# jinseikenai/glomeruli_segmentation

Measured on AMD Instinct MI355X. Metric: patches/sec (1024x512 RGB) ESPNet p=2 q=8 5 classes, HBM-resident, two batches in flight, higher is better.
Workload: dtype f32; 1 GPU; ESPNet p=2 q=8 encoder+decoder, batch=32 synthetic 1024x512 uint8 BGR tiles per GPU, normalise+forward+argmax+counts, inputs resident in HBM, steps rotate through 4 distinct batches, 2 batch(es) in flight (engine lanes, one HIP stream each) for `value`; global_batch=32, weights=espnet_fold1 (tests/golden), parallelism=tile-range per rank x1

## Files before the change

### glomeruli_segmentation_amd/_lib.py

```python
import ctypes
import os

_PKG = os.path.dirname(os.path.abspath(__file__))
LIB_PATH = os.path.join(_PKG, "libglomseg.so")
if os.environ.get("GLOMSEG_LIB") and os.environ.get("GLOMSEG_EXPERIMENT") == "1":
    LIB_PATH = os.environ["GLOMSEG_LIB"]

GS_OK = 0
GS_IN_U8_BGR_NHWC = 0
GS_IN_F32_NCHW = 1
ABI_VERSION = 9
GS_BUILD_DIAG = 1
GS_FORM_NONE = -1
GS_MAX_ENSEMBLE_C = 8
MAX_CROPS_PER_CALL = 64

STATUS_NAMES = {0: "GS_OK", 1: "GS_ERR_INVALID", 2: "GS_ERR_HIP", 3: "GS_ERR_NOMEM", 4: "GS_ERR_UNSUPPORTED",
                5: "GS_ERR_NODEVICE", 6: "GS_ERR_DEVICE_FAULT"}


class GlomsegError(RuntimeError):
    def __init__(self, status, message):
        super().__init__("%s: %s" % (STATUS_NAMES.get(status, status), message))
        self.status = status


class LayerDesc(ctypes.Structure):
    _fields_ = [("name", ctypes.c_char * 96), ("offset", ctypes.c_int64), ("ndim", ctypes.c_int32),
                ("shape", ctypes.c_int32 * 4)]


class CropDesc(ctypes.Structure):
    _fields_ = [("in_off", ctypes.c_int64), ("out_off", ctypes.c_int64), ("h", ctypes.c_int32), ("w", ctypes.c_int32),
                ("x1", ctypes.c_int32), ("y1", ctypes.c_int32)]


class PasteTarget(ctypes.Structure):
    _fields_ = [("slide_map", ctypes.c_void_p), ("map_h", ctypes.c_int32), ("map_w", ctypes.c_int32), ("ds", ctypes.c_int32),
                ("sx_lut", ctypes.c_void_p), ("sy_lut", ctypes.c_void_p)]


class CropOverlay(ctypes.Structure):
    _fields_ = [("palette_rgb", ctypes.c_void_p), ("n_colours", ctypes.c_int32), ("wa", ctypes.c_float), ("wb", ctypes.c_float),
                ("out_bgr", ctypes.POINTER(ctypes.c_void_p))]


class CropScoring(ctypes.Structure):
    _fields_ = [("labels", ctypes.POINTER(ctypes.c_void_p)), ("conf", ctypes.c_void_p), ("seen", ctypes.c_void_p),
                ("gt_overlay_bgr", ctypes.POINTER(ctypes.c_void_p)), ("gt_clamp", ctypes.c_int32)]


class EvalBox(ctypes.Structure):
    _fields_ = [("x0", ctypes.c_int32), ("y0", ctypes.c_int32), ("x1", ctypes.c_int32), ("y1", ctypes.c_int32),
                ("raster_w", ctypes.c_int32), ("raster_h", ctypes.c_int32), ("offset", ctypes.c_int64)]


class EvalSet(ctypes.Structure):
    _fields_ = [("rasters", ctypes.c_void_p), ("raster_bytes", ctypes.c_int64), ("boxes", ctypes.c_void_p),
                ("n_boxes", ctypes.c_int32), ("win_ptr", ctypes.c_void_p), ("win_idx", ctypes.c_void_p), ("n_idx", ctypes.c_int32),
                ("small_map", ctypes.c_void_p)]


class DetectorLayerPlan(ctypes.Structure):
    _fields_ = [("images", ctypes.c_int64), ("in_h", ctypes.c_int32), ("in_w", ctypes.c_int32), ("out_h", ctypes.c_int32),
                ("out_w", ctypes.c_int32), ("form", ctypes.c_int32)]


class DetectorPlan(ctypes.Structure):
    _fields_ = [("hf", ctypes.c_int32), ("wf", ctypes.c_int32), ("workspace_bytes", ctypes.c_int64), ("n_layers", ctypes.c_int32),
                ("layers", DetectorLayerPlan * 16)]


class KernelTime(ctypes.Structure):
    _fields_ = [("name", ctypes.c_char * 64), ("total_ms", ctypes.c_double), ("launches", ctypes.c_int64),
                ("flops_per_tile", ctypes.c_double)]


_P = ctypes.c_void_p
_FP = ctypes.POINTER(ctypes.c_float)
_I = ctypes.c_int

PROTOTYPES = {
    "gs_last_error": (ctypes.c_char_p, []),
    "gs_abi_version": (_I, []),
    "gs_build_flags": (_I, []),
    "gs_device_fault_check": (_I, []),
    "gs_espnet_create": (_I, [_P, ctypes.POINTER(LayerDesc), _I, _I, _I, _I, _I, ctypes.POINTER(_P)]),
    "gs_espnet_destroy": (None, [_P]),
    "gs_espnet_reserve": (_I, [_P, _I, _I, _I]),
    "gs_espnet_forward": (_I, [_P, _P, _I, _I, _I, _I, _FP, _FP, _P, _P, _P, _P]),
    "gs_espnet_set_lanes": (_I, [_P, _I]),
    "gs_espnet_lanes": (_I, [_P]),
    "gs_espnet_forward_lane": (_I, [_P, _I, _P, _I, _I, _I, _I, _FP, _FP, _P, _P, _P, _P]),
    "gs_espnet_segment_host": (_I, [_P, _P, _I, _I, _I, _FP, _FP, _I, _P, _P]),
    "gs_espnet_segment_crops": (_I, [_P, _I, _P, ctypes.POINTER(CropDesc), _I, _FP, _FP, _I, _I, _P, _P, _P,
                                ctypes.POINTER(PasteTarget), _P]),
    "gs_espnet_ensemble_segment_crops": (_I, [ctypes.POINTER(_P), _I, _P, ctypes.POINTER(CropDesc), _I, _FP, _FP, _I, _I, _P, _P, _P,
                                         ctypes.POINTER(PasteTarget), _P]),
    "gs_espnet_segment_crops_host": (_I, [ctypes.POINTER(_P), _I, ctypes.POINTER(_P), ctypes.POINTER(_I), ctypes.POINTER(_I), _I, _FP, _FP,
                                     _I, _I, _I, ctypes.POINTER(_P), _P, _P, ctypes.POINTER(PasteTarget), ctypes.POINTER(_I),
                                     ctypes.POINTER(_I), ctypes.POINTER(CropOverlay)]),
    "gs_plan_crop_batches": (_I, [ctypes.POINTER(_I), ctypes.POINTER(_I), _I, _I, ctypes.POINTER(_I), _I, ctypes.POINTER(_I)]),
    "gs_host_block_is_pinned": (_I, [_P, ctypes.c_size_t]),
    "gs_espnet_ensemble_forward": (_I, [ctypes.POINTER(_P), _I, _P, _I, _I, _I, _FP, _FP, _P, _P, _P]),
    "gs_espnet_read_stage": (_I, [_P, ctypes.c_char_p, _I, _P, ctypes.c_size_t, ctypes.POINTER(_I * 3)]),
    "gs_espnet_block_forward": (_I, [_P, _I, _I, _I, _P, _I, _I, _P]),
    "gs_espnet_plan_forward": (_I, [_I, _I, _I, _I, _I, _I, _I, ctypes.POINTER(_I), _I, ctypes.POINTER(_I)]),
    "gs_espnet_form_info": (_I, [_I, _I, ctypes.POINTER(ctypes.c_char_p), ctypes.POINTER(_I)]),
    "gs_espnet_profile_enable": (_I, [_P, _I]),
    "gs_espnet_profile_read": (_I, [_P, ctypes.POINTER(KernelTime), _I, ctypes.POINTER(_I)]),
    "gs_crop_preprocess": (_I, [_P, _I, _I, _FP, _FP, _I, _I, _P, _P]),
    "gs_mask_resize_nearest": (_I, [_P, _I, _I, _I, _I, _P, _P]),
    "gs_find_contours": (_I, [_P, _I, _I, _I, _P, _I, _P, _I, ctypes.POINTER(_I), ctypes.POINTER(_I)]),
    "gs_arc_length_closed": (ctypes.c_double, [_P, _I]),
    "gs_approx_poly_closed": (_I, [_P, _I, ctypes.c_double, _P]),
    "gs_wsi_paste_max": (_I, [_P, _I, _I, _I, _P, _I, _I, _I, _I, _P]),
    "gs_wsi_paste_max_lut": (_I, [_P, _I, _I, _I, _P, _P, _P, _I, _I, _I, _I, _P]),
    "gs_overlay_classmap": (_I, [_P, _P, _I, _I, _P, _I, ctypes.c_float, ctypes.c_float, _P, _P]),
    "gs_confusion_u8": (_I, [_P, _P, ctypes.c_longlong, _I, _P, _P]),
    "gs_wsi_eval_windows": (_I, [_I, _I, _I, _I, ctypes.POINTER(EvalSet), ctypes.POINTER(EvalSet), _P, _P, _I, _I, _P, _P, _P]),
    "gs_conv2d_nhwc": (_I, [_P, _I, _I, _I, _I, _P, _I, _I, _I, _P, _I, _I, _I, _P, _P]),
    "gs_conv2d_nhwc_form": (_I, [_I] * 10 + [ctypes.POINTER(ctypes.c_char_p)]),
    "gs_roialign": (_I, [_P, _I, _I, _I, _I, _P, _P, _I, _I, _P, _P]),
    "gs_nms": (_I, [_P, _P, _I, ctypes.c_float, ctypes.c_float, _I, _P, _P, _P]),
    "gs_detector_create": (_I, [_P, ctypes.POINTER(LayerDesc), _I, ctypes.POINTER(_P)]),
    "gs_detector_destroy": (None, [_P]),
    "gs_detector_max_detections": (_I, []),
    "gs_detector_num_proposals": (_I, []),
    "gs_detector_layer_info": (_I, [_I, ctypes.POINTER(ctypes.c_char_p)] + [ctypes.POINTER(_I)] * 6),
    "gs_detector_plan": (_I, [_I, _I, _I, ctypes.POINTER(DetectorPlan)]),
    "gs_detector_set_thresholds": (_I, [_P, ctypes.c_float, ctypes.c_float, ctypes.c_float]),
    "gs_detector_forward": (_I, [_P, _P, _I, _I, _I, _P, _P, _P, _P, _P, _P, _P, _P, _P]),
    "gs_detector_detect_host": (_I, [_P, ctypes.POINTER(_P), _I, _I, _I, _I, _P, _P, _P, _P]),
}

SCORING_PROTOTYPES = {
    "gs_espnet_score_crops": (_I, [_P, _P, ctypes.POINTER(CropDesc), _I, _I, _I, _I, _P, _P, _P]),
    "gs_espnet_segment_crops_host_scored": (_I, PROTOTYPES["gs_espnet_segment_crops_host"][1] + [ctypes.POINTER(CropScoring)]),
}

_lib = None


def load():
    global _lib
    if _lib is not None:
        return _lib
    if not os.path.exists(LIB_PATH):
        raise ImportError(
            "%s is missing: build it with `python -m glomeruli_segmentation_amd.build` "
            "(hipcc --offload-arch=gfx950).  There is no CPU fallback." % LIB_PATH)
    lib = ctypes.CDLL(LIB_PATH, mode=ctypes.RTLD_GLOBAL)
    for name, (res, args) in list(PROTOTYPES.items()) + list(SCORING_PROTOTYPES.items()):
        fn = getattr(lib, name)
        fn.restype = res
        fn.argtypes = args
    if lib.gs_abi_version() != ABI_VERSION:
        raise ImportError("libglomseg.so ABI %d != binding ABI %d: rebuild" % (lib.gs_abi_version(), ABI_VERSION))
    if (lib.gs_build_flags() & GS_BUILD_DIAG) and os.environ.get("GLOMSEG_ALLOW_DIAG") != "1":
        raise ImportError("%s is a -DGS_DIAG experiment build (its timing variants return wrong results by construction); "
                          "set GLOMSEG_ALLOW_DIAG=1 to load it for an A/B measurement" % LIB_PATH)
    _lib = lib
    return lib


def check(status):
    if status != GS_OK:
        raise GlomsegError(status, load().gs_last_error().decode("utf-8", "replace"))


def fptr3(values):
    arr = (ctypes.c_float * len(values))(*[float(v) for v in values])
    return arr
```

### glomeruli_segmentation_amd/build.py

```python
import os
import subprocess
import sys
import tempfile

PKG = os.path.dirname(os.path.abspath(__file__))
CSRC = os.path.join(PKG, "csrc")
LIB = os.path.join(PKG, "libglomseg.so")
SOURCES = ["espnet.hip", "dec_tail.hip", "crops.hip", "detect_ops.hip", "detector.hip", "wsi_eval.hip", "contours.cpp"]
HEADERS = ["gs_internal.h", "conv_mfma.h", "dec_tail.h", "dec_tail_args.h", "espnet_kernels.h", "crop_sample.h", "crop_plan.h", "detect_math.h", "detect_plan.h", "host_copy.h", "host_jobs.h", "host_pipe.h",
           os.path.join("..", "..", "include", "glomseg.h"), os.path.join("..", "..", "include", "glomseg_scoring.h")]
FLAGS = ["-O3", "--offload-arch=gfx950", "-std=c++17", "-fPIC", "-Wall", "-Wno-unused-result",
         "-Wno-unused-value"]


def _sources():
    return [s for s in SOURCES if os.path.exists(os.path.join(CSRC, s))]


def _stale(lib):
    if not os.path.exists(lib):
        return True
    t = os.path.getmtime(lib)
    deps = [os.path.join(CSRC, s) for s in _sources() + HEADERS] + [os.path.abspath(__file__)]
    deps += [os.path.join(CSRC, f) for f in os.listdir(CSRC) if f.endswith(".h") or f.endswith(".inc")]
    return any(os.path.getmtime(d) > t for d in deps)


def build_lib(force=False, verbose=False, out=None, extra_flags=()):
    lib = os.path.abspath(out) if out else LIB
    if not (force or _stale(lib)):
        return lib
    hipcc = os.environ.get("HIPCC", "/opt/rocm/bin/hipcc")
    os.makedirs(os.path.dirname(lib), exist_ok=True)
    objdir = CSRC if out is None else tempfile.mkdtemp(prefix="glomseg_obj_")
    objs = []
    procs = []
    for s in _sources():
        o = os.path.join(objdir, s.replace(".hip", ".o").replace(".cpp", ".o"))
        objs.append(o)
        cmd = [hipcc] + FLAGS + list(extra_flags) + (["-x", "hip"] if s.endswith(".cpp") else []) + ["-c", os.path.join(CSRC, s), "-o", o]
        if verbose:
            print(" ".join(cmd))
        procs.append((cmd, subprocess.Popen(cmd)))
    for cmd, p in procs:
        if p.wait() != 0:
            raise RuntimeError("hipcc failed: " + " ".join(cmd))
    cmd = [hipcc, "--offload-arch=gfx950", "-shared", "-fPIC", "-o", lib] + objs + ["-Wl,-rpath,/opt/rocm/lib"]
    if verbose:
        print(" ".join(cmd))
    subprocess.check_call(cmd)
    return lib


if __name__ == "__main__":
    argv = sys.argv[1:]
    extra = []
    if "--" in argv:
        extra = argv[argv.index("--") + 1:]
        argv = argv[:argv.index("--")]
    out = argv[argv.index("--out") + 1] if "--out" in argv else None
    print(build_lib(force="--force" in argv or out is not None, verbose=True, out=out, extra_flags=extra))
```

### glomeruli_segmentation_amd/csrc/conv_mfma.h

```cpp
#pragma once
#include <map>
#include <mutex>
#include <type_traits>

#include "gs_internal.h"

namespace gs {

#ifdef GS_DIAG
constexpr bool kDiag = true;
#else
constexpr bool kDiag = false;
#endif

template <int N, typename F>
__device__ __forceinline__ void static_for(F &&f)
{
    if constexpr (N > 0) {
        static_for<N - 1>(f);
        f(std::integral_constant<int, N - 1>{});
    }
}

typedef float f32x16 __attribute__((ext_vector_type(16)));
typedef float f32x4 __attribute__((ext_vector_type(4)));

template <int MT>
struct Mfma;
template <>
struct Mfma<32> {
    static constexpr int KL = 2, NACC = 16;
    using acc_t = f32x16;
    static __device__ __forceinline__ acc_t run(float a, float b, acc_t c)
    {
        return __builtin_amdgcn_mfma_f32_32x32x2f32(a, b, c, 0, 0, 0);
    }
    static __device__ __forceinline__ int row(int r, int kq) { return (r & 3) + 8 * (r >> 2) + 4 * kq; }
};
template <>
struct Mfma<16> {
    static constexpr int KL = 4, NACC = 4;
    using acc_t = f32x4;
    static __device__ __forceinline__ acc_t run(float a, float b, acc_t c)
    {
        return __builtin_amdgcn_mfma_f32_16x16x4f32(a, b, c, 0, 0, 0);
    }
    static __device__ __forceinline__ int row(int r, int kq) { return kq * 4 + r; }
};

struct ConvArgs {
    const float *in;
    long long in_sn;
    int in_sc, in_pitch, in_off;
    unsigned in_img_bytes;
    const float *wpack;
    int wfloats;
    float *out;
    long long out_sn;
    int out_sc, out_pitch, out_off;
    unsigned out_img_bytes, res_img_bytes;
    const float *res;
    long long res_sn;
    int res_sc, res_pitch, res_off;
    float *out2;
    long long out2_sn;
    int out2_sc, out2_pitch, out2_off, out2_coff;
    unsigned out2_img_bytes;
    float *out3;
    long long out3_sn;
    int out3_sc, out3_pitch, out3_off, nout3;
    unsigned out3_img_bytes;
    int bnl_s0, bnl_s1;
    int stagger;
    int prio_mode;
    unsigned long long *stamp;
    int N, H, W;
    int strips;
    int total_tasks;
    int wu;
};

typedef unsigned u32x3_t __attribute__((ext_vector_type(3)));
typedef unsigned u32x2_t __attribute__((ext_vector_type(2)));
typedef unsigned u32x4_t __attribute__((ext_vector_type(4)));

template <int N, int AUX = 0>
__device__ __forceinline__ void buf_load_vec(const __amdgpu_buffer_rsrc_t &rs, int voff, int soff, float *dst)
{
    if constexpr (N == 1) {
        dst[0] = __builtin_bit_cast(float, __builtin_amdgcn_raw_buffer_load_b32(rs, voff, soff, AUX));
    } else if constexpr (N == 2) {
        const u32x2_t v = __builtin_amdgcn_raw_buffer_load_b64(rs, voff, soff, AUX);
        const unsigned e0 = v[0], e1 = v[1];
        dst[0] = __builtin_bit_cast(float, e0);
        dst[1] = __builtin_bit_cast(float, e1);
    } else {
        static_assert(N == 4 || N == 8, "vector width");
#pragma unroll
        for (int h = 0; h < N / 4; ++h) {
            const u32x4_t v = __builtin_amdgcn_raw_buffer_load_b128(rs, voff + 16 * h, soff, AUX);
            const unsigned e0 = v[0], e1 = v[1], e2 = v[2], e3 = v[3];
            dst[4 * h + 0] = __builtin_bit_cast(float, e0);
            dst[4 * h + 1] = __builtin_bit_cast(float, e1);
            dst[4 * h + 2] = __builtin_bit_cast(float, e2);
            dst[4 * h + 3] = __builtin_bit_cast(float, e3);
        }
    }
}
template <int N, int AUX = 0>
__device__ __forceinline__ void buf_store_vec(const __amdgpu_buffer_rsrc_t &rs, int voff, const float *src)
{
    if constexpr (N == 1) {
        __builtin_amdgcn_raw_buffer_store_b32(__builtin_bit_cast(unsigned, src[0]), rs, voff, 0, AUX);
    } else if constexpr (N == 2) {
        u32x2_t v;
        v[0] = __builtin_bit_cast(unsigned, src[0]);
        v[1] = __builtin_bit_cast(unsigned, src[1]);
        __builtin_amdgcn_raw_buffer_store_b64(v, rs, voff, 0, AUX);
    } else {
#pragma unroll
        for (int h = 0; h < N / 4; ++h) {
            u32x4_t v;
#pragma unroll
            for (int j = 0; j < 4; ++j)
                v[j] = __builtin_bit_cast(unsigned, src[4 * h + j]);
            __builtin_amdgcn_raw_buffer_store_b128(v, rs, voff + 16 * h, 0, AUX);
        }
    }
}

__device__ __forceinline__ float prelu_pin(float alpha)
{
    return alpha <= 1.0f ? __builtin_inff() : -__builtin_inff();
}
__device__ __forceinline__ float prelu_med3(float v, float alpha, float pin)
{
    return __builtin_amdgcn_fmed3f(v, alpha * v, pin);
}

constexpr int F_BNACT = 1;
constexpr int F_RES = 2;
constexpr int F_NOSTORE = 4;
constexpr int F_DUAL = 8;
constexpr int F_S2PAIR = 512;
constexpr int F_VEC = 1024;
constexpr int F_RES_NT = 8192;
constexpr int F_ST_NT = 16384;
constexpr int F_ST2_NT = 32768;
constexpr int F_IN_NT = 65536;
constexpr int F_A_GLOBAL = 131072;
constexpr int F_FUSE1X1 = 262144;
constexpr int F_S2_FLIP = 1048576;
constexpr int F_SKIP_PAD = 4194304;
constexpr int F_BNLOAD = 8388608;
constexpr int F_X_NOLOAD = 16;
constexpr int F_X_NOLDS = 32;
constexpr int F_X_NOEPI = 64;
constexpr int F_X_STAMP2 = 4096;
constexpr int STAMP2_SLOTS = 128;
constexpr int F_X_STAMP = 128;
constexpr int F_X_NOEPIMEM = 2097152;
constexpr int F_X_RESL2 = 33554432;
constexpr int F_X_STL2 = 67108864;
constexpr int F_X_ALL = F_X_NOLOAD | F_X_NOLDS | F_X_NOEPI | F_X_STAMP | F_X_STAMP2 | F_X_NOEPIMEM | F_X_RESL2 | F_X_STL2;

struct ConvImage {
    int nrow, cout, w, bn, tab, total;
};
constexpr ConvImage conv_image(int CINP, int TAPS, int NDIL, int NOUT1, int NOUT, bool bn, bool dual = false, int fuse_nacc = 0)
{
    ConvImage im{};
    im.nrow = NOUT1 > NOUT ? NOUT1 : NOUT;
    im.cout = NOUT1 + (NDIL - 1) * NOUT;
    im.w = NDIL * TAPS * CINP * im.nrow;
    im.bn = (bn ? 3 * im.cout : 0) + (dual ? 3 * im.cout : 0);
    im.tab = NDIL * fuse_nacc * 64;
    im.total = (im.w + im.bn + im.tab + 3) / 4 * 4;
    return im;
}

#ifndef CFG_STAGE_ROT
#define CFG_STAGE_ROT 17
#endif
#ifndef CFG_L3_RING
#define CFG_L3_RING 13
#endif
#ifndef CFG_L2_RING
#define CFG_L2_RING 27
#endif
constexpr int conv_ring_depth(int MT, int TAPS, int NDIL, int P, int G)
{
    return (MT == 32 && TAPS == 9 && NDIL == 5 && (P == 1 || P == 2) && G == 13) ? CFG_L3_RING
           : (MT == 16 && TAPS == 9 && NDIL == 5 && P == 4 && G == 9) ? CFG_L2_RING
                                                                    : G * (TAPS == 9 ? 3 : 1);
}

#define M_KL_OF(MT_) (Mfma<MT_>::KL)
template <int MT, int WAVES, int CINP, int TAPS, int STRIDE, int NDIL, int NOUT1, int NOUT, int P, int G, int FLAGS>
__global__ void __launch_bounds__(WAVES * 64, WAVES >= 8 ? WAVES / 8 : 2) conv_mfma_kernel(const ConvArgs a)
{
    constexpr bool BNACT = FLAGS & F_BNACT, RES = FLAGS & F_RES, STORE1 = !(FLAGS & F_NOSTORE), DUAL = FLAGS & F_DUAL;
    constexpr bool S2P = FLAGS & F_S2PAIR;
    constexpr bool VEC = FLAGS & F_VEC;
    constexpr bool AGL = FLAGS & F_A_GLOBAL, FUSE = FLAGS & F_FUSE1X1;
    constexpr bool S2FLIP = FLAGS & F_S2_FLIP;
    constexpr bool SKIP = FLAGS & F_SKIP_PAD;
    constexpr bool BNL = FLAGS & F_BNLOAD;
    static_assert(!BNL || ((FLAGS & F_S2PAIR) && !(FLAGS & (F_BNACT | F_A_GLOBAL | F_VEC))), "F_BNLOAD is for the plain stride-2 reduce");
    static_assert(!SKIP || (TAPS == 9 && STRIDE == 1 && !(FLAGS & F_S2PAIR) && G * M_KL_OF(MT) == CINP),
                  "F_SKIP_PAD: unit-stride 3x3 with one tap row per chunk");
    static_assert(!S2FLIP || (STRIDE == 2 && TAPS == 9 && NDIL == 1), "F_S2_FLIP is for the stride-2 3x3 reduce");
    static_assert(kDiag || !(FLAGS & F_X_ALL), "timing / stamp variants exist in -DGS_DIAG builds only");
    constexpr int IAUX = (FLAGS & F_IN_NT) ? 2 : 0;
    constexpr int RAUX = (FLAGS & F_RES_NT) ? 2 : 0, SAUX = (FLAGS & F_ST_NT) ? 2 : 0, SAUX2 = (FLAGS & F_ST2_NT) ? 2 : 0;
    static_assert(!VEC || (STRIDE == 1 && (P == 2 || P == 4 || P == 8)), "F_VEC needs unit stride and P in {2,4,8}");
    static_assert(!S2P || (STRIDE == 2 && TAPS == 9 && NDIL == 1), "F_S2PAIR is for the stride-2 3x3 reduce");
    using M = Mfma<MT>;
    constexpr int KL = M::KL;
    constexpr int NSTEP = CINP / KL;
    constexpr int NROW = NOUT1 > NOUT ? NOUT1 : NOUT;
    constexpr int COUT = NOUT1 + (NDIL - 1) * NOUT;
    constexpr int TYN = TAPS == 1 ? 1 : 3;
    constexpr int TXN = TAPS == 9 ? 3 : 1;
    constexpr int XSTEP = P * MT;
    constexpr int RGN = TYN * NSTEP;
    constexpr int D = G * TXN;
    constexpr int R = conv_ring_depth(MT, TAPS, NDIL, P, G);
    constexpr int RA = R;
    static_assert(D % R == 0 && (R == D || !(FLAGS & (F_S2PAIR | F_BNLOAD))), "the ring divides the chunk");
    constexpr int CPD = RGN / G;
    constexpr int NCHUNK = NDIL * CPD;
    static_assert(CINP % KL == 0, "k-steps must tile");
    static_assert(TAPS == 1 || TAPS == 9, "1x1 or 3x3");
    static_assert(RGN % G == 0, "chunk must divide the row groups of one dilation");
    static_assert(NROW <= MT, "one MFMA row block");
    constexpr int KSTR = 4;

    extern __shared__ __attribute__((aligned(16))) float lds[];
    const int tid = threadIdx.x;
    unsigned long long tstamp0 = 0;
    if (FLAGS & (F_X_STAMP | F_X_STAMP2))
        tstamp0 = __builtin_amdgcn_s_memrealtime();
    constexpr int WFL = NDIL * TAPS * CINP * NROW;
    constexpr int LDS_SRC0 = AGL ? WFL : 0;
    static_assert(!AGL || WFL % 4 == 0, "LDS-DMA source must stay 16-byte aligned");
    static_assert(!FUSE || (TAPS == 9 && BNACT), "the fused 1x1 follows a branch kernel's epilogue");
    const float *bnp = lds + (WFL - LDS_SRC0);
    constexpr int BNFL = (BNACT ? 3 * COUT : 0) + (DUAL ? 3 * COUT : 0);
    const float *tab = bnp + BNFL;
    constexpr int BNL_C = CINP + M::KL;
    const float *bnl = lds + (conv_image(CINP, TAPS, NDIL, NOUT1, NOUT, BNACT, DUAL, FUSE ? M::NACC : 0).total - LDS_SRC0);
    const __amdgpu_buffer_rsrc_t rsrc_w =
        __builtin_amdgcn_make_buffer_rsrc(const_cast<float *>(a.wpack), 0, AGL ? WFL * 4 : 0, 0x00020000);

    const int lane = tid & 63;
    const int wid = __builtin_amdgcn_readfirstlane(tid >> 6);
    const int px = lane % MT, kq = lane / MT;
    const int xl = VEC ? px * P : px;
    const int voff = (kq * a.in_sc + xl * STRIDE) * 4;
    const int lbase = kq * NROW + (px < NROW ? px : NROW - 1);
    const int vout = (kq * KSTR * a.out_sc + xl) * 4;
    const int vres = RES ? (kq * KSTR * a.res_sc + xl) * 4 : 0;
    const int vout2 = DUAL ? (kq * KSTR * a.out2_sc + xl) * 4 : 0;
    const int vout3 = FUSE ? (kq * KSTR * a.out3_sc + xl) * 4 : 0;
    const int prio_mode = kDiag ? a.prio_mode : 1;
    const bool second_of_simd = WAVES >= 8 ? wid >= WAVES / 2 : blockIdx.x >= gridDim.x / 2;

    const int NB = gridDim.x;
    const int wu = a.wu;
    int t0, t1, tstride;
    if ((NB & 7) == 0) {
        const int xcd = blockIdx.x & 7, per = NB >> 3;
        const int c0 = (int)((long long)a.total_tasks * xcd / 8), c1 = (int)((long long)a.total_tasks * (xcd + 1) / 8);
        t0 = c0 + (blockIdx.x >> 3) * wu + wid;
        t1 = c1;
        tstride = per * wu;
    } else {
        t0 = blockIdx.x * wu + wid;
        t1 = a.total_tasks;
        tstride = NB * wu;
    }
    if (wid >= wu)
        t0 = t1;
    const long long wg = (long long)blockIdx.x * WAVES + wid;
    const int tasks_per_img = a.H * a.strips;
    bool staged = false;

    float aq[RA], bq[S2P ? 1 : R][P];
    float bl[S2P ? G : 1][P][3];

    for (int task = t0; task < t1 || !staged; task += tstride) {
        const bool idle = task >= t1;
        const int tk = idle ? (a.total_tasks - 1) : task;
        const int n = tk / tasks_per_img;
        const int rem = tk - n * tasks_per_img;
        const int img_stride = tstride / tasks_per_img > 0 ? tstride / tasks_per_img : 1;
        const int yrot = SKIP ? a.H / 2 : 0;
        const int y0r = rem / a.strips;
        const int y = SKIP && ((n / img_stride) & 1) ? (y0r + yrot >= a.H ? y0r + yrot - a.H : y0r + yrot) : y0r;
        const int x0 = (rem - y0r * a.strips) * XSTEP;

        const __amdgpu_buffer_rsrc_t rsrc = __builtin_amdgcn_make_buffer_rsrc(
            const_cast<float *>(a.in + (long long)n * a.in_sn), 0, a.in_img_bytes, 0x00020000);
        const int sbase = (a.in_off + y * STRIDE * a.in_pitch + x0 * STRIDE) * 4;
        const int tn = task + tstride < t1 ? task + tstride : tk;
        const int n_n = tn / tasks_per_img;
        const int rem_n = tn - n_n * tasks_per_img;
        const int y0r_n = rem_n / a.strips;
        const int y_n = SKIP && ((n_n / img_stride) & 1) ? (y0r_n + yrot >= a.H ? y0r_n + yrot - a.H : y0r_n + yrot) : y0r_n;
        const __amdgpu_buffer_rsrc_t rsrc_n = __builtin_amdgcn_make_buffer_rsrc(
            const_cast<float *>(a.in + (long long)n_n * a.in_sn), 0, a.in_img_bytes, 0x00020000);
        const int sbase_n = (a.in_off + y_n * STRIDE * a.in_pitch + (rem_n - y0r_n * a.strips) * XSTEP * STRIDE) * 4;
        const bool flip = S2FLIP && (y & 1), flip_n = S2FLIP && (y_n & 1);
        const __amdgpu_buffer_rsrc_t rout =
            __builtin_amdgcn_make_buffer_rsrc(a.out + (long long)n * a.out_sn, 0, a.out_img_bytes, 0x00020000);
        const int sout = (a.out_off + y * a.out_pitch + x0) * 4;
        const __amdgpu_buffer_rsrc_t rres = __builtin_amdgcn_make_buffer_rsrc(
            const_cast<float *>(RES ? a.res + (long long)n * a.res_sn : a.in), 0, RES ? a.res_img_bytes : 0u, 0x00020000);
        const int sres = RES ? (a.res_off + y * a.res_pitch + x0) * 4 : 0;
        const __amdgpu_buffer_rsrc_t rout2 = __builtin_amdgcn_make_buffer_rsrc(
            DUAL ? a.out2 + (long long)n * a.out2_sn : a.out, 0, DUAL ? a.out2_img_bytes : 0u, 0x00020000);
        const int sout2 = DUAL ? (a.out2_off + y * a.out2_pitch + x0) * 4 : 0;
        const __amdgpu_buffer_rsrc_t rout3 = __builtin_amdgcn_make_buffer_rsrc(
            FUSE ? a.out3 + (long long)n * a.out3_sn : a.out, 0, FUSE ? a.out3_img_bytes : 0u, 0x00020000);
        const int sout3 = FUSE ? (a.out3_off + y * a.out3_pitch + x0) * 4 : 0;

        typename M::acc_t acc[P];
        typename M::acc_t acc2[FUSE ? P : 1];
        auto chunk_live = [&](int yy, int c) {
            const int di = c / CPD, ty = c - di * CPD;
            return ty == 1 || (ty == 0 ? yy >= (1 << di) : yy + (1 << di) < a.H);
        };
        const int c_first = SKIP && !chunk_live(y, 0) ? 1 : 0;
        const int c_first_n = SKIP && !chunk_live(y_n, 0) ? 1 : 0;

        constexpr int OOB = 0x7ffffff0;
        int vo[P], vr[P], vo2[P], vo3[P];
#pragma unroll
        for (int p = 0; p < P; ++p) {
            const bool xok = x0 + (VEC ? xl : p * MT + px) < a.W;
            vo[p] = xok ? vout + (VEC ? 0 : p * MT * 4) : OOB;
            vr[p] = xok ? vres + (VEC ? 0 : p * MT * 4) : OOB;
            vo2[p] = xok ? vout2 + (VEC ? 0 : p * MT * 4) : OOB;
            vo3[p] = xok ? vout3 + (VEC ? 0 : p * MT * 4) : OOB;
        }
        constexpr int RR = RES ? M::NACC : 1;
        float resv[RR][P];
        auto load_res = [&](int di, int r) {
            if (!RES)
                return;
            if (FLAGS & F_X_NOEPIMEM) {
#pragma unroll
                for (int p = 0; p < P; ++p)
                    resv[r % RR][p] = __builtin_bit_cast(float, di + r + p);
                return;
            }
            const int nout = di == 0 ? NOUT1 : NOUT;
            const int cb = di == 0 ? 0 : NOUT1 + (di - 1) * NOUT;
            const int ch0 = M::row(r, 0);
            const bool live = ch0 + kq * KSTR < nout;
            const int sr = (cb + ch0) * a.res_sc * 4 + sres;
            if (VEC) {
                if (FLAGS & F_X_RESL2)
                    buf_load_vec<P, RAUX>(rres, live ? ((int)(wg & 255) * 8192 + ((vr[0] + sr) & 0x1ff0)) : OOB, 0, resv[r % RR]);
                else
                    buf_load_vec<P, RAUX>(rres, live ? vr[0] : OOB, sr, resv[r % RR]);
                return;
            }
#pragma unroll
            for (int p = 0; p < P; ++p)
                resv[r % RR][p] = __builtin_bit_cast(
                    float, __builtin_amdgcn_raw_buffer_load_b32(rres, live ? vr[p] : OOB, sr, RAUX));
        };
        auto prefetch_res = [&](int di) {
#pragma unroll
            for (int r = 0; r < RR; ++r)
                load_res(di, r);
        };

        auto decode_rg = [&](int cw, int g, int &ty0, int &sidx) {
            if constexpr (G % NSTEP == 0) {
                ty0 = cw * (G / NSTEP) + g / NSTEP;
                sidx = g % NSTEP;
            } else if constexpr (NSTEP % G == 0) {
                constexpr int CPR = NSTEP / G;
                ty0 = cw / CPR;
                sidx = (cw - ty0 * CPR) * G + g;
            } else {
                const int rg = cw * G + g;
                ty0 = rg / NSTEP;
                sidx = rg - ty0 * NSTEP;
            }
        };
        auto fetch_b = [&](const __amdgpu_buffer_rsrc_t &rs, int sb, int c, int g, int tx, bool fl) {
            const int di = c / CPD;
            int ty0, sidx;
            decode_rg(c - di * CPD, g, ty0, sidx);
            const int ty = S2FLIP && fl ? TYN - 1 - ty0 : ty0;
            const int toff = TAPS == 9 ? ((ty - 1) * a.in_pitch + (tx - 1)) << di : 0;
            const int soff = sb + (toff + sidx * KL * a.in_sc) * 4;
            if ((FLAGS & F_X_NOLOAD) && staged)
                return;
            if (VEC) {
                buf_load_vec<P, IAUX>(rs, voff, soff, bq[S2P ? 0 : (g * TXN + tx) % R]);
                return;
            }
#pragma unroll
            for (int p = 0; p < P; ++p)
                bq[(g * TXN + tx) % R][p] = __builtin_bit_cast(
                    float, __builtin_amdgcn_raw_buffer_load_b32(rs, voff + p * MT * STRIDE * 4, soff, IAUX));
        };
        auto fetch_pair = [&](const __amdgpu_buffer_rsrc_t &rs, int sb, int c, int g, bool fl) {
            if ((FLAGS & F_X_NOLOAD) && staged)
                return;
            int ty0, sidx;
            decode_rg(c, g, ty0, sidx);
            const int ty = S2FLIP && fl ? TYN - 1 - ty0 : ty0;
            const int soff = sb + ((ty - 1) * a.in_pitch - 1 + sidx * KL * a.in_sc) * 4;
#pragma unroll
            for (int p = 0; p < P; ++p) {
                const u32x3_t v = __builtin_amdgcn_raw_buffer_load_b96(rs, voff + p * MT * STRIDE * 4, soff, IAUX);
                const unsigned e0 = v[0], e1 = v[1], e2 = v[2];
                bl[g][p][0] = __builtin_bit_cast(float, e0);
                bl[g][p][1] = __builtin_bit_cast(float, e1);
                bl[g][p][2] = __builtin_bit_cast(float, e2);
            }
        };
        auto fetch_a = [&](int c, int g, int tx, bool fl) {
            const int di = c / CPD;
            int ty0, sidx;
            decode_rg(c - di * CPD, g, ty0, sidx);
            const int ty = S2FLIP && fl ? TYN - 1 - ty0 : ty0;
            const int tap = TAPS == 9 ? ty * 3 + tx : 0;
            if ((FLAGS & F_X_NOLDS) && staged)
                return;
            if (AGL)
                aq[(g * TXN + tx) % R] = __builtin_bit_cast(
                    float, __builtin_amdgcn_raw_buffer_load_b32(rsrc_w, lbase * 4, (((di * TAPS + tap) * CINP + sidx * KL) * NROW) * 4, 0));
            else
                aq[(g * TXN + tx) % R] = lds[((di * TAPS + tap) * CINP + sidx * KL) * NROW + lbase];
        };

        auto bnl_fetch = [&](int cc, int gg, int yy, bool ff, float &sc2, float &sh2, float &al2, bool &raw) {
            int ty0c, sidxc;
            decode_rg(cc, gg, ty0c, sidxc);
            const int tyc = S2FLIP && ff ? TYN - 1 - ty0c : ty0c;
            raw = sidxc >= a.bnl_s0 && sidxc < a.bnl_s1;
            const bool padrow = yy * STRIDE + tyc - 1 < 0 && raw;
            const int ch = (padrow ? NSTEP : sidxc) * KL + kq;
            sc2 = bnl[ch];
            sh2 = bnl[BNL_C + ch];
            al2 = bnl[2 * BNL_C + ch];
        };
        float tsc = 1.0f, tsh = 0.0f, tal = 1.0f, tpin = 0.0f;
        float nsc = 1.0f, nsh = 0.0f, nal = 1.0f;
        bool traw = false, nraw = false;
        float bt[BNL ? 2 : 1][P][3];
        static_assert(!BNL || G % 2 == 0, "F_BNLOAD: the two-group operand buffer alternates by row-group parity");
        auto bnl_apply = [&](float &dst, float v, float sc2, float sh2, float al2, float pin2, bool zero) {
            v = v * sc2 + sh2;
            v = prelu_med3(v, al2, pin2);
            dst = zero ? 0.0f : v;
        };

        if (task == t0) {
#pragma unroll
            for (int g = 0; g < G; ++g) {
                if (S2P) {
                    fetch_pair(rsrc, sbase, 0, g, flip);
                    continue;
                }
#pragma unroll
                for (int tx = 0; tx < TXN; ++tx)
                    if (g * TXN + tx < R)
                        fetch_b(rsrc, sbase, c_first, g, tx, flip);
            }
        }
        if (!staged) {
            const int pieces = (a.wfloats - LDS_SRC0 + 255) / 256;
            if ((FLAGS & F_X_STAMP2) && lane == 0)
                a.stamp[wg * STAMP2_SLOTS + STAMP2_SLOTS - 2] = __builtin_amdgcn_s_memrealtime();
            const int rot = (int)((blockIdx.x * (unsigned)CFG_STAGE_ROT) % (unsigned)(pieces > 0 ? pieces : 1));
            for (int j0 = wid; j0 < pieces; j0 += WAVES) {
                const int j = j0 + rot < pieces ? j0 + rot : j0 + rot - pieces;
                __builtin_amdgcn_global_load_lds(
                    (const __attribute__((address_space(1))) void *)(a.wpack + LDS_SRC0 + j * 256 + lane * 4),
                    (__attribute__((address_space(3))) void *)(lds + j * 256), 16, 0, 0);
            }
            if ((FLAGS & F_X_STAMP2) && lane == 0)
                a.stamp[wg * STAMP2_SLOTS + STAMP2_SLOTS - 1] = __builtin_amdgcn_s_memrealtime();
            __syncthreads();
            staged = true;
        }
        if (idle)
            break;
        if ((FLAGS & F_X_STAMP) && lane == 0 && task == t0) {
            a.stamp[wg * 8 + 0] = tstamp0;
            a.stamp[wg * 8 + 1] = __builtin_amdgcn_s_memrealtime();
        }
        if ((FLAGS & F_X_STAMP2) && lane == 0 && task == t0) {
            a.stamp[wg * STAMP2_SLOTS + 0] = tstamp0;
            a.stamp[wg * STAMP2_SLOTS + 1] = __builtin_amdgcn_s_memrealtime();
        }
        const int ti_ = (FLAGS & F_X_STAMP2) ? (task - t0) / tstride : 0;
        const bool stamp2 = (FLAGS & F_X_STAMP2) && lane == 0 && 2 + (ti_ + 1) * 2 * NCHUNK <= STAMP2_SLOTS;
        const long long sbase2 = wg * STAMP2_SLOTS + 2 + ti_ * 2 * NCHUNK;
        if (kDiag && a.stagger > 0 && task == t0) {
            const int ph = second_of_simd ? 1 : 0;
            for (int z = 0; z < a.stagger * ph; ++z)
                __builtin_amdgcn_s_sleep(16);
        }
        if (task == t0) {
#pragma unroll
            for (int g = 0; g < G; ++g)
#pragma unroll
                for (int tx = 0; tx < TXN; ++tx)
                    if (g * TXN + tx < R)
                        fetch_a(c_first, g, tx, flip);
        }

        if (BNL) {
            bnl_fetch(c_first, 0, y, flip, tsc, tsh, tal, traw);
            bnl_fetch(c_first, 1, y, flip, nsc, nsh, nal, nraw);
            tpin = prelu_pin(tal);
#pragma unroll
            for (int p = 0; p < P; ++p)
#pragma unroll
                for (int t = 0; t < 3; ++t)
                    bnl_apply(bt[0][p][t], bl[0][p][t], tsc, tsh, tal, tpin, t == 0 && p == 0 && x0 == 0 && px == 0);
        }
        if (FUSE) {
#pragma unroll
            for (int p = 0; p < P; ++p)
                acc2[p] = (typename M::acc_t)(0.0f);
        }
        if (prio_mode == 1) {
            if ((((task - t0) / tstride) + (second_of_simd ? 1 : 0)) & 1)
                __builtin_amdgcn_s_setprio(1);
            else
                __builtin_amdgcn_s_setprio(0);
        } else if (prio_mode == 3 && task == t0) {
            if (second_of_simd)
                __builtin_amdgcn_s_setprio(1);
        }

        struct EpiParams {
            float scale = 1.0f, shift = 0.0f, alpha = 1.0f, scale2 = 1.0f, shift2 = 0.0f, alpha2 = 1.0f, a2 = 0.0f;
        };
        auto epi_params = [&](int di, auto r_) __attribute__((always_inline)) {
            constexpr int r = decltype(r_)::value;
            const int nout = di == 0 ? NOUT1 : NOUT;
            const int cb = di == 0 ? 0 : NOUT1 + (di - 1) * NOUT;
            const int ch0 = M::row(r, 0);
            const bool live = ch0 + kq * KSTR < nout;
            EpiParams q;
            q.a2 = (FUSE && BNACT) ? tab[(di * M::NACC + r) * 64 + lane] : 0.0f;
            if (BNACT) {
                const float *bp = bnp + (live ? cb + ch0 + kq * KSTR : 0);
                q.scale = bp[0];
                q.shift = bp[COUT];
                q.alpha = bp[2 * COUT];
                if (DUAL) {
                    q.scale2 = bp[3 * COUT];
                    q.shift2 = bp[4 * COUT];
                    q.alpha2 = bp[5 * COUT];
                }
            }
            return q;
        };
        auto epi_reg = [&](int di, auto r_) __attribute__((always_inline)) {
            constexpr int r = decltype(r_)::value;
            const int nout = di == 0 ? NOUT1 : NOUT;
            const int cb = di == 0 ? 0 : NOUT1 + (di - 1) * NOUT;
            const int ch0 = M::row(r, 0);
            const bool live = ch0 + kq * KSTR < nout;
            const EpiParams q = epi_params(di, r_);
            const float a2 = q.a2;
            const int so = (cb + ch0) * a.out_sc * 4 + sout;
            const int so2 = DUAL ? (a.out2_coff + cb + ch0) * a.out2_sc * 4 + sout2 : 0;
            const float scale = q.scale, shift = q.shift, alpha = q.alpha, scale2 = q.scale2, shift2 = q.shift2, alpha2 = q.alpha2;
            float o1[P], o2[P];
            const float pin = prelu_pin(alpha), pin2 = prelu_pin(alpha2);
#pragma unroll
            for (int p = 0; p < P; ++p) {
                float v = acc[p][r];
                if (RES)
                    v += resv[r % RR][p];
                if (BNACT) {
                    v = v * scale + shift;
                    v = prelu_med3(v, alpha, pin);
                }
                o1[p] = v;
                if (!VEC && STORE1)
                    __builtin_amdgcn_raw_buffer_store_b32(__builtin_bit_cast(unsigned, v), rout, live ? vo[p] : OOB, so, SAUX);
                if (DUAL) {
                    float v2 = v * scale2 + shift2;
                    v2 = prelu_med3(v2, alpha2, pin2);
                    o2[p] = v2;
                    if (!VEC)
                        __builtin_amdgcn_raw_buffer_store_b32(__builtin_bit_cast(unsigned, v2), rout2,
                                                              live ? vo2[p] : OOB, so2, SAUX2);
                }
            }
            if (VEC && STORE1 && !(FLAGS & F_X_NOEPIMEM))
                buf_store_vec<P, SAUX>(rout, live ? ((FLAGS & F_X_STL2) ? ((int)(wg & 255) * 8192 + ((vo[0] + so) & 0x1ff0)) : vo[0] + so) : OOB, o1);
            if (VEC && DUAL)
                buf_store_vec<P, SAUX2>(rout2, live ? vo2[0] + so2 : OOB, o2);
            if (FUSE && ch0 < nout) {
#pragma unroll
                for (int p = 0; p < P; ++p)
                    acc2[p] = M::run(a2, o1[p], acc2[p]);
            }
        };

        for (int c = 0; c < NCHUNK; ++c) {
            if (NDIL > 1 && c % CPD == 0 && prio_mode == 0) {
                if (((c / CPD) + (second_of_simd ? 1 : 0)) & 1)
                    __builtin_amdgcn_s_setprio(1);
                else
                    __builtin_amdgcn_s_setprio(0);
            }
            if (RES && c % CPD == 0)
                prefetch_res(c / CPD);
            if (c % CPD == 0 && c < 2 * CPD) {
#pragma unroll
                for (int p = 0; p < P; ++p)
                    acc[p] = (typename M::acc_t)(0.0f);
            }
            int nxl = c + 1;
            if (SKIP)
                while (nxl < NCHUNK && !chunk_live(y, nxl))
                    ++nxl;
            const bool last = nxl >= NCHUNK;
            const int nx = last ? c_first_n : nxl;
            const __amdgpu_buffer_rsrc_t rs = last ? rsrc_n : rsrc;
            const int sb = last ? sbase_n : sbase;
            const bool fl = last ? flip_n : flip;
            auto refill = [&](int u) __attribute__((always_inline)) {
                const int v = u + R;
                if (v < D && R < D) {
                    fetch_b(rsrc, sbase, c, v / TXN, v % TXN, flip);
                    fetch_a(c, v / TXN, v % TXN, flip);
                } else {
                    const int gn = (v - D) / TXN, txn = (v - D) % TXN;
                    if (!S2P)
                        fetch_b(rs, sb, nx, gn, txn, fl);
                    else if (txn == 2)
                        fetch_pair(rs, sb, nx, gn, fl);
                    fetch_a(nx, gn, txn, fl);
                }
            };
            if (!SKIP || chunk_live(y, c)) {
#pragma unroll
            for (int g = 0; g < G; ++g)
#pragma unroll
                for (int tx = 0; tx < TXN; ++tx) {
                    const int u = g * TXN + tx;
                    const bool ahead = BNL && (g + 1 < G || !last);
                    if (BNL && tx == 0) {
                        tsc = nsc;
                        tsh = nsh;
                        tal = nal;
                        traw = nraw;
                        tpin = prelu_pin(tal);
                        if (g + 2 < G)
                            bnl_fetch(c, g + 2, y, flip, nsc, nsh, nal, nraw);
                        else if (!last)
                            bnl_fetch(nx, g + 2 - G, y, flip, nsc, nsh, nal, nraw);
                    }
#pragma unroll
                    for (int p = 0; p < P; ++p) {
                        acc[p] = M::run(aq[u % RA], BNL ? bt[BNL ? g & 1 : 0][p][S2P ? tx : 0]
                                                       : S2P ? bl[S2P ? g : 0][p][S2P ? tx : 0] : bq[S2P ? 0 : u % R][p], acc[p]);
                        if (ahead) {
                            const int e = tx * P + p;
                            if (e < 3 * P)
                                bnl_apply(bt[BNL ? (g + 1) & 1 : 0][e / 3][e % 3], bl[S2P ? (g + 1) % G : 0][e / 3][e % 3], tsc, tsh, tal, tpin,
                                          e == 0 && x0 == 0 && px == 0);
                        }
                    }
                    refill(u);
                    __builtin_amdgcn_sched_barrier(0);
                }
            }
            if (stamp2)
                a.stamp[sbase2 + 2 * c] = __builtin_amdgcn_s_memrealtime();
            if ((c + 1) % CPD != 0)
                continue;
            if (FLAGS & F_X_NOEPI) {
                float keep = 0.0f;
#pragma unroll
                for (int p = 0; p < P; ++p)
#pragma unroll
                    for (int r = 0; r < M::NACC; ++r)
                        keep += acc[p][r];
                if (keep == 123.456f)
                    __builtin_amdgcn_raw_buffer_store_b32(__builtin_bit_cast(unsigned, keep), rout, vout, sout, 0);
                continue;
            }
            const int di = c / CPD;
            static_for<M::NACC>([&](auto r_) { epi_reg(di, r_); });
            if (FUSE && di + 1 == NDIL) {
#pragma unroll
                for (int r = 0; r < M::NACC; ++r) {
                    const int ch0 = M::row(r, 0);
                    if (ch0 >= a.nout3)
                        continue;
                    const bool live3 = ch0 + kq * KSTR < a.nout3;
                    const int so3 = ch0 * a.out3_sc * 4 + sout3;
                    float o3[P];
#pragma unroll
                    for (int p = 0; p < P; ++p) {
                        o3[p] = acc2[p][r];
                        if (!VEC)
                            __builtin_amdgcn_raw_buffer_store_b32(__builtin_bit_cast(unsigned, o3[p]), rout3, live3 ? vo3[p] : OOB, so3, 0);
                    }
                    if (VEC)
                        buf_store_vec<P, 0>(rout3, live3 ? vo3[0] + so3 : OOB, o3);
                }
            }
            if ((FLAGS & F_X_STAMP) && lane == 0 && task == t0)
                a.stamp[wg * 8 + 2 + di] = __builtin_amdgcn_s_memrealtime();
            if (stamp2)
                a.stamp[sbase2 + 2 * c + 1] = __builtin_amdgcn_s_memrealtime();
        }
    }
}

constexpr int conv_wfloats(int CINP, int TAPS, int NDIL, int NOUT1, int NOUT, bool bn, bool dual = false, int fuse_nacc = 0)
{
    return conv_image(CINP, TAPS, NDIL, NOUT1, NOUT, bn, dual, fuse_nacc).total;
}

struct LaunchInfo {
    bool attr_done = false;
    int per_cu = 0;
};

template <int MT, int WAVES, int CINP, int TAPS, int STRIDE, int NDIL, int NOUT1, int NOUT, int P, int G, int FLAGS>
gs_status launch_conv_mfma(ConvArgs a, int num_cus, hipStream_t stream)
{
    auto kern = conv_mfma_kernel<MT, WAVES, CINP, TAPS, STRIDE, NDIL, NOUT1, NOUT, P, G, FLAGS>;
    constexpr ConvImage im = conv_image(CINP, TAPS, NDIL, NOUT1, NOUT, FLAGS & F_BNACT, FLAGS & F_DUAL,
                                        (FLAGS & F_FUSE1X1) ? Mfma<MT>::NACC : 0);
    a.strips = cdiv(a.W, P * MT);
    a.total_tasks = a.N * a.H * a.strips;
    a.prio_mode = 1;
#ifdef GS_DIAG
    if (const char *e = std::getenv("GS_PRIO"))
        a.prio_mode = std::atoi(e);
    if (const char *e = std::getenv("GS_STAGGER"))
        a.stagger = std::atoi(e);
#endif
    constexpr int EXTRA = (FLAGS & F_BNLOAD) ? 3 * (CINP + Mfma<MT>::KL) : 0;
    a.wfloats = im.total + EXTRA;
    const int lds_floats = im.total + EXTRA - ((FLAGS & F_A_GLOBAL) ? im.w : 0);
    const size_t lds_bytes = (size_t)((lds_floats + 255) / 256 * 256) * sizeof(float);
    static std::mutex mu;
    static std::map<int, LaunchInfo> by_device;
    int dev = 0;
    GS_HIP(hipGetDevice(&dev));
    int per_cu;
    {
        std::lock_guard<std::mutex> lock(mu);
        LaunchInfo &li = by_device[dev];
        if (!li.attr_done) {
            GS_HIP(hipFuncSetAttribute(reinterpret_cast<const void *>(kern), hipFuncAttributeMaxDynamicSharedMemorySize,
                                       (int)lds_bytes));
            li.attr_done = true;
        }
        if (li.per_cu == 0) {
            int nb = 0;
            GS_HIP(hipOccupancyMaxActiveBlocksPerMultiprocessor(&nb, reinterpret_cast<const void *>(kern), WAVES * 64, lds_bytes));
            li.per_cu = nb < 1 ? 1 : nb;
        }
        per_cu = li.per_cu;
    }
    int grid = num_cus * per_cu;
    if (grid >= 8) grid = grid / 8 * 8;
    a.wu = WAVES;
    if ((long long)a.total_tasks < (long long)grid * WAVES) {
        a.wu = cdiv(a.total_tasks, grid);
        if (a.wu < 1) a.wu = 1;
        int g = cdiv(a.total_tasks, a.wu);
        if (g >= 8) g = (g + 7) / 8 * 8;
        grid = g < grid ? g : grid;
    }
    if (grid < 1) grid = 1;
    hipLaunchKernelGGL(kern, dim3(grid), dim3(WAVES * 64), lds_bytes, stream, a);
    GS_HIP(hipGetLastError());
    return GS_OK;
}

}
```

### glomeruli_segmentation_amd/csrc/espnet.hip

```cpp
#include <chrono>
#include <cmath>
#include <cstdio>
#include <cstdlib>
#include <functional>
#include <map>
#include <memory>
#include <string>
#include <thread>
#include <vector>

#include "conv_mfma.h"
#include "dec_tail_args.h"
#include "enc_head.h"
#include "enc_head_ens.h"
#include "espnet_config.h"
#include "forward_plan.h"
#include "espnet_kernels.h"
#include "host_copy.h"
#include "host_pipe.h"

namespace gs {

static thread_local std::string g_err;
void set_error(const char *fmt, ...)
{
    char buf[1024];
    va_list ap;
    va_start(ap, fmt);
    vsnprintf(buf, sizeof buf, fmt, ap);
    va_end(ap);
    g_err = buf;
}

#ifdef GS_DIAG
static bool getenv_flag(const char *name)
{
    const char *e = std::getenv(name);
    return e && std::atoi(e) != 0;
}
static bool no_vec() { return getenv_flag("GS_NO_VEC"); }
#else
static constexpr bool no_vec() { return false; }
#endif

enum KernelId {
    K_STEM, K_POOL, K_L2_C1S, K_L2_DOWN, K_L2_C1, K_L2_ESP, K_CAT_B2, K_L3_C1S, K_L3_DOWN, K_L3_C1, K_L3_ESP,
    K_DEC1, K_DEC2, K_DEC3, K_DEC_CONV, K_DEC4, K_DEC_TAIL, K_ENC_HEAD, K_ENC_HEAD_ENS, K_COUNT
};
static const char *kKernelNames[K_COUNT] = {
    "stem_kernel", "pool_kernel", "conv_l2_reduce_s2", "conv_l2_down_branches", "conv_l2_reduce_1x1",
    "conv_l2_esp_branches", "cat_b2_kernel", "conv_l3_reduce_s2", "conv_l3_down_branches", "conv_l3_reduce_1x1",
    "conv_l3_esp_branches", "dec1_kernel", "dec2_kernel", "dec3_kernel", "conv_dec_cbr", "dec4_kernel", "dec_tail_kernel",
    "enc_head_kernel", "enc_head_ens_kernel"};

struct PackedConv {
    long long c1 = -1, br = -1;
    bool fused_next = false;
};

struct Model {
    int classes = 0, p = 0, q = 0;
    int cp = 0;
    bool encoder_only = false;
    int device = 0, num_cus = 256;
#ifdef GS_DIAG
    int variant = 0;
#else
    static constexpr int variant = 0;
#endif
    float *dblob = nullptr;
    float stem_params[537] = {0};
    long long w1, bn1, b1, b2, b3, wcls, br, wup3, w3c, cbr0, wcc, bncc, wup2, bnu2, wclassifier, wtail;
    long long wconv = -1;
    long long wcc_mfma = -1;
    PackedConv l2_0;
    std::vector<PackedConv> l2, l3;
    PackedConv l3_0;

    void *ws = nullptr;
    size_t ws_bytes = 0;
    int ws_n = 0, ws_h = 0, ws_w = 0;
    Act a0c, a0, inp1, inp2, r2[2], bb[3], a1, r3[2], cc[3], o2c, tt, t3, ee, ff;
    float *prob = nullptr;
    size_t prob_bytes = 0;
    std::map<std::string, std::pair<Act, int>> stages;
    void set_stage(const std::string &name, const Act &act, int C)
    {
        for (auto it = stages.begin(); it != stages.end();)
            it = it->second.first.base == act.base ? stages.erase(it) : std::next(it);
        stages[name] = {act, C};
    }
    int last_n = 0;
    bool b2_lazy = false;

    bool profile = false;
    struct Ev { hipEvent_t a, b; int k; };
    std::vector<Ev> events;
    double prof_ms[K_COUNT] = {0};
    long long prof_launches[K_COUNT] = {0};
    double prof_flops[K_COUNT] = {0};
};

struct WeightTable {
    const float *blob;
    std::map<std::string, const gs_layer_desc *> by_name;
    std::string prefix;
    bool ok = true;
    const float *get(const std::string &name, std::initializer_list<int> shape)
    {
        auto it = by_name.find(name);
        if (it == by_name.end()) {
            set_error("weight tensor '%s' missing from the table", name.c_str());
            ok = false;
            return nullptr;
        }
        const gs_layer_desc *d = it->second;
        int i = 0;
        bool match = d->ndim == (int)shape.size();
        for (int s : shape)
            match = match && d->shape[i++] == s;
        if (!match) {
            set_error("weight tensor '%s' has the wrong shape", name.c_str());
            ok = false;
            return nullptr;
        }
        return blob + d->offset;
    }
};

struct BlobBuilder {
    std::vector<float> data;
    long long reserve(size_t n)
    {
        const size_t at = (data.size() + 3) / 4 * 4;
        data.resize(at + (n + 3) / 4 * 4, 0.0f);
        return (long long)at;
    }
    long long push(const float *src, size_t n)
    {
        const long long at = reserve(n);
        std::memcpy(data.data() + at, src, n * sizeof(float));
        return at;
    }
};

static bool fold_bn(WeightTable &t, const std::string &bn, const std::string &act, int C, float *dst, bool with_alpha = true)
{
    const float *g = t.get(bn + ".weight", {C}), *b = t.get(bn + ".bias", {C});
    const float *m = t.get(bn + ".running_mean", {C}), *v = t.get(bn + ".running_var", {C});
    const float *al = act.empty() ? nullptr : t.get(act + ".weight", {C});
    if (!t.ok)
        return false;
    for (int c = 0; c < C; ++c) {
        const double inv = 1.0 / std::sqrt((double)v[c] + 1e-3);
        dst[c] = (float)((double)g[c] * inv);
        dst[C + c] = (float)((double)b[c] - (double)m[c] * (double)g[c] * inv);
        if (with_alpha)
            dst[2 * C + c] = al ? al[c] : 1.0f;
    }
    return true;
}

static void pack_conv(const float *w, int cout, int cin, int k, float *dst, int slot, int taps, int cinp, int nrow)
{
    for (int tap = 0; tap < taps; ++tap)
        for (int ci = 0; ci < cin; ++ci)
            for (int co = 0; co < cout; ++co)
                dst[(((size_t)slot * taps + tap) * cinp + ci) * nrow + co] = w[((size_t)co * cin + ci) * k * k + tap];
}

static bool pack_block(WeightTable &t, BlobBuilder &bb, const std::string &pre, bool down, int level, PackedConv &pc,
                       const float *dual = nullptr, int dual_coff = 0, int dual_c = 0, const std::string &next = "",
                       const float *in2_bn = nullptr, int in2_c0 = 0, int in2_cn = 0, int in2_c = 0)
{
    const int n = level == 2 ? 12 : 25, n1 = level == 2 ? 16 : 28, nOut = n1 + 4 * n;
    const int cin = level == 2 ? (down ? 19 : 64) : (down ? 131 : 128);
    const int kl = level == 2 ? 4 : 2;
    const int cinp = (cin + kl - 1) / kl * kl;
    const int taps = down ? 9 : 1;
    const float *wc1 = t.get(pre + ".c1.conv.weight", {n, cin, down ? 3 : 1, down ? 3 : 1});
    if (!t.ok)
        return false;
    const int c1_floats = conv_wfloats(cinp, taps, 1, n, n, false);
    const int bnl_c = cinp + kl;
    pc.c1 = bb.reserve(c1_floats + (in2_bn ? 3 * bnl_c : 0));
    pack_conv(wc1, n, cin, down ? 3 : 1, bb.data.data() + pc.c1, 0, taps, cinp, n);
    if (in2_bn) {
        float *x = bb.data.data() + pc.c1 + c1_floats;
        for (int c = 0; c < bnl_c; ++c) {
            const bool raw = c >= in2_c0 && c < in2_c0 + in2_cn, zero = c >= cinp;
            x[c] = zero ? 0.0f : raw ? in2_bn[c] : 1.0f;
            x[bnl_c + c] = zero ? 0.0f : raw ? in2_bn[in2_c + c] : 0.0f;
            x[2 * bnl_c + c] = raw ? in2_bn[2 * in2_c + c] : 1.0f;
        }
    }

    const int rcinp = (n + kl - 1) / kl * kl;
    const int mt = level == 2 ? 16 : 32, nacc = level == 2 ? 4 : 16;
    pc.fused_next = !next.empty();
    const ConvImage im = conv_image(rcinp, 9, 5, n1, n, true, dual != nullptr, pc.fused_next ? nacc : 0);
    pc.br = bb.reserve(im.total);
    static const char *dn[5] = {".d1", ".d2", ".d4", ".d8", ".d16"};
    for (int di = 0; di < 5; ++di) {
        const int co = di == 0 ? n1 : n;
        const float *w = t.get(pre + dn[di] + ".conv.weight", {co, n, 3, 3});
        if (!t.ok)
            return false;
        pack_conv(w, co, n, 3, bb.data.data() + pc.br, di, 9, rcinp, n1);
    }
    if (pc.fused_next) {
        const float *w2 = t.get(next + ".c1.conv.weight", {n, nOut, 1, 1});
        if (!t.ok)
            return false;
        float *tab = bb.data.data() + pc.br + im.w + im.bn;
        for (int di = 0; di < 5; ++di) {
            const int nout = di == 0 ? n1 : n, cb = di == 0 ? 0 : n1 + (di - 1) * n;
            for (int r = 0; r < nacc; ++r)
                for (int lane = 0; lane < 64; ++lane) {
                    const int i = lane % mt, kq = lane / mt;
                    const int row = mt == 32 ? (r & 3) + 8 * (r >> 2) + 4 * kq : kq * 4 + r;
                    tab[(di * nacc + r) * 64 + lane] = (row < nout && i < n) ? w2[(size_t)i * nOut + cb + row] : 0.0f;
                }
        }
    }
    float *bnp = bb.data.data() + pc.br + im.w;
    if (dual)
        for (int j = 0; j < 3; ++j)
            for (int c = 0; c < nOut; ++c)
                bnp[(3 + j) * nOut + c] = dual[j * dual_c + dual_coff + c];
    return down ? fold_bn(t, pre + ".bn", pre + ".act", nOut, bnp) : fold_bn(t, pre + ".bn.bn", pre + ".bn.act", nOut, bnp);
}

static Act make_act(int C, int Cp, int H, int W, int pad_t, int pad_b, int pad_l, int pad_r)
{
    Act a;
    a.C = C;
    a.Cp = Cp;
    a.H = H;
    a.W = W;
    a.pitch = (int)round_up(pad_l + W + pad_r, 32);
    a.sc = (pad_t + H + pad_b) * a.pitch + 96;
    a.off = pad_t * a.pitch + pad_l;
    a.sn = (long long)Cp * a.sc;
    return a;
}

static gs_status layout_workspace(Model *m, int n, int H, int W)
{
    if (m->ws && n <= m->ws_n && H == m->ws_h && W == m->ws_w)
        return GS_OK;
    if (m->ws) {
        GS_HIP(hipDeviceSynchronize());
        GS_HIP(hipFree(m->ws));
        m->ws = nullptr;
    }
    const int cls = m->cp;
    const int H1 = H / 2, W1 = W / 2, H2 = H / 4, W2 = W / 4, H3 = H / 8, W3 = W / 8;
    m->a0c = make_act(cls + 19, cls + 20, H1, W1, 1, 1, 32, 1);
    m->inp1 = make_act(3, 3, H1, W1, 0, 0, 0, 0);
    m->inp2 = make_act(3, 3, H2, W2, 0, 0, 0, 0);
    for (int i = 0; i < 2; ++i)
        m->r2[i] = make_act(12, 12, H2, W2, 16, 16, 32, 16);
    for (int i = 0; i < 3; ++i)
        m->bb[i] = make_act(64, 64, H2, W2, 0, 0, 0, 0);
    m->a1 = make_act(131, 132, H2, W2, 1, 0, 32, 1);
    for (int i = 0; i < 2; ++i)
        m->r3[i] = make_act(25, 26, H3, W3, 16, 16, 32, 16);
    for (int i = 0; i < 3; ++i)
        m->cc[i] = make_act(128, 128, H3, W3, 0, 0, 0, 0);
    m->o2c = make_act(cls, cls, H2, W2, 0, 0, 0, 0);
    const bool dec3_mfma = dec3_on_mfma(cls);
    m->tt = dec3_mfma ? make_act(2 * cls, 2 * cls, H2, W2, 1, 1, 32, 1) : make_act(2 * cls, 2 * cls, H2, W2, 0, 0, 0, 0);
    m->t3 = dec3_mfma ? make_act(cls, cls, H2, W2, 0, 0, 0, 0) : make_act(1, 1, 8, 8, 0, 0, 0, 0);
    m->ff = make_act(cls, cls, H1, W1, 0, 0, 0, 0);
    const bool lazy_b2 = b2_is_lazy(m->p);
    if (lazy_b2)
        m->bb[0] = Act();
    Act *all[] = {&m->a0c, &m->inp1, &m->inp2, &m->r2[0], &m->r2[1], &m->bb[0], &m->bb[1], &m->bb[2], &m->a1, &m->r3[0], &m->r3[1],
                  &m->cc[0], &m->cc[1], &m->cc[2], &m->o2c, &m->tt, &m->t3, &m->ff};
    for (Act *a : all) {
        if ((unsigned long long)a->sn * sizeof(float) >= (1ull << 31)) {
            set_error("tile %dx%d is too large: an activation of one image exceeds 2 GiB", H, W);
            return GS_ERR_UNSUPPORTED;
        }
    }
    const size_t slack = 64 * 1024;
    size_t total = 0;
    for (Act *a : all)
        total += round_up(a->bytes(n) + slack, 256);
    void *ws = nullptr;
    if (hipMalloc(&ws, total) != hipSuccess) {
        set_error("workspace allocation of %zu bytes failed (n=%d, %dx%d)", total, n, H, W);
        return GS_ERR_NOMEM;
    }
    GS_HIP(hipMemset(ws, 0, total));
    GS_HIP(hipDeviceSynchronize());
    size_t at = 0;
    for (Act *a : all) {
        a->base = reinterpret_cast<float *>(static_cast<char *>(ws) + at);
        at += round_up(a->bytes(n) + slack, 256);
    }
    if (lazy_b2) {
        m->bb[0] = m->a1;
        m->bb[0].base = m->a1.base + (long long)64 * m->a1.sc;
        m->bb[0].C = 64;
        m->bb[0].Cp = 64;
    }
    m->ee = m->a0c;
    m->ee.C = cls;
    m->a0 = m->a0c;
    m->a0.base = m->a0c.base + (long long)cls * m->a0c.sc;
    m->a0.C = 19;
    m->ws = ws;
    m->ws_bytes = total;
    m->ws_n = n;
    m->ws_h = H;
    m->ws_w = W;
    return GS_OK;
}

struct Launcher {
    Model *m;
    hipStream_t s;
    gs_status st = GS_OK;
    int n;
    template <typename F>
    void run(int kid, double flops_per_tile, F &&f)
    {
        if (st != GS_OK)
            return;
        Model::Ev ev{nullptr, nullptr, kid};
        if (m->profile) {
            if (hipEventCreate(&ev.a) != hipSuccess || hipEventCreate(&ev.b) != hipSuccess ||
                hipEventRecord(ev.a, s) != hipSuccess) {
                set_error("profiling event setup failed");
                st = GS_ERR_HIP;
                return;
            }
        }
        st = f();
        if (st == GS_OK && hipGetLastError() != hipSuccess) {
            set_error("launch of %s failed", kKernelNames[kid]);
            st = GS_ERR_HIP;
        }
        if (m->profile && st == GS_OK) {
            hipEventRecord(ev.b, s);
            m->events.push_back(ev);
            m->prof_flops[kid] += flops_per_tile;
        }
    }
};

static ConvArgs conv_args(const Act &in, const float *wpack, const Act &out, const Act *res, int n)
{
    ConvArgs a{};
    a.in = in.base;
    a.in_sn = in.sn;
    a.in_sc = in.sc;
    a.in_pitch = in.pitch;
    a.in_off = in.off;
    a.in_img_bytes = (unsigned)(in.sn * sizeof(float));
    a.wpack = wpack;
    a.out = out.base;
    a.out_sn = out.sn;
    a.out_sc = out.sc;
    a.out_pitch = out.pitch;
    a.out_off = out.off;
    a.out_img_bytes = (unsigned)(out.sn * sizeof(float));
    if (res) {
        a.res = res->base;
        a.res_sn = res->sn;
        a.res_sc = res->sc;
        a.res_pitch = res->pitch;
        a.res_off = res->off;
        a.res_img_bytes = (unsigned)(res->sn * sizeof(float));
    }
    a.N = n;
    a.H = out.H;
    a.W = out.W;
    return a;
}

static inline unsigned blocks_for(long long items) { return (unsigned)((items + 255) / 256); }

#ifdef GS_DIAG
#include "espnet_diag.inc"
#define GS_DIAG_TRY(call)     \
    do {                      \
        gs_status dst_;       \
        if (call) return dst_; \
    } while (0)
#else
#define GS_DIAG_TRY(call) \
    do {                  \
    } while (0)
#define GS_DIAG_STAMPED(var, tag, ca, ...)
#endif

static gs_status not_planned(const char *launch_class)
{
    set_error("internal: the forward plan has no form for launch class %s", launch_class);
    return GS_ERR_INVALID;
}

template <int FLAGS, int... C>
static gs_status launch_vec(const ConvArgs &ca, int num_cus, hipStream_t s, bool vec)
{
    return vec ? launch_conv_mfma<C..., FLAGS | F_VEC>(ca, num_cus, s) : launch_conv_mfma<C..., FLAGS>(ca, num_cus, s);
}

static gs_status launch_l2_reduce(const Model *m, const ConvArgs &ca, hipStream_t s) { return launch_conv_mfma<CFG_L2_C1S, F_S2PAIR | POL_L2_C1S | S2FLIP_L2>(ca, m->num_cus, s); }
static gs_status launch_l2_c1(const Model *m, const ConvArgs &ca, hipStream_t s) { return launch_conv_mfma<CFG_L2_C1, POL_L2_C1>(ca, m->num_cus, s); }
static gs_status launch_l3_c1(const Model *m, const ConvArgs &ca, hipStream_t s) { return launch_conv_mfma<CFG_L3_C1, POL_L3_C1>(ca, m->num_cus, s); }

static gs_status launch_l2_down(const Model *m, form::l2_down f, const ConvArgs &ca, hipStream_t s)
{
    switch (f) {
    case form::l2_down::P2S_VEC: return launch_vec<F_BNACT | (POL_L2_DOWN & F_ST_NT) | FUSE_L2, CFG_L2_BR_P2S>(ca, m->num_cus, s, true);
    case form::l2_down::P4S_VEC_SKIP:
        GS_DIAG_STAMPED(162, "l2down", ca, F_BNACT | (POL_L2_DOWN & F_ST_NT) | FUSE_L2 | F_VEC, CFG_L2_BR_P4)
        return launch_conv_mfma<CFG_L2_BR_P4S, F_BNACT | (POL_L2_DOWN & F_ST_NT) | FUSE_L2 | F_VEC | F_SKIP_PAD>(ca, m->num_cus, s);
    case form::l2_down::P4_VEC:
        GS_DIAG_STAMPED(162, "l2down", ca, F_BNACT | (POL_L2_DOWN & F_ST_NT) | FUSE_L2 | F_VEC, CFG_L2_BR_P4)
        return launch_vec<F_BNACT | (POL_L2_DOWN & F_ST_NT) | FUSE_L2, CFG_L2_BR_P4>(ca, m->num_cus, s, true);
    case form::l2_down::P4: return launch_vec<F_BNACT | (POL_L2_DOWN & F_ST_NT) | FUSE_L2, CFG_L2_BR_P4>(ca, m->num_cus, s, false);
    case form::l2_down::UNFUSED_P4_VEC: return launch_vec<F_BNACT | (POL_L2_DOWN & F_ST_NT), CFG_L2_BR_P4>(ca, m->num_cus, s, true);
    case form::l2_down::UNFUSED_P4: return launch_vec<F_BNACT | (POL_L2_DOWN & F_ST_NT), CFG_L2_BR_P4>(ca, m->num_cus, s, false);
    case form::l2_down::none: break;
    }
    return not_planned("l2_down");
}

static gs_status launch_l2_esp_fused(const Model *m, form::l2_esp_fused f, const ConvArgs &ca, hipStream_t s)
{
    switch (f) {
    case form::l2_esp_fused::P2S_VEC: return launch_vec<F_BNACT | F_RES | POL_L2_ESP | FUSE_L2, CFG_L2_BR_P2S>(ca, m->num_cus, s, true);
    case form::l2_esp_fused::P4_VEC:
        GS_DIAG_STAMPED(161, "l2esp", ca, F_BNACT | F_RES | POL_L2_ESP | FUSE_L2 | F_VEC, CFG_L2_BR_P4)
        return launch_vec<F_BNACT | F_RES | POL_L2_ESP | FUSE_L2, CFG_L2_BR_P4>(ca, m->num_cus, s, true);
    case form::l2_esp_fused::P4: return launch_vec<F_BNACT | F_RES | POL_L2_ESP | FUSE_L2, CFG_L2_BR_P4>(ca, m->num_cus, s, false);
    case form::l2_esp_fused::UNFUSED_P4_VEC: return launch_vec<F_BNACT | F_RES | POL_L2_ESP, CFG_L2_BR_P4>(ca, m->num_cus, s, true);
    case form::l2_esp_fused::UNFUSED_P4: return launch_vec<F_BNACT | F_RES | POL_L2_ESP, CFG_L2_BR_P4>(ca, m->num_cus, s, false);
    case form::l2_esp_fused::none: break;
    }
    return not_planned("l2_esp_fused");
}

static gs_status launch_l2_esp_last(const Model *m, form::l2_esp_last f, const ConvArgs &ca, hipStream_t s)
{
    switch (f) {
    case form::l2_esp_last::P2S_VEC: return launch_vec<F_BNACT | F_RES | F_NOSTORE | F_DUAL | POL_L2_LAST, CFG_L2_BR_P2S>(ca, m->num_cus, s, true);
    case form::l2_esp_last::P4_VEC:
        GS_DIAG_STAMPED(163, "l2last", ca, F_BNACT | F_RES | F_NOSTORE | F_DUAL | POL_L2_LAST | F_VEC, CFG_L2_BR_P4)
        return launch_vec<F_BNACT | F_RES | F_NOSTORE | F_DUAL | POL_L2_LAST, CFG_L2_BR_P4>(ca, m->num_cus, s, true);
    case form::l2_esp_last::P4: return launch_vec<F_BNACT | F_RES | F_NOSTORE | F_DUAL | POL_L2_LAST, CFG_L2_BR_P4>(ca, m->num_cus, s, false);
    case form::l2_esp_last::none: break;
    }
    return not_planned("l2_esp_last");
}

static gs_status launch_l3_reduce(const Model *m, form::l3_reduce f, const ConvArgs &ca, hipStream_t s)
{
    switch (f) {
    case form::l3_reduce::BNL_P1: return launch_conv_mfma<CFG_L3_C1S_BNL_P1, F_S2PAIR | POL_L3_C1S | S2FLIP_L3 | F_BNLOAD>(ca, m->num_cus, s);
    case form::l3_reduce::BNL:
        GS_DIAG_STAMPED(165, "l3c1s", ca, F_S2PAIR | POL_L3_C1S | S2FLIP_L3 | F_BNLOAD, CFG_L3_C1S_BNL)
        return launch_conv_mfma<CFG_L3_C1S_BNL, F_S2PAIR | POL_L3_C1S | S2FLIP_L3 | F_BNLOAD>(ca, m->num_cus, s);
    case form::l3_reduce::C1S: return launch_conv_mfma<CFG_L3_C1S, F_S2PAIR | POL_L3_C1S | S2FLIP_L3>(ca, m->num_cus, s);
    case form::l3_reduce::none: break;
    }
    return not_planned("l3_reduce");
}

static gs_status launch_l3_down(const Model *m, form::l3_down f, const ConvArgs &ca, hipStream_t s)
{
    switch (f) {
    case form::l3_down::P1R: return launch_conv_mfma<CFG_L3_BR_P1R, F_BNACT | POL_L3_DOWN | FUSE_L3 | SKIP_L3 | (CFG_SMALL_AGL ? F_A_GLOBAL : 0)>(ca, m->num_cus, s);
    case form::l3_down::P2R_VEC:
        GS_DIAG_STAMPED(164, "l3down", ca, F_BNACT | POL_L3_DOWN | FUSE_L3 | F_VEC | SKIP_L3, CFG_L3_BR_P2R)
        return launch_conv_mfma<CFG_L3_BR_P2R, F_BNACT | POL_L3_DOWN | FUSE_L3 | F_VEC | SKIP_L3>(ca, m->num_cus, s);
    case form::l3_down::BR_VEC: return launch_conv_mfma<CFG_L3_BR, F_BNACT | POL_L3_DOWN | FUSE_L3 | F_VEC>(ca, m->num_cus, s);
    case form::l3_down::P2F: return launch_conv_mfma<CFG_L3_BR_P2F, F_BNACT | POL_L3_DOWN | FUSE_L3>(ca, m->num_cus, s);
    case form::l3_down::UNFUSED_BR_VEC: return launch_vec<F_BNACT | POL_L3_DOWN, CFG_L3_BR>(ca, m->num_cus, s, true);
    case form::l3_down::UNFUSED_BR: return launch_vec<F_BNACT | POL_L3_DOWN, CFG_L3_BR>(ca, m->num_cus, s, false);
    case form::l3_down::none: break;
    }
    return not_planned("l3_down");
}

static gs_status launch_l3_esp_fused(const Model *m, form::l3_esp_fused f, const ConvArgs &ca, int block, hipStream_t s)
{
    switch (f) {
    case form::l3_esp_fused::P1R: return launch_conv_mfma<CFG_L3_BR_P1R, F_BNACT | F_RES | POL_L3_ESP | FUSE_L3 | SKIP_L3 | (CFG_SMALL_AGL ? F_A_GLOBAL : 0)>(ca, m->num_cus, s);
    case form::l3_esp_fused::P2R_VEC:
        if (block == 1) {
            GS_DIAG_STAMPED(160, "l3esp", ca, F_BNACT | F_RES | F_VEC | POL_L3_ESP | FUSE_L3 | SKIP_L3, CFG_L3_BR_P2R)
        }
        return launch_conv_mfma<CFG_L3_BR_P2R, F_BNACT | F_RES | F_VEC | POL_L3_ESP | FUSE_L3 | SKIP_L3>(ca, m->num_cus, s);
    case form::l3_esp_fused::P2F: return launch_conv_mfma<CFG_L3_BR_P2F, F_BNACT | F_RES | FUSE_L3>(ca, m->num_cus, s);
    case form::l3_esp_fused::none: break;
    }
    return not_planned("l3_esp_fused");
}

static gs_status launch_l3_esp_last(const Model *m, form::l3_esp_last f, const ConvArgs &ca, hipStream_t s)
{
    switch (f) {
    case form::l3_esp_last::P1R: return launch_conv_mfma<CFG_L3_BR_P1R, F_BNACT | F_RES | POL_L3_ESP | SKIP_L3 | (CFG_SMALL_AGL ? F_A_GLOBAL : 0)>(ca, m->num_cus, s);
    case form::l3_esp_last::P2R_VEC: return launch_conv_mfma<CFG_L3_BR_P2R, F_BNACT | F_RES | F_VEC | POL_L3_ESP | SKIP_L3>(ca, m->num_cus, s);
    case form::l3_esp_last::BR_VEC: return launch_conv_mfma<CFG_L3_BR, F_BNACT | F_RES | F_VEC | POL_L3_ESP>(ca, m->num_cus, s);
    case form::l3_esp_last::P2: return launch_conv_mfma<CFG_L3_BR_P2, F_BNACT | F_RES>(ca, m->num_cus, s);
    case form::l3_esp_last::none: break;
    }
    return not_planned("l3_esp_last");
}

template <int CLS>
static gs_status launch_dec3(const Model *m, form::dec3 f, const ConvArgs &ca, hipStream_t s)
{
    switch (f) {
    case form::dec3::MT16:
    case form::dec3::MT32: return launch_vec<F_BNACT, dec_mt(CLS), 8, 2 * CLS, 9, 1, 1, CLS, CLS, dec_pixels(CLS), 3>(ca, m->num_cus, s, false);
    case form::dec3::MT16_VEC:
    case form::dec3::MT32_VEC: return launch_vec<F_BNACT, dec_mt(CLS), 8, 2 * CLS, 9, 1, 1, CLS, CLS, dec_pixels(CLS), 3>(ca, m->num_cus, s, true);
    case form::dec3::KERNEL:
    case form::dec3::none: break;
    }
    return not_planned("dec3");
}

template <int CLS>
static gs_status launch_dec_conv(const Model *m, form::dec_conv f, const ConvArgs &ca, hipStream_t s)
{
    constexpr int CINP = (19 + CLS + 3) / 4 * 4;
    switch (f) {
    case form::dec_conv::MT16:
    case form::dec_conv::MT32: return launch_vec<F_BNACT | POL_DEC_CONV, dec_mt(CLS), 8, CINP, 9, 1, 1, CLS, CLS, dec_pixels(CLS), 3>(ca, m->num_cus, s, false);
    case form::dec_conv::MT16_VEC:
    case form::dec_conv::MT32_VEC: return launch_vec<F_BNACT | POL_DEC_CONV, dec_mt(CLS), 8, CINP, 9, 1, 1, CLS, CLS, dec_pixels(CLS), 3>(ca, m->num_cus, s, true);
    case form::dec_conv::TAIL:
    case form::dec_conv::none: break;
    }
    return not_planned("dec_conv");
}

struct Encoded { int last; bool lazy_b2; };
static Encoded encode(Model *m, Launcher &L, const ForwardPlan &plan, const ForwardReq &r)
{
    const float *wb = m->dblob;
    const hipStream_t s = r.s;
    const int n = r.n, H = r.H, W = r.W, H1 = H / 2, W1 = W / 2, H2 = H / 4, W2 = W / 4, H3 = H / 8, W3 = W / 8;
    const double px1 = (double)H1 * W1, px2 = (double)H2 * W2, px3 = (double)H3 * W3;
    m->stages.clear();
    m->last_n = n;
    L.run(K_STEM, px1 * (27 * 16 * 2), [&] {
        StemArgs a{};
        a.in = r.in;
        for (int i = 0; i < 3; ++i) {
            a.mean[i] = r.mean ? r.mean[i] : 0.0f;
            a.std[i] = r.stdv ? r.stdv[i] : 1.0f;
        }
        std::memcpy(a.w1, m->stem_params, sizeof(float) * 432);
        std::memcpy(a.bn1, m->stem_params + 432, sizeof(float) * 48);
        std::memcpy(a.b1, m->stem_params + 480, sizeof(float) * 57);
        a.a0 = view(m->a0);
        a.inp1 = view(m->inp1);
        a.N = n;
        a.H = H;
        a.W = W;
        if (r.hist && ens_finishes((int)r.role)) {
            a.hist_zero = r.hist;
            a.hist_count = n * m->classes;
        }
        hipLaunchKernelGGL(r.in_format == GS_IN_U8_BGR_NHWC ? stem_kernel<true> : stem_kernel<false>,
                           dim3(blocks_for((long long)n * H1 * ((W1 + STEM_PX - 1) / STEM_PX))), dim3(256), 0, s, a);
        return GS_OK;
    });
    L.run(K_POOL, 0, [&] {
        hipLaunchKernelGGL(pool_kernel, dim3(blocks_for((long long)n * 3 * H2 * W2)), dim3(256), 0, s, view(m->inp1),
                           view(m->inp2), n, 3, m->p > 0 ? wb + m->b2 : nullptr, view(m->a1), 128, 131);
        return GS_OK;
    });
    m->set_stage("b1", m->a0, 19);
    m->set_stage("sample2", m->inp2, 3);

    L.run(K_L2_C1S, px2 * (19 * 9 * 12 * 2), [&] {
        GS_DIAG_TRY(diag_reduce_s2(m, 2, conv_args(m->a0, wb + m->l2_0.c1, m->r2[0], nullptr, n), s, dst_));
        return launch_l2_reduce(m, conv_args(m->a0, wb + m->l2_0.c1, m->r2[0], nullptr, n), s);
    });
    auto with_dual = [&](ConvArgs a, int coff) {
        a.out2 = m->a1.base;
        a.out2_sn = m->a1.sn;
        a.out2_sc = m->a1.sc;
        a.out2_pitch = m->a1.pitch;
        a.out2_off = m->a1.off;
        a.out2_coff = coff;
        a.out2_img_bytes = (unsigned)(m->a1.sn * sizeof(float));
        return a;
    };
    auto with_fused = [&](ConvArgs a, const Act &r, int nout3) {
        a.out3 = r.base;
        a.out3_sn = r.sn;
        a.out3_sc = r.sc;
        a.out3_pitch = r.pitch;
        a.out3_off = r.off;
        a.out3_img_bytes = (unsigned)(r.sn * sizeof(float));
        a.nout3 = nout3;
        return a;
    };
    const bool lazy_b2 = plan.lazy_b2;
    m->b2_lazy = lazy_b2;
    int rd2 = 0;
    L.run(K_L2_DOWN, px2 * (12 * 9 * 64 * 2) + (m->l2_0.fused_next ? px2 * (64 * 12 * 2) : 0), [&] {
        const ConvArgs ca = conv_args(m->r2[rd2], wb + m->l2_0.br, m->bb[0], nullptr, n);
        return launch_l2_down(m, plan.l2_down, m->l2_0.fused_next ? with_fused(ca, m->r2[rd2 ^ 1], 12) : ca, s);
    });
    bool have_r2 = m->l2_0.fused_next;
    rd2 ^= have_r2 ? 1 : 0;
    m->set_stage("level2_0", m->bb[0], 64);
    int cur2 = 0;
    for (int i = 0; i < m->p; ++i) {
        const int nxt = cur2 == 1 ? 2 : 1;
        const bool last = i == m->p - 1;
        const bool fuse_next = m->l2[i].fused_next;
        if (!have_r2)
            L.run(K_L2_C1, px2 * (64 * 12 * 2), [&] {
                return launch_l2_c1(m, conv_args(m->bb[cur2], wb + m->l2[i].c1, m->r2[rd2], nullptr, n), s);
            });
        L.run(K_L2_ESP, px2 * (12 * 9 * 64 * 2) + (fuse_next ? px2 * (64 * 12 * 2) : 0), [&] {
            const ConvArgs ca = conv_args(m->r2[rd2], wb + m->l2[i].br, m->bb[nxt], &m->bb[cur2], n);
            if (last)
                return launch_l2_esp_last(m, plan.l2_esp_last, with_dual(ca, 0), s);
            return launch_l2_esp_fused(m, plan.l2_esp_fused, fuse_next ? with_fused(ca, m->r2[rd2 ^ 1], 12) : ca, s);
        });
        have_r2 = fuse_next;
        rd2 ^= have_r2 ? 1 : 0;
        cur2 = nxt;
        if (!last)
            m->set_stage("level2." + std::to_string(i), m->bb[cur2], 64);
    }
    if (plan.cat_b2 == form::cat_b2::KERNEL) {
        L.run(K_CAT_B2, 0, [&] {
            hipLaunchKernelGGL(cat_b2_kernel, dim3(blocks_for((long long)n * 131 * H2 * W2)), dim3(256), 0, s, view(m->bb[cur2]),
                               view(m->bb[0]), view(m->inp2), wb + m->b2, view(m->a1), n);
            return GS_OK;
        });
    }
    m->set_stage("b2", m->a1, 131);

    int rd3 = 0;
    L.run(K_L3_C1S, px3 * (131 * 9 * 25 * 2), [&] {
        GS_DIAG_TRY(diag_reduce_s2(m, 3, conv_args(m->a1, wb + m->l3_0.c1, m->r3[0], nullptr, n), s, dst_));
        ConvArgs ca = conv_args(m->a1, wb + m->l3_0.c1, m->r3[0], nullptr, n);
        if (lazy_b2) {
            ca.bnl_s0 = 64 / 2;
            ca.bnl_s1 = 128 / 2;
        }
        return launch_l3_reduce(m, plan.l3_reduce, ca, s);
    });
    L.run(K_L3_DOWN, px3 * (25 * 9 * 128 * 2) + (m->l3_0.fused_next ? px3 * (128 * 25 * 2) : 0), [&] {
        const ConvArgs ca = conv_args(m->r3[rd3], wb + m->l3_0.br, m->cc[0], nullptr, n);
        return launch_l3_down(m, plan.l3_down, m->l3_0.fused_next ? with_fused(ca, m->r3[rd3 ^ 1], 25) : ca, s);
    });
    bool have_r3 = m->l3_0.fused_next;
    m->set_stage("level3_reduce", m->r3[rd3], 25);
    rd3 ^= have_r3 ? 1 : 0;
    m->set_stage("level3_0", m->cc[0], 128);
    int cur3 = 0;
    for (int i = 0; i < m->q; ++i) {
        const int nxt = cur3 == 1 ? 2 : 1;
        const bool fuse_next = m->l3[i].fused_next;
        if (!have_r3)
            L.run(K_L3_C1, px3 * (128 * 25 * 2), [&] {
                return launch_l3_c1(m, conv_args(m->cc[cur3], wb + m->l3[i].c1, m->r3[rd3], nullptr, n), s);
            });
        L.run(K_L3_ESP, px3 * (25 * 9 * 128 * 2) + (fuse_next ? px3 * (128 * 25 * 2) : 0), [&] {
            const ConvArgs ca = conv_args(m->r3[rd3], wb + m->l3[i].br, m->cc[nxt], &m->cc[cur3], n);
            GS_DIAG_TRY(diag_l3_esp(m, ca, i, s, dst_));
            if (fuse_next)
                return launch_l3_esp_fused(m, plan.l3_esp_fused, with_fused(ca, m->r3[rd3 ^ 1], 25), i, s);
            return launch_l3_esp_last(m, plan.l3_esp_last, ca, s);
        });
        have_r3 = fuse_next;
        rd3 ^= have_r3 ? 1 : 0;
        cur3 = nxt;
        m->set_stage("level3." + std::to_string(i), m->cc[cur3], 128);
    }
    return {cur3, lazy_b2};
}

template <int CLS>
static gs_status decode(Model *m, Launcher &L, const ForwardPlan &plan, const ForwardReq &r, const Encoded &enc)
{
    const float *wb = m->dblob;
    const hipStream_t s = r.s;
    const int n = r.n, H = r.H, W = r.W, H1 = H / 2, W1 = W / 2, H2 = H / 4, W2 = W / 4, H3 = H / 8, W3 = W / 8;
    const double px1 = (double)H1 * W1, px2 = (double)H2 * W2, px3 = (double)H3 * W3;
    const int ncls = m->classes;
    float *enc_logits = !m->encoder_only ? nullptr : r.logits ? r.logits : m->o2c.base;
    L.run(K_DEC1, px3 * (256 * ncls * 2) + px3 * (ncls * ncls * 4 * 2), [&] {
        Dec1Args a{};
        a.c0 = view(m->cc[0]);
        a.clast = view(m->cc[enc.last]);
        a.b3w = wb + m->b3;
        a.br = m->encoder_only ? nullptr : wb + m->br;
        a.wup = m->encoder_only ? nullptr : wb + m->wup3;
        a.out = view(m->o2c);
        a.enc_logits = enc_logits;
        a.N = n;
        a.classes = ncls;
        constexpr int CB = CLS <= 5 ? 16 : CLS <= 8 ? 8 : 4;
        hipLaunchKernelGGL((dec1_kernel<CLS, CB>), dim3((unsigned)(((long long)n * H3 * W3 + 63) / 64)), dim3(256), 0, s, a);
        return GS_OK;
    });
    if (m->encoder_only) {
        if (r.mask)
            L.run(K_ENC_HEAD, (double)H * W * (ncls * 6), [&] {
                EncHeadArgs a{};
                a.logits = enc_logits;
                a.mask = r.mask;
                a.hist = r.hist;
                a.classes = ncls;
                a.H3 = H3;
                a.W3 = W3;
                launch_enc_head(a, n, s);
                return GS_OK;
            });
        return L.st;
    }
    m->set_stage("up_l3", m->o2c, ncls);

    L.run(K_DEC2, px2 * (131 * ncls * 2), [&] {
        Dec2Args a{};
        a.a1 = view(m->a1);
        a.raw = view(m->bb[0]);
        a.b2 = wb + m->b2;
        a.raw_c0 = 64;
        a.raw_cn = enc.lazy_b2 ? 64 : 0;
        a.o2c = view(m->o2c);
        a.w3c = wb + m->w3c;
        a.br = wb + m->cbr0;
        a.t = view(m->tt);
        a.N = n;
        a.classes = ncls;
        hipLaunchKernelGGL(dec2_kernel<CLS>, dim3((unsigned)(((long long)n * H2 * W2 + 63) / 64)), dim3(256), 0, s, a);
        return GS_OK;
    });
    if (ncls == CLS)
        m->set_stage("combine_t", m->tt, 2 * CLS);
    if constexpr (dec3_on_mfma(CLS)) {
        L.run(K_DEC3, px2 * (2 * ncls * 9 * ncls * 2), [&] {
            return launch_dec3<CLS>(m, plan.dec3, conv_args(m->tt, wb + m->wcc_mfma, m->t3, nullptr, n), s);
        });
        L.run(K_DEC3, px2 * (ncls * ncls * 4 * 2), [&] {
            Dec3Args a{};
            a.t = view(m->t3);
            a.wup = wb + m->wup2;
            a.bnu = wb + m->bnu2;
            a.e = view(m->ee);
            a.N = n;
            a.classes = ncls;
            hipLaunchKernelGGL(dec3b_kernel<CLS>, dim3(blocks_for((long long)n * H2 * W2)), dim3(256), 0, s, a);
            return GS_OK;
        });
    } else {
        L.run(K_DEC3, px2 * (2 * ncls * 9 * ncls * 2) + px2 * (ncls * ncls * 4 * 2), [&] {
            Dec3Args a{};
            a.t = view(m->tt);
            a.wc = wb + m->wcc;
            a.bnc = wb + m->bncc;
            a.wup = wb + m->wup2;
            a.bnu = wb + m->bnu2;
            a.e = view(m->ee);
            a.N = n;
            a.classes = ncls;
            hipLaunchKernelGGL(dec3_kernel<CLS>, dim3(blocks_for((long long)n * H2 * W2)), dim3(256), 0, s, a);
            return GS_OK;
        });
    }
    m->set_stage("up_l2", m->ee, ncls);
    if constexpr (dec_tail_fused(CLS)) {
        L.run(K_DEC_TAIL, px1 * ((19 + CLS) * 9 * CLS * 2) + px1 * (CLS * CLS * 4 * 2), [&] {
            DecTailArgs a{};
            a.in = m->a0c.base;
            a.in_sn = m->a0c.sn;
            a.in_sc = m->a0c.sc;
            a.in_pitch = m->a0c.pitch;
            a.in_off = m->a0c.off;
            a.in_img_bytes = (unsigned)(m->a0c.sn * sizeof(float));
            a.wpack = wb + m->wtail;
            a.logits = r.logits;
            a.mask = r.mask;
            a.hist = ens_finishes((int)r.role) ? r.hist : nullptr;
            a.prob = r.prob;
            a.ens_mode = (int)r.role;
            a.ens_w = r.ens_w;
            if (r.logits) {
                a.ff = m->ff.base;
                a.ff_sn = m->ff.sn;
                a.ff_sc = m->ff.sc;
                a.ff_pitch = m->ff.pitch;
                a.ff_off = m->ff.off;
            }
            a.N = n;
            a.H1 = H1;
            a.W1 = W1;
            return launch_dec_tail(a, m->num_cus, s);
        });
        if (r.logits)
            m->set_stage("conv", m->ff, CLS);
    } else {
        L.run(K_DEC_CONV, px1 * ((19 + ncls) * 9 * ncls * 2), [&] {
            return launch_dec_conv<CLS>(m, plan.dec_conv, conv_args(m->a0c, wb + m->wconv, m->ff, nullptr, n), s);
        });
        m->set_stage("conv", m->ff, ncls);
        L.run(K_DEC4, px1 * (ncls * ncls * 4 * 2), [&] {
            Dec4Args a{};
            a.f = view(m->ff);
            a.wcl = wb + m->wclassifier;
            a.logits = r.logits;
            a.mask = r.mask;
            a.hist = r.hist;
            a.prob = r.prob;
            a.ens_mode = (int)r.role;
            a.ens_w = r.ens_w;
            a.N = n;
            a.classes = ncls;
            const dim3 grid(blocks_for(((long long)H1 * W1 + dec4_px<CLS>() - 1) / dec4_px<CLS>()), n);
            hipLaunchKernelGGL((r.role != EnsRole::NONE ? dec4_kernel<CLS, true> : dec4_kernel<CLS, false>), grid, dim3(256), 0, s, a);
            return GS_OK;
        });
    }
    return L.st;
}

static gs_status forward_any(Model *m, const ForwardReq &r)
{
    Launcher L{m, r.s, GS_OK, r.n};
    const ForwardPlan plan = plan_forward(r.n, r.H, r.W, m->p, m->q, m->cp, m->num_cus, no_vec());
    const Encoded e = encode(m, L, plan, r);
    switch (m->cp) {
    case 5: return decode<5>(m, L, plan, r, e);
    case 4: return decode<4>(m, L, plan, r, e);
    case 8: return decode<8>(m, L, plan, r, e);
    case 12: return decode<12>(m, L, plan, r, e);
    case 16: return decode<16>(m, L, plan, r, e);
    case 20: return decode<20>(m, L, plan, r, e);
    }
    set_error("internal: no decoder instantiation for %d padded classes", m->cp);
    return GS_ERR_UNSUPPORTED;
}

struct TileSlot : PipeSlot {
    Staging<uint8_t> in, out;
    Staging<unsigned long long> hist;
    void free_staging() { in.free(), out.free(), hist.free(); }
};

}

using namespace gs;

extern "C" {

const char *gs_last_error(void) { return g_err.c_str(); }
int gs_abi_version(void) { return 9; }
gs_status gs_device_fault_check(void)
{
    GS_HIP(hipDeviceSynchronize());
    int flags = 0;
    gs_status st = dec_tail_fault_flags(&flags);
    if (st != GS_OK) return st;
    if (flags) {
        set_error("device fault word %d: a decoder-tail wave gave up its strip-boundary exchange; the results of the calls since the last check are invalid", flags);
        return GS_ERR_DEVICE_FAULT;
    }
    return GS_OK;
}
int gs_build_flags(void)
{
#ifdef GS_DIAG
    return GS_BUILD_DIAG;
#else
    return 0;
#endif
}

struct gs_espnet {
    Model m;
    std::vector<std::unique_ptr<Model>> lanes;
    HostPipe<TileSlot, 4> tile_pipe;
    gs::CropPipe *crop_pipe = nullptr;
    Model &lane(int k) { return k == 0 ? m : *lanes[k - 1]; }
};

}

namespace gs {
CropPipe *&espnet_crop_pipe(gs_espnet *h) { return h->crop_pipe; }
int espnet_device(gs_espnet *h) { return h->m.device; }
int espnet_is_full_net(gs_espnet *h) { return h->m.encoder_only ? 0 : 1; }
int espnet_lanes(gs_espnet *h) { return 1 + (int)h->lanes.size(); }
int espnet_classes(gs_espnet *h) { return h->m.classes; }
static gs_status ensemble_scratch(gs_espnet *h, int lane, int n, int height, int width, float **prob)
{
    GS_REQUIRE(lane >= 0 && lane <= (int)h->lanes.size(), "lane %d does not exist (gs_espnet_set_lanes)", lane);
    Model &m0 = h->lane(lane);
    const gs_status st = grow(m0.prob, m0.prob_bytes, (size_t)n * m0.classes * height * width * sizeof(float), "ensemble scratch");
    *prob = m0.prob;
    return st;
}
gs_status espnet_forward(gs_espnet *h, int lane, const ForwardReq &r)
{
    GS_REQUIRE(h && r.in, "forward: null handle or input");
    GS_REQUIRE(lane >= 0 && lane <= (int)h->lanes.size(), "lane %d does not exist (gs_espnet_set_lanes)", lane);
    Model &m = h->lane(lane);
    GS_REQUIRE(!m.encoder_only || r.role == EnsRole::NONE, "an ESPNet-C handle cannot be an ensemble member");
    const gs_status st = layout_workspace(&m, r.n, r.H, r.W);
    return st != GS_OK ? st : forward_any(&m, r);
}

gs_status ensemble_kind(gs_espnet *const *models, int n_models, bool *enc_only)
{
    int n_enc = 0;
    for (int k = 0; k < n_models; ++k) {
        GS_REQUIRE(models[k], "ensemble member %d is null", k);
        n_enc += models[k]->m.encoder_only ? 1 : 0;
    }
    *enc_only = n_enc == n_models;
    for (int k = 0; k < n_models; ++k) {
        GS_REQUIRE(*enc_only || !models[k]->m.encoder_only, "ensemble member %d is not a full ESPNet", k);
        GS_REQUIRE(models[k]->m.classes == models[0]->m.classes, "ensemble member %d has %d classes, member 0 has %d", k,
                   models[k]->m.classes, models[0]->m.classes);
        for (int j = 0; *enc_only && j < k; ++j)
            GS_REQUIRE(models[j] != models[k], "ESPNet-C ensemble members %d and %d are the same handle", j, k);
    }
    if (*enc_only && n_models > GS_MAX_ENSEMBLE_C) {
        set_error("an ESPNet-C ensemble has at most %d members (got %d)", GS_MAX_ENSEMBLE_C, n_models);
        return GS_ERR_UNSUPPORTED;
    }
    return GS_OK;
}

static gs_status espnet_c_ensemble_head(gs_espnet *const *models, int n_models, int lane, const ForwardReq &r)
{
    EncHeadEnsArgs a{};
    for (int k = 0; k < n_models; ++k) {
        const Model &mk = models[k]->lane(lane);
        GS_REQUIRE(mk.encoder_only && mk.ws && r.n <= mk.ws_n && r.H == mk.ws_h && r.W == mk.ws_w,
                   "internal: member %d holds no 1/8-scale logits of this batch", k);
        a.logits[k] = mk.o2c.base;
    }
    a.mask = r.mask;
    a.hist = r.hist;
    a.classes = models[0]->m.classes;
    a.members = n_models;
    a.H3 = r.H / 8;
    a.W3 = r.W / 8;
    a.inv_members = 1.0f / (float)n_models;
    Model &m0 = models[0]->lane(lane);
    Launcher L{&m0, r.s, GS_OK, r.n};
    L.run(K_ENC_HEAD_ENS, (double)r.H * r.W * (a.classes * n_models * 20), [&] {
        launch_ens_head(a, r.n, r.s);
        return GS_OK;
    });
    return L.st;
}

gs_status run_ensemble(gs_espnet *const *models, int n_models, int lane, const ForwardReq &shared, const float *means,
                       const float *stds, const std::function<gs_status(int)> &prepare)
{
    const bool enc_only = models[0]->m.encoder_only;
    ForwardReq r = shared;
    r.ens_w = 1.0f / (float)n_models;
    gs_status st = GS_OK;
    if (!enc_only && (st = ensemble_scratch(models[0], lane, r.n, r.H, r.W, &r.prob)) != GS_OK) return st;
    for (int k = 0; k < n_models; ++k) {
        if (prepare && (st = prepare(k)) != GS_OK) return st;
        r.mean = means ? means + 3 * k : nullptr, r.stdv = stds ? stds + 3 * k : nullptr;
        if (enc_only)
            r.mask = nullptr, r.hist = k == 0 ? shared.hist : nullptr;
        else
            r.role = ens_role(k, n_models);
        st = espnet_forward(models[k], lane, r);
        if (st != GS_OK) return st;
    }
    return enc_only ? espnet_c_ensemble_head(models, n_models, lane, shared) : GS_OK;
}
}

extern "C" {

gs_status gs_espnet_create(const float *blob, const gs_layer_desc *table, int n_layers, int classes, int p, int q,
                           int encoder_only, gs_espnet **out)
{
    GS_REQUIRE(blob && table && out && n_layers > 0, "gs_espnet_create: null argument");
    GS_REQUIRE(p >= 0 && q >= 0, "gs_espnet_create: p and q must be non-negative");
    if (classes < 2 || classes > 20) {
        set_error("gs_espnet_create: classes must be 2..20 (got %d)", classes);
        return GS_ERR_UNSUPPORTED;
    }
    int ndev = 0;
    if (hipGetDeviceCount(&ndev) != hipSuccess || ndev == 0) {
        set_error("gs_espnet_create: no HIP device visible");
        return GS_ERR_NODEVICE;
    }
    std::unique_ptr<gs_espnet> h(new gs_espnet());
    Model &m = h->m;
    m.classes = classes;
    m.cp = padded_classes(classes);
    m.p = p;
    m.q = q;
    m.encoder_only = encoder_only != 0;
    GS_HIP(hipGetDevice(&m.device));
    hipDeviceProp_t prop;
    GS_HIP(hipGetDeviceProperties(&prop, m.device));
    if (std::strncmp(prop.gcnArchName, "gfx950", 6) != 0) {
        set_error("gs_espnet_create: device %d is %s; this library is built for gfx950 only", m.device, prop.gcnArchName);
        return GS_ERR_NODEVICE;
    }
    m.num_cus = prop.multiProcessorCount;
#ifdef GS_DIAG
    if (const char *v = std::getenv("GS_VARIANT"))
        m.variant = std::atoi(v);
#endif

    WeightTable t;
    t.blob = blob;
    for (int i = 0; i < n_layers; ++i)
        t.by_name[std::string(table[i].name)] = &table[i];
    const std::string e = m.encoder_only ? "" : "encoder.";
    const int c = classes;
    BlobBuilder bb;
    std::vector<float> tmp(3 * 256);

    const float *w;
    if (!(w = t.get(e + "level1.conv.weight", {16, 3, 3, 3}))) return GS_ERR_INVALID;
    m.w1 = bb.push(w, 432);
    if (!fold_bn(t, e + "level1.bn", e + "level1.act", 16, tmp.data())) return GS_ERR_INVALID;
    m.bn1 = bb.push(tmp.data(), 48);
    if (!fold_bn(t, e + "b1.bn", e + "b1.act", 19, tmp.data())) return GS_ERR_INVALID;
    m.b1 = bb.push(tmp.data(), 57);
    std::memcpy(m.stem_params, bb.data.data() + m.w1, sizeof(float) * 432);
    std::memcpy(m.stem_params + 432, bb.data.data() + m.bn1, sizeof(float) * 48);
    std::memcpy(m.stem_params + 480, bb.data.data() + m.b1, sizeof(float) * 57);
    std::vector<float> b2f(3 * 131);
    if (!fold_bn(t, e + "b2.bn", e + "b2.act", 131, b2f.data())) return GS_ERR_INVALID;
    m.b2 = bb.push(b2f.data(), 393);
    auto next2 = [&](int i) { return l2_c1_fused(i, p) ? e + "level2." + std::to_string(i) : std::string(); };
    auto next3 = [&](int i) { return l3_c1_fused(i, q) ? e + "level3." + std::to_string(i) : std::string(); };
    if (!pack_block(t, bb, e + "level2_0", true, 2, m.l2_0, nullptr, 0, 0, next2(0))) return GS_ERR_INVALID;
    m.l2.resize(p);
    for (int i = 0; i < p; ++i)
        if (!pack_block(t, bb, e + "level2." + std::to_string(i), false, 2, m.l2[i], i == p - 1 ? b2f.data() : nullptr, 0, 131, next2(i + 1)))
            return GS_ERR_INVALID;
    if (!pack_block(t, bb, e + "level3_0", true, 3, m.l3_0, nullptr, 0, 0, next3(0), b2f.data(), 64, 64, 131)) return GS_ERR_INVALID;
    m.l3.resize(q);
    for (int i = 0; i < q; ++i)
        if (!pack_block(t, bb, e + "level3." + std::to_string(i), false, 3, m.l3[i], nullptr, 0, 0, next3(i + 1))) return GS_ERR_INVALID;
    const int cp = m.cp;
    auto pad_deconv = [&](const float *src) {
        std::vector<float> o((size_t)cp * cp * 4, 0.0f);
        for (int i = 0; i < c; ++i)
            for (int o2 = 0; o2 < c; ++o2)
                for (int k = 0; k < 4; ++k)
                    o[((size_t)i * cp + o2) * 4 + k] = src[((size_t)i * c + o2) * 4 + k];
        return o;
    };
    auto pad_bn = [&](const float *src, int C, int rows, int cpn, const std::function<int(int)> &map) {
        std::vector<float> o((size_t)rows * cpn, 0.0f);
        for (int k = 0; k < cpn; ++k) {
            const int sc = map(k);
            for (int r = 0; r < rows; ++r)
                o[(size_t)r * cpn + k] = sc >= 0 ? src[(size_t)r * C + sc] : (r == 2 ? 1.0f : 0.0f);
        }
        return o;
    };
    auto ident = [&](int k) { return k < c ? k : -1; };
    if (!fold_bn(t, e + "b3.bn", e + "b3.act", 256, tmp.data())) return GS_ERR_INVALID;
    if (!(w = t.get(e + "classifier.conv.weight", {c, 256, 1, 1}))) return GS_ERR_INVALID;
    {
        const int rec = (3 + cp + 3) / 4 * 4;
        std::vector<float> pk((size_t)256 * rec, 0.0f);
        for (int ch = 0; ch < 256; ++ch) {
            for (int j = 0; j < 3; ++j) pk[(size_t)ch * rec + j] = tmp[j * 256 + ch];
            for (int k = 0; k < c; ++k) pk[(size_t)ch * rec + 3 + k] = w[k * 256 + ch];
        }
        m.b3 = bb.push(pk.data(), pk.size());
        m.wcls = m.b3;
    }
    if (!m.encoder_only) {
        if (!fold_bn(t, "br", "", c, tmp.data(), false)) return GS_ERR_INVALID;
        {
            const std::vector<float> v = pad_bn(tmp.data(), c, 2, cp, ident);
            m.br = bb.push(v.data(), v.size());
        }
        if (!(w = t.get("up_l3.0.weight", {c, c, 2, 2}))) return GS_ERR_INVALID;
        {
            const std::vector<float> v = pad_deconv(w);
            m.wup3 = bb.push(v.data(), v.size());
        }
        if (!(w = t.get("level3_C.conv.weight", {c, 131, 1, 1}))) return GS_ERR_INVALID;
        {
            const int rec = (cp + 3) / 4 * 4;
            std::vector<float> pk((size_t)131 * rec, 0.0f);
            for (int ch = 0; ch < 131; ++ch)
                for (int k = 0; k < c; ++k) pk[(size_t)ch * rec + k] = w[k * 131 + ch];
            m.w3c = bb.push(pk.data(), pk.size());
        }
        auto cat2 = [&](int k) { return k < cp ? (k < c ? k : -1) : (k - cp < c ? c + k - cp : -1); };
        if (!fold_bn(t, "combine_l2_l3.0.bn", "combine_l2_l3.0.act", 2 * c, tmp.data())) return GS_ERR_INVALID;
        {
            const std::vector<float> v = pad_bn(tmp.data(), 2 * c, 3, 2 * cp, cat2);
            m.cbr0 = bb.push(v.data(), v.size());
        }
        if (!(w = t.get("combine_l2_l3.1.conv.weight", {c, 2 * c, 3, 3}))) return GS_ERR_INVALID;
        {
            std::vector<float> v((size_t)cp * 2 * cp * 9, 0.0f);
            for (int k = 0; k < c; ++k)
                for (int ch = 0; ch < 2 * cp; ++ch) {
                    const int sc = cat2(ch);
                    if (sc < 0) continue;
                    for (int tap = 0; tap < 9; ++tap)
                        v[cp == 5 ? ((size_t)k * 2 * cp + ch) * 9 + tap : ((size_t)ch * 9 + tap) * cp + k] = w[((size_t)k * 2 * c + sc) * 9 + tap];
                }
            m.wcc = bb.push(v.data(), v.size());
        }
        if (dec3_on_mfma(cp)) {
            m.wcc_mfma = bb.reserve(conv_wfloats(2 * cp, 9, 1, cp, cp, true));
            float *dst = bb.data.data() + m.wcc_mfma;
            for (int tap = 0; tap < 9; ++tap)
                for (int ch = 0; ch < 2 * cp; ++ch) {
                    const int sc = cat2(ch);
                    if (sc < 0) continue;
                    for (int k = 0; k < c; ++k)
                        dst[((size_t)tap * 2 * cp + ch) * cp + k] = w[((size_t)k * 2 * c + sc) * 9 + tap];
                }
        }
        if (!fold_bn(t, "combine_l2_l3.1.bn", "combine_l2_l3.1.act", c, tmp.data())) return GS_ERR_INVALID;
        {
            const std::vector<float> v = pad_bn(tmp.data(), c, 3, cp, ident);
            m.bncc = bb.push(v.data(), v.size());
            if (m.wcc_mfma >= 0)
                std::memcpy(bb.data.data() + m.wcc_mfma + (size_t)9 * 2 * cp * cp, v.data(), sizeof(float) * 3 * cp);
        }
        if (!(w = t.get("up_l2.0.weight", {c, c, 2, 2}))) return GS_ERR_INVALID;
        {
            const std::vector<float> v = pad_deconv(w);
            m.wup2 = bb.push(v.data(), v.size());
        }
        if (!fold_bn(t, "up_l2.1.bn", "up_l2.1.act", c, tmp.data())) return GS_ERR_INVALID;
        {
            const std::vector<float> v = pad_bn(tmp.data(), c, 3, cp, ident);
            m.bnu2 = bb.push(v.data(), v.size());
        }
        if (!(w = t.get("conv.conv.weight", {c, 19 + c, 3, 3}))) return GS_ERR_INVALID;
        auto cat_ch = [&](int pl) { return pl < cp ? (pl < c ? pl : -1) : (pl - cp < 19 ? c + pl - cp : -1); };
        if (!fold_bn(t, "conv.bn", "conv.act", c, tmp.data())) return GS_ERR_INVALID;
        const std::vector<float> bn_conv = pad_bn(tmp.data(), c, 3, cp, ident);
        if (!dec_tail_fused(cp)) {
            const int cinp = (19 + cp + 3) / 4 * 4;
            m.wconv = bb.reserve(conv_wfloats(cinp, 9, 1, cp, cp, true));
            float *dst = bb.data.data() + m.wconv;
            for (int tap = 0; tap < 9; ++tap)
                for (int pl = 0; pl < cinp; ++pl) {
                    const int wch = cat_ch(pl);
                    if (wch < 0) continue;
                    for (int co = 0; co < c; ++co)
                        dst[((size_t)tap * cinp + pl) * cp + co] = w[((size_t)co * (19 + c) + wch) * 9 + tap];
                }
            std::memcpy(dst + (size_t)9 * cinp * cp, bn_conv.data(), sizeof(float) * 3 * cp);
        }
        if (!(w = t.get("classifier.weight", {c, c, 2, 2}))) return GS_ERR_INVALID;
        {
            const std::vector<float> v = pad_deconv(w);
            m.wclassifier = bb.push(v.data(), v.size());
        }
        if (dec_tail_fused(cp)) {
            const float *wc = t.get("conv.conv.weight", {c, 19 + c, 3, 3});
            if (!wc) return GS_ERR_INVALID;
            m.wtail = bb.reserve(DT_PACK_FLOATS);
            float *dt = bb.data.data() + m.wtail;
            for (int ty = 0; ty < 3; ++ty)
                for (int g = 0; g < 6; ++g)
                    for (int lane = 0; lane < 64; ++lane) {
                        const int rho = lane & 15, ch = 4 * g + (lane >> 4);
                        dt[(ty * 6 + g) * 64 + lane] =
                            rho < 3 * c ? wc[(((size_t)(rho % c) * (19 + c) + ch) * 3 + ty) * 3 + rho / c] : 0.0f;
                    }
            std::memcpy(dt + DT_A_FLOATS, bn_conv.data(), sizeof(float) * 3 * c);
            std::memcpy(dt + DT_A_FLOATS + 16, w, sizeof(float) * c * c * 4);
        }
    }
    bb.reserve(512);
    GS_HIP(hipMalloc(reinterpret_cast<void **>(&m.dblob), bb.data.size() * sizeof(float)));
    GS_HIP(hipMemcpy(m.dblob, bb.data.data(), bb.data.size() * sizeof(float), hipMemcpyHostToDevice));
    *out = h.release();
    return GS_OK;
}

static void free_lane(Model &l)
{
    for (auto &ev : l.events) {
        hipEventDestroy(ev.a);
        hipEventDestroy(ev.b);
    }
    if (l.ws) hipFree(l.ws);
    if (l.prob) hipFree(l.prob);
}

void gs_espnet_destroy(gs_espnet *h)
{
    if (!h)
        return;
    hipDeviceSynchronize();
    h->tile_pipe.destroy();
    crop_pipe_destroy(h->crop_pipe);
    for (int k = 0; k <= (int)h->lanes.size(); ++k)
        free_lane(h->lane(k));
    if (h->m.dblob) hipFree(h->m.dblob);
    delete h;
}

static gs_status check_shape(int n, int height, int width)
{
    GS_REQUIRE(n > 0, "batch size must be positive (got %d)", n);
    GS_REQUIRE(height >= 8 && width >= 8 && height % 8 == 0 && width % 8 == 0,
               "tile size must be a positive multiple of 8 in both dimensions (got %dx%d)", height, width);
    return GS_OK;
}

gs_status gs_espnet_reserve(gs_espnet *h, int n, int height, int width)
{
    GS_REQUIRE(h, "null handle");
    gs_status st = check_shape(n, height, width);
    if (st != GS_OK) return st;
    for (int k = 0; k <= (int)h->lanes.size(); ++k) {
        st = layout_workspace(&h->lane(k), n, height, width);
        if (st != GS_OK) return st;
    }
    return GS_OK;
}

gs_status gs_espnet_set_lanes(gs_espnet *h, int n_lanes)
{
    GS_REQUIRE(h, "null handle");
    GS_REQUIRE(n_lanes >= 1 && n_lanes <= 4, "gs_espnet_set_lanes: 1 to 4 lanes (got %d)", n_lanes);
    GS_HIP(hipDeviceSynchronize());
    while ((int)h->lanes.size() > n_lanes - 1) {
        free_lane(*h->lanes.back());
        h->lanes.pop_back();
    }
    while ((int)h->lanes.size() < n_lanes - 1) {
        std::unique_ptr<Model> l(new Model(h->m));
        l->ws = nullptr;
        l->ws_bytes = 0;
        l->ws_n = l->ws_h = l->ws_w = 0;
        l->prob = nullptr;
        l->prob_bytes = 0;
        l->stages.clear();
        l->events.clear();
        l->profile = false;
        h->lanes.push_back(std::move(l));
    }
    return GS_OK;
}

int gs_espnet_lanes(gs_espnet *h) { return h ? 1 + (int)h->lanes.size() : 0; }

gs_status gs_espnet_forward(gs_espnet *h, const void *in, int in_format, int n, int height, int width,
                            const float mean[3], const float std[3], float *logits, uint8_t *mask,
                            unsigned long long *hist, void *hip_stream)
{
    return gs_espnet_forward_lane(h, 0, in, in_format, n, height, width, mean, std, logits, mask, hist, hip_stream);
}

gs_status gs_espnet_forward_lane(gs_espnet *h, int lane, const void *in, int in_format, int n, int height, int width,
                                 const float mean[3], const float std[3], float *logits, uint8_t *mask,
                                 unsigned long long *hist, void *hip_stream)
{
    GS_REQUIRE(h && in, "gs_espnet_forward: null handle or input");
    GS_REQUIRE(lane >= 0 && lane <= (int)h->lanes.size(), "lane %d does not exist (gs_espnet_set_lanes)", lane);
    gs_status st = check_shape(n, height, width);
    if (st != GS_OK) return st;
    GS_REQUIRE(in_format == GS_IN_U8_BGR_NHWC || in_format == GS_IN_F32_NCHW, "unknown input format %d", in_format);
    GS_REQUIRE(in_format != GS_IN_U8_BGR_NHWC || (mean && std), "uint8 input needs mean and std");
    GS_REQUIRE(logits || mask, "nothing to compute: logits and mask are both NULL");
    GS_REQUIRE(!hist || mask, "hist requires the mask output");
    if (in_format == GS_IN_U8_BGR_NHWC)
        for (int i = 0; i < 3; ++i)
            GS_REQUIRE(std[i] != 0.0f, "std[%d] is zero", i);
    ForwardReq r;
    r.in = in, r.in_format = in_format, r.n = n, r.H = height, r.W = width;
    r.mean = mean, r.stdv = std, r.logits = logits, r.mask = mask, r.hist = hist, r.s = static_cast<hipStream_t>(hip_stream);
    return espnet_forward(h, lane, r);
}

gs_status gs_espnet_read_stage(gs_espnet *h, const char *stage, int image, float *dst, size_t cap, int dims[3])
{
    GS_REQUIRE(h && stage && dims, "gs_espnet_read_stage: null argument");
    Model &m = h->m;
    auto it = m.stages.find(stage);
    GS_REQUIRE(it != m.stages.end(), "stage '%s' was not produced by the last forward", stage);
    GS_REQUIRE(image >= 0 && image < m.last_n, "image index %d out of range", image);
    const Act &a = it->second.first;
    const int C = it->second.second;
    dims[0] = C;
    dims[1] = a.H;
    dims[2] = a.W;
    const size_t count = (size_t)C * a.H * a.W;
    if (!dst)
        return GS_OK;
    GS_REQUIRE(cap >= count, "destination too small for stage '%s'", stage);
    float *tmp = nullptr;
    GS_HIP(hipMalloc(reinterpret_cast<void **>(&tmp), count * sizeof(float)));
    hipLaunchKernelGGL(unpad_kernel, dim3(blocks_for((long long)count)), dim3(256), 0, 0, view(a), image, C, tmp);
    if (m.b2_lazy && std::string(stage) == "b2")
        hipLaunchKernelGGL(b2_apply_kernel, dim3(blocks_for((long long)64 * a.H * a.W)), dim3(256), 0, 0, tmp, m.dblob + m.b2, a.H * a.W, 64, 64);
    hipError_t e = hipMemcpy(dst, tmp, count * sizeof(float), hipMemcpyDeviceToHost);
    hipFree(tmp);
    GS_HIP(e);
    return GS_OK;
}

gs_status gs_espnet_block_forward(gs_espnet *h, int kind, int level, int index, const float *in, int height, int width,
                                  float *out)
{
    GS_REQUIRE(h && in && out, "gs_espnet_block_forward: null argument");
    GS_REQUIRE((kind == 0 || kind == 1) && (level == 2 || level == 3), "kind must be 0/1 and level 2/3");
    GS_REQUIRE(height >= 1 && width >= 1, "empty input");
    Model &m = h->m;
    GS_REQUIRE(kind == 1 || (index >= 0 && index < (level == 2 ? m.p : m.q)), "no ESP block %d at level %d", index, level);
    GS_REQUIRE(kind == 0 || (height % 2 == 0 && width % 2 == 0), "the down-sampler needs an even input size");
    const int up = kind == 0 ? (level == 2 ? 4 : 8) : (level == 2 ? 2 : 4);
    gs_status st = layout_workspace(&m, 1, height * up, width * up);
    if (st != GS_OK) return st;
    const float *wb = m.dblob;
    const Act &src = kind == 0 ? (level == 2 ? m.bb[0] : m.cc[0]) : (level == 2 ? m.a0 : m.a1);
    const Act &dst = level == 2 ? (kind == 0 ? m.bb[1] : m.bb[0]) : (kind == 0 ? m.cc[1] : m.cc[0]);
    const Act &red = level == 2 ? m.r2[0] : m.r3[0];
    const int cin = kind == 0 ? (level == 2 ? 64 : 128) : (level == 2 ? 19 : 131);
    const int cout = level == 2 ? 64 : 128;
    GS_REQUIRE(src.H == height && src.W == width, "internal: workspace level size mismatch");
    const size_t nin = (size_t)cin * height * width, nout = (size_t)cout * dst.H * dst.W;
    float *tmp = nullptr;
    GS_HIP(hipMalloc(reinterpret_cast<void **>(&tmp), (nin > nout ? nin : nout) * sizeof(float)));
    gs_status rc = GS_OK;
    hipStream_t s = nullptr;
    auto body = [&]() -> gs_status {
        GS_HIP(hipMemcpy(tmp, in, nin * sizeof(float), hipMemcpyHostToDevice));
        hipLaunchKernelGGL(pad_kernel, dim3(blocks_for((long long)nin)), dim3(256), 0, s, view(src), 0, cin, tmp);
        const PackedConv &pc = kind == 1 ? (level == 2 ? m.l2_0 : m.l3_0) : (level == 2 ? m.l2[index] : m.l3[index]);
        const ConvArgs rca = conv_args(src, wb + pc.c1, red, nullptr, 1);
        const ConvArgs bca = conv_args(red, wb + pc.br, dst, kind == 1 ? nullptr : &src, 1);
        gs_status r;
        if (level == 2) {
            r = kind == 1 ? launch_l2_reduce(&m, rca, s) : launch_l2_c1(&m, rca, s);
            if (r != GS_OK) return r;
            r = kind == 1 ? launch_l2_down(&m, unfused_l2_down(dst.W, no_vec()), bca, s)
                          : launch_l2_esp_fused(&m, unfused_l2_esp(dst.W, no_vec()), bca, s);
        } else {
            r = kind == 1 ? launch_l3_reduce(&m, form::l3_reduce::C1S, rca, s) : launch_l3_c1(&m, rca, s);
            if (r != GS_OK) return r;
            r = kind == 1 ? launch_l3_down(&m, unfused_l3_down(dst.W, no_vec()), bca, s)
                          : launch_l3_esp_last(&m, whole_row_l3_esp(dst.W, no_vec()), bca, s);
        }
        if (r != GS_OK) return r;
        hipLaunchKernelGGL(unpad_kernel, dim3(blocks_for((long long)nout)), dim3(256), 0, s, view(dst), 0, cout, tmp);
        GS_HIP(hipGetLastError());
        GS_HIP(hipMemcpy(out, tmp, nout * sizeof(float), hipMemcpyDeviceToHost));
        return GS_OK;
    };
    rc = body();
    hipFree(tmp);
    m.stages.clear();
    return rc;
}

gs_status gs_espnet_plan_forward(int n, int height, int width, int p, int q, int classes, int num_cus, int *out_forms, int cap,
                                 int *n_out)
{
    GS_REQUIRE(n_out, "gs_espnet_plan_forward: null argument");
    gs_status st = check_shape(n, height, width);
    if (st != GS_OK) return st;
    GS_REQUIRE(p >= 0 && q >= 0 && num_cus > 0, "gs_espnet_plan_forward: p and q must be non-negative, num_cus positive");
    if (classes < 2 || classes > 20) {
        set_error("gs_espnet_plan_forward: classes must be 2..20 (got %d)", classes);
        return GS_ERR_UNSUPPORTED;
    }
    *n_out = kLaunchClassCount;
    if (!out_forms)
        return GS_OK;
    GS_REQUIRE(cap >= kLaunchClassCount, "gs_espnet_plan_forward: %d entries needed, room for %d", kLaunchClassCount, cap);
    plan_forward(n, height, width, p, q, padded_classes(classes), num_cus, no_vec()).codes(out_forms);
    return GS_OK;
}

gs_status gs_espnet_form_info(int launch_class, int form, const char **name, int *pixels_per_lane)
{
    GS_REQUIRE(launch_class >= 0 && launch_class < kLaunchClassCount, "no launch class %d", launch_class);
    const LaunchClassInfo &c = kLaunchClasses[launch_class];
    GS_REQUIRE(form >= GS_FORM_NONE && form < c.n_forms, "launch class %s has no form %d", c.name, form);
    if (name) *name = form == GS_FORM_NONE ? c.name : c.forms[form].name;
    if (pixels_per_lane) *pixels_per_lane = form == GS_FORM_NONE ? 0 : c.forms[form].pixels_per_lane;
    return GS_OK;
}

gs_status gs_espnet_profile_enable(gs_espnet *h, int on)
{
    GS_REQUIRE(h, "null handle");
    h->m.profile = on != 0;
    return GS_OK;
}

gs_status gs_espnet_profile_read(gs_espnet *h, gs_kernel_time *out, int cap, int *n_out)
{
    GS_REQUIRE(h && n_out, "null argument");
    Model &m = h->m;
    for (auto &ev : m.events) {
        GS_HIP(hipEventSynchronize(ev.b));
        float ms = 0.0f;
        GS_HIP(hipEventElapsedTime(&ms, ev.a, ev.b));
        m.prof_ms[ev.k] += ms;
        m.prof_launches[ev.k] += 1;
        hipEventDestroy(ev.a);
        hipEventDestroy(ev.b);
    }
    m.events.clear();
    int k = 0;
    for (int i = 0; i < K_COUNT && out && k < cap; ++i) {
        if (!m.prof_launches[i])
            continue;
        std::snprintf(out[k].name, sizeof out[k].name, "%s", kKernelNames[i]);
        out[k].total_ms = m.prof_ms[i];
        out[k].launches = m.prof_launches[i];
        out[k].flops_per_tile = m.prof_flops[i] / (double)m.prof_launches[i];
        ++k;
    }
    *n_out = k;
    for (int i = 0; i < K_COUNT; ++i) {
        m.prof_ms[i] = 0;
        m.prof_launches[i] = 0;
        m.prof_flops[i] = 0;
    }
    return GS_OK;
}

gs_status gs_espnet_ensemble_forward(gs_espnet *const *models, int n_models, const void *in_u8, int n, int height,
                                     int width, const float *means, const float *stds, uint8_t *mask,
                                     unsigned long long *hist, void *hip_stream)
{
    GS_REQUIRE(models && n_models > 0 && in_u8 && means && stds && mask, "gs_espnet_ensemble_forward: null argument");
    gs_status st = check_shape(n, height, width);
    if (st != GS_OK) return st;
    bool enc_only = false;
    st = ensemble_kind(models, n_models, &enc_only);
    if (st != GS_OK) return st;
    for (int k = 0; k < n_models; ++k)
        for (int i = 0; i < 3; ++i)
            GS_REQUIRE(stds[3 * k + i] != 0.0f, "ensemble member %d: std[%d] is zero", k, i);
    ForwardReq r;
    r.in = in_u8, r.in_format = GS_IN_U8_BGR_NHWC, r.n = n, r.H = height, r.W = width;
    r.mask = mask, r.hist = hist, r.s = static_cast<hipStream_t>(hip_stream);
    return run_ensemble(models, n_models, 0, r, means, stds);
}

gs_status gs_espnet_segment_host(gs_espnet *h, const uint8_t *tiles, int n_tiles, int height, int width,
                                 const float mean[3], const float std[3], int batch, uint8_t *masks,
                                 unsigned long long *hist)
{
    GS_REQUIRE(h && tiles && masks && mean && std, "gs_espnet_segment_host: null argument");
    GS_REQUIRE(n_tiles > 0 && batch > 0, "n_tiles and batch must be positive");
    gs_status st = check_shape(batch, height, width);
    if (st != GS_OK) return st;
    if (batch > n_tiles) batch = n_tiles;
    const size_t in_b = (size_t)height * width * 3, out_b = (size_t)height * width;
    const size_t ncl = (size_t)h->m.classes;
    const int nl = h->lanes.empty() ? 1 : 2;
    const bool in_pinned = host_is_pinned(tiles), out_pinned = host_is_pinned(masks) && (!hist || host_is_pinned(hist));
    auto &pipe = h->tile_pipe;
    HipLatch fail;
    if (!pipe.ensure(2, true, fail, [&](TileSlot &s) {
            s.in.grow(in_b * batch, fail);
            s.out.grow(out_b * batch, fail);
            s.hist.grow(sizeof(unsigned long long) * GS_MAX_CLASSES * batch, fail);
        }))
        return fail.rc;
#ifdef GS_DIAG
    const bool ptrace = std::getenv("GS_PIPE_TRACE") != nullptr;
    const auto pt0 = std::chrono::steady_clock::now();
    auto stamp = [&](int bi, const char *what) {
        if (ptrace && bi < 12)
            std::fprintf(stderr, "pipe %2d %-10s %9.1f us\n", bi, what,
                         std::chrono::duration<double, std::micro>(std::chrono::steady_clock::now() - pt0).count());
    };
    const int pskip = std::getenv("GS_PIPE_SKIP") ? std::atoi(std::getenv("GS_PIPE_SKIP")) : 0;
#else
    auto stamp = [](int, const char *) {};
    constexpr int pskip = 0;
#endif
    const gs_status rc = pipe.run(
        (n_tiles + batch - 1) / batch, nl == 1, fail,
        [&](int bi, TileSlot &s, hipStream_t h2d) {
            s.first = bi * batch;
            s.count = n_tiles - s.first < batch ? n_tiles - s.first : batch;
            const uint8_t *src = tiles + (size_t)s.first * in_b;
            if (!in_pinned) {
                parallel_memcpy(s.in.h, src, in_b * s.count);
                src = s.in.h;
            }
            if (!(pskip & 1) || bi < pipe.NSLOT)
                fail(hipMemcpyAsync(s.in.d, src, in_b * s.count, hipMemcpyHostToDevice, h2d), "H2D copy");
        },
        [&](int bi, TileSlot &s, hipStream_t compute) {
            return gs_espnet_forward_lane(h, bi % nl, s.in.d, GS_IN_U8_BGR_NHWC, s.count, height, width, mean, std, nullptr, s.out.d,
                                          s.hist.d, compute);
        },
        [&](int, TileSlot &s, hipStream_t compute) {
            uint8_t *hdst = out_pinned ? masks + (size_t)s.first * out_b : s.out.h;
            unsigned long long *hhdst = (out_pinned && hist) ? hist + (size_t)s.first * ncl : s.hist.h;
            const size_t hb = sizeof(unsigned long long) * ncl * s.count;
            if (!(pskip & 2))
                fail(hipMemcpy2DAsync(hdst, out_b, s.out.d, out_b, out_b, s.count, hipMemcpyDeviceToHost, compute), "D2H copy");
            if (hist || !out_pinned)
                fail(hipMemcpy2DAsync(hhdst, hb, s.hist.d, hb, hb, 1, hipMemcpyDeviceToHost, compute), "D2H copy");
        },
        [&](TileSlot &s) {
            if (out_pinned)
                return;
            parallel_memcpy(masks + (size_t)s.first * out_b, s.out.h, out_b * s.count);
            if (hist) std::memcpy(hist + (size_t)s.first * ncl, s.hist.h, sizeof(unsigned long long) * ncl * s.count);
        },
        stamp);
    return rc != GS_OK ? rc : gs_device_fault_check();
}

}
```

### glomeruli_segmentation_amd/csrc/espnet_kernels.h

```cpp
#pragma once
#include <type_traits>
#include "gs_internal.h"

namespace gs {

struct ActV {
    float *base;
    long long sn;
    int sc, pitch, off;
    int H, W;
};
static inline ActV view(const Act &a) { return ActV{a.base, a.sn, a.sc, a.pitch, a.off, a.H, a.W}; }

__device__ __forceinline__ float *at(const ActV &t, int n, int c, int y, int x)
{
    return t.base + (long long)n * t.sn + (long long)c * t.sc + t.off + y * t.pitch + x;
}
__device__ __forceinline__ float ldz(const ActV &t, int n, int c, int y, int x)
{
    const bool ok = (unsigned)y < (unsigned)t.H && (unsigned)x < (unsigned)t.W;
    const int yc = min(max(y, 0), t.H - 1), xc = min(max(x, 0), t.W - 1);
    const float v = *at(t, n, c, yc, xc);
    return ok ? v : 0.0f;
}
// ... 267 lines not shown
#pragma unroll
        for (int k = 0; k < CLS; ++k)
            s[k] = k < ncls ? s[k] : 0.0f;
    }
}
template <int CLS>
constexpr int dec1_record() { return (3 + CLS + 3) / 4 * 4; }
template <int CLS>
constexpr int dec2_record() { return (CLS + 3) / 4 * 4; }

struct Dec1Args {
    ActV c0, clast;
    const float *b3w;
    const float *br;
    const float *wup;
    ActV out;
    float *enc_logits;
    int N;
    int classes;
};

template <int CLS, int CB>
__global__ void __launch_bounds__(256) dec1_kernel(const Dec1Args a)
{
    const int H3 = a.c0.H, W3 = a.c0.W;
    __shared__ float part[3][CLS][64];
    const int lane = threadIdx.x & 63, w = __builtin_amdgcn_readfirstlane(threadIdx.x >> 6);
    const long long total = (long long)a.N * H3 * W3;
    long long idx = (long long)blockIdx.x * 64 + lane;
    const bool active = idx < total;
    if (!active)
        idx = total - 1;
    const int x = (int)(idx % W3);
    const int y = (int)((idx / W3) % H3);
    const int n = (int)(idx / ((long long)W3 * H3));
    float s[CLS];
#pragma unroll
    for (int k = 0; k < CLS; ++k)
        s[k] = 0.0f;
    const long long pix = (long long)n * a.c0.sn + a.c0.off + y * a.c0.pitch + x;
    const float *plane0 = (w < 2 ? a.c0.base : a.clast.base) + pix + (long long)((w & 1) * 64) * a.c0.sc;
    auto fetch = [&](int c0, float *dst) {
#pragma unroll
        for (int j = 0; j < CB; ++j)
            dst[j] = ld_stream<NT_DEC1_LD>(plane0 + (long long)(c0 + j) * a.c0.sc);
    };
    float cur[CB], nxt[CB];
    fetch(0, cur);
    for (int c0 = 0; c0 < 64; c0 += CB) {
        if (c0 + CB < 64)
            fetch(c0 + CB, nxt);
        __builtin_amdgcn_sched_barrier(0);
#pragma unroll
        for (int j = 0; j < CB; ++j) {
            const float *pc = a.b3w + (w * 64 + c0 + j) * dec1_record<CLS>();
            const float t = cur[j] * pc[0] + pc[1];
            const float v = prelu(t, pc[2]);
#pragma unroll
            for (int k = 0; k < CLS; ++k)
                s[k] = fmaf(pc[3 + k], v, s[k]);
        }
#pragma unroll
        for (int j = 0; j < CB; ++j)
            cur[j] = nxt[j];
    }
    if (w > 0) {
#pragma unroll
        for (int k = 0; k < CLS; ++k)
            part[w - 1][k][lane] = s[k];
    }
    __syncthreads();
    if (w > 0 || !active)
        return;
#pragma unroll
    for (int k = 0; k < CLS; ++k)
        s[k] = (s[k] + part[0][k][lane]) + (part[1][k][lane] + part[2][k][lane]);
    const int ncls = real_classes<CLS>(a.classes);
    if (a.enc_logits) {
#pragma unroll
        for (int k = 0; k < CLS; ++k)
            if (k < ncls)
                a.enc_logits[(((long long)n * ncls + k) * H3 + y) * W3 + x] = s[k];
        return;
    }
#pragma unroll
    for (int k = 0; k < CLS; ++k)
        s[k] = s[k] * a.br[k] + a.br[CLS + k];
    zero_padding_lanes<CLS>(s, ncls);
    if constexpr (CLS != 5) {
        for (int o = 0; o < ncls; ++o) {
            float t[4] = {0.0f, 0.0f, 0.0f, 0.0f};
#pragma unroll
            for (int i = 0; i < CLS; ++i)
#pragma unroll
                for (int k = 0; k < 4; ++k)
                    t[k] = fmaf(s[i], a.wup[(i * CLS + o) * 4 + k], t[k]);
            *reinterpret_cast<float2 *>(at(a.out, n, o, 2 * y, 2 * x)) = make_float2(t[0], t[1]);
            *reinterpret_cast<float2 *>(at(a.out, n, o, 2 * y + 1, 2 * x)) = make_float2(t[2], t[3]);
        }
        return;
    }
    float up[CLS][2][2];
#pragma unroll
    for (int o = 0; o < CLS; ++o)
#pragma unroll
        for (int dy = 0; dy < 2; ++dy)
#pragma unroll
            for (int dx = 0; dx < 2; ++dx) {
                float t = 0.0f;
#pragma unroll
                for (int i = 0; i < CLS; ++i)
                    t = fmaf(s[i], a.wup[((i * CLS + o) * 2 + dy) * 2 + dx], t);
                up[o][dy][dx] = t;
            }
#pragma unroll
    for (int o = 0; o < CLS; ++o)
#pragma unroll
        for (int dy = 0; dy < 2; ++dy)
            *reinterpret_cast<float2 *>(at(a.out, n, o, 2 * y + dy, 2 * x)) = make_float2(up[o][dy][0], up[o][dy][1]);
}

struct Dec2Args {
    ActV a1;
    ActV raw;
    const float *b2;
    int raw_c0, raw_cn;
    ActV o2c;
    const float *w3c;
    const float *br;
    ActV t;
    int N;
    int classes;
};

template <int CLS>
__global__ void __launch_bounds__(256) dec2_kernel(const Dec2Args a)
{
    const int H2 = a.a1.H, W2 = a.a1.W;
    __shared__ float part[3][CLS][64];
    const int lane = threadIdx.x & 63, w = __builtin_amdgcn_readfirstlane(threadIdx.x >> 6);
    const long long total = (long long)a.N * H2 * W2;
    long long idx = (long long)blockIdx.x * 64 + lane;
    const bool active = idx < total;
    if (!active)
        idx = total - 1;
    const int x = (int)(idx % W2);
    const int y = (int)((idx / W2) % H2);
    const int n = (int)(idx / ((long long)W2 * H2));
    float s[CLS];
#pragma unroll
    for (int k = 0; k < CLS; ++k)
        s[k] = 0.0f;
    const int cb = 32 * w;
#if defined(GS_DIAG) && defined(DEC2_X_NOCAT)
    if (w == 0) {
#pragma unroll
        for (int k = 0; k < CLS; ++k)
            s[k] = ld_stream<NT_DEC2_LD>(at(a.a1, n, k, y, x));
    }
    if (false)
#endif
    if (cb >= a.raw_c0 && cb < a.raw_c0 + a.raw_cn) {
#pragma unroll 16
        for (int c = cb; c < cb + 32; ++c) {
            const float v = bn_prelu(ld_stream<NT_DEC2_LD>(at(a.raw, n, c - a.raw_c0, y, x)), a.b2, 131, c);
            const float *pc = a.w3c + c * dec2_record<CLS>();
#pragma unroll
            for (int k = 0; k < CLS; ++k)
                s[k] = fmaf(pc[k], v, s[k]);
        }
    } else {
#pragma unroll 16
        for (int c = cb; c < cb + 32; ++c) {
            const float v = ld_stream<NT_DEC2_LD>(at(a.a1, n, c, y, x));
            const float *pc = a.w3c + c * dec2_record<CLS>();
#pragma unroll
            for (int k = 0; k < CLS; ++k)
                s[k] = fmaf(pc[k], v, s[k]);
        }
    }
#if defined(GS_DIAG) && defined(DEC2_X_NOCAT)
    if (false)
#endif
    if (w == 3) {
#pragma unroll
        for (int c = 128; c < 131; ++c) {
            const float v = ld_stream<NT_DEC2_LD>(at(a.a1, n, c, y, x));
            const float *pc = a.w3c + c * dec2_record<CLS>();
#pragma unroll
            for (int k = 0; k < CLS; ++k)
                s[k] = fmaf(pc[k], v, s[k]);
        }
    }
    if (w > 0) {
#pragma unroll
        for (int k = 0; k < CLS; ++k)
            part[w - 1][k][lane] = s[k];
    }
    __syncthreads();
    if (w > 0 || !active)
        return;
#pragma unroll
    for (int k = 0; k < CLS; ++k)
        s[k] = (s[k] + part[0][k][lane]) + (part[1][k][lane] + part[2][k][lane]);
    float tv[2 * CLS];
#pragma unroll
    for (int k = 0; k < CLS; ++k) {
        tv[k] = bn_prelu(s[k], a.br, 2 * CLS, k);
        tv[CLS + k] = bn_prelu(*at(a.o2c, n, k, y, x), a.br, 2 * CLS, CLS + k);
    }
    const int ncls = real_classes<CLS>(a.classes);
#pragma unroll
    for (int k = 0; k < 2 * CLS; ++k)
        if (k % CLS < ncls)
            *at(a.t, n, k, y, x) = tv[k];
}

struct Dec3Args {
    ActV t;
    const float *wc;
    const float *bnc;
    const float *wup;
    const float *bnu;
    ActV e;
    int N;
    int classes;
};

template <int CLS>
__global__ void __launch_bounds__(256) dec3_kernel(const Dec3Args a)
{
    const int H2 = a.t.H, W2 = a.t.W;
    const long long idx = (long long)blockIdx.x * 256 + threadIdx.x;
    if (idx >= (long long)a.N * H2 * W2)
        return;
    const int x = (int)(idx % W2);
    const int y = (int)((idx / W2) % H2);
    const int n = (int)(idx / ((long long)W2 * H2));
    float s[CLS];
#pragma unroll
    for (int k = 0; k < CLS; ++k)
        s[k] = 0.0f;
    const int ncls = real_classes<CLS>(a.classes);
    for (int c = 0; c < 2 * CLS; ++c) {
        if (CLS != 5 && c % CLS >= ncls)
            continue;
#pragma unroll
        for (int ky = 0; ky < 3; ++ky)
#pragma unroll
            for (int kx = 0; kx < 3; ++kx) {
                const float v = ldz(a.t, n, c, y - 1 + ky, x - 1 + kx);
#pragma unroll
                for (int k = 0; k < CLS; ++k)
                    s[k] = fmaf(CLS == 5 ? a.wc[((k * 2 * CLS + c) * 3 + ky) * 3 + kx] : a.wc[((c * 3 + ky) * 3 + kx) * CLS + k], v, s[k]);
            }
    }
#pragma unroll
    for (int k = 0; k < CLS; ++k)
        s[k] = bn_prelu(s[k], a.bnc, CLS, k);
    zero_padding_lanes<CLS>(s, ncls);
    float up[CLS][2][2];
#pragma unroll
    for (int o = 0; o < CLS; ++o)
#pragma unroll
        for (int dy = 0; dy < 2; ++dy)
#pragma unroll
            for (int dx = 0; dx < 2; ++dx) {
                float t = 0.0f;
#pragma unroll
                for (int i = 0; i < CLS; ++i)
                    t = fmaf(s[i], a.wup[((i * CLS + o) * 2 + dy) * 2 + dx], t);
                up[o][dy][dx] = bn_prelu(t, a.bnu, CLS, o);
            }
#pragma unroll
    for (int o = 0; o < CLS; ++o)
#pragma unroll
        for (int dy = 0; dy < 2; ++dy)
            if (o < ncls)
                *reinterpret_cast<float2 *>(at(a.e, n, o, 2 * y + dy, 2 * x)) = make_float2(up[o][dy][0], up[o][dy][1]);
}

template <int CLS>
__global__ void __launch_bounds__(256) dec3b_kernel(const Dec3Args a)
{
    const int H2 = a.t.H, W2 = a.t.W;
    const long long idx = (long long)blockIdx.x * 256 + threadIdx.x;
    if (idx >= (long long)a.N * H2 * W2)
        return;
    const int x = (int)(idx % W2);
    const int y = (int)((idx / W2) % H2);
    const int n = (int)(idx / ((long long)W2 * H2));
    const int ncls = real_classes<CLS>(a.classes);
    float s[CLS];
#pragma unroll
    for (int k = 0; k < CLS; ++k)
        s[k] = *at(a.t, n, k, y, x);
    zero_padding_lanes<CLS>(s, ncls);
    for (int o = 0; o < ncls; ++o) {
        float t[4] = {0.0f, 0.0f, 0.0f, 0.0f};
#pragma unroll
        for (int i = 0; i < CLS; ++i)
#pragma unroll
            for (int k = 0; k < 4; ++k)
                t[k] = fmaf(s[i], a.wup[(i * CLS + o) * 4 + k], t[k]);
#pragma unroll
        for (int k = 0; k < 4; ++k)
            t[k] = bn_prelu(t[k], a.bnu, CLS, o);
        *reinterpret_cast<float2 *>(at(a.e, n, o, 2 * y, 2 * x)) = make_float2(t[0], t[1]);
        *reinterpret_cast<float2 *>(at(a.e, n, o, 2 * y + 1, 2 * x)) = make_float2(t[2], t[3]);
    }
}

struct Dec4Args {
    ActV f;
    const float *wcl;
    float *logits;
    unsigned char *mask;
    unsigned long long *hist;
    float *prob;
    int ens_mode;
    float ens_w;
    int N;
    int classes;
};

template <int CLS>
constexpr int dec4_px() { return CLS <= 8 ? 4 : CLS <= 12 ? 2 : 1; }
template <int CLS, bool ENS>
__global__ void __launch_bounds__(256) dec4_kernel(const Dec4Args a)
{
    __shared__ unsigned int lhist[CLS];
    const int H1 = a.f.H, W1 = a.f.W;
    const int H = 2 * H1, W = 2 * W1;
    const int n = blockIdx.y;
    const int ncls = real_classes<CLS>(a.classes);
    constexpr int DEC4_PX = dec4_px<CLS>();
    __shared__ float wl[CLS * CLS * 4];
    for (int i = threadIdx.x; i < CLS * CLS * 4; i += 256)
        wl[i] = a.wcl[i];
    if (threadIdx.x < CLS)
        lhist[threadIdx.x] = 0;
    __syncthreads();
    int cls_of[DEC4_PX][4];
    float s[DEC4_PX][CLS];
    bool live[DEC4_PX];
    int xs[DEC4_PX], ys[DEC4_PX];
#pragma unroll
    for (int q = 0; q < DEC4_PX; ++q) {
        const int idx = (blockIdx.x * DEC4_PX + q) * 256 + threadIdx.x;
        live[q] = idx < H1 * W1;
        const int ic = live[q] ? idx : 0;
        xs[q] = ic % W1;
        ys[q] = ic / W1;
#pragma unroll
        for (int k = 0; k < CLS; ++k)
            s[q][k] = *at(a.f, n, k, ys[q], xs[q]);
        zero_padding_lanes<CLS>(s[q], ncls);
    }
#pragma unroll
    for (int q = 0; q < DEC4_PX; ++q) {
        const int x = xs[q], y = ys[q];
#pragma unroll
        for (int dy = 0; dy < 2; ++dy) {
            unsigned char m[2];
#pragma unroll
            for (int dx = 0; dx < 2; ++dx) {
                float best = 0.0f;
                int bi = 0;
// ... 109 lines not shown
```

### glomeruli_segmentation_amd/csrc/forward_plan.h

```cpp
#pragma once
#include "espnet_config.h"

namespace gs {

constexpr int cfg_pixels(int, int, int, int, int, int, int, int, int p, int) { return p; }

constexpr int padded_classes(int classes) { return classes == 5 ? 5 : (classes + 3) / 4 * 4; }
constexpr bool b2_is_lazy(int p) { return p > 0; }
constexpr bool l2_c1_fused(int i, int p) { return CFG_FUSE_L2 && i < p; }
constexpr bool l3_c1_fused(int i, int q) { return (CFG_FUSE_L3 == 2 || (CFG_FUSE_L3 == 1 && i == 0)) && i < q; }
constexpr bool dec3_on_mfma(int cp) { return cp >= 12; }
constexpr bool dec_tail_fused(int cp) { return cp == 5; }
constexpr int dec_mt(int cp) { return cp <= 16 ? 16 : 32; }
constexpr int dec_pixels(int cp) { return cp <= 16 ? 8 : 4; }

#define GS_FORMS_L2_DOWN(X)                              \
    X(P2S_VEC, "CFG_L2_BR_P2S+F_VEC", cfg_pixels(CFG_L2_BR_P2S))                                  \
    X(P4S_VEC_SKIP, "CFG_L2_BR_P4S+F_VEC+F_SKIP_PAD", cfg_pixels(CFG_L2_BR_P4S))                  \
    X(P4_VEC, "CFG_L2_BR_P4+F_VEC", cfg_pixels(CFG_L2_BR_P4))                                     \
    X(P4, "CFG_L2_BR_P4", 0)                                                                      \
    X(UNFUSED_P4_VEC, "unfused CFG_L2_BR_P4+F_VEC", cfg_pixels(CFG_L2_BR_P4))                     \
    X(UNFUSED_P4, "unfused CFG_L2_BR_P4", 0)
#define GS_FORMS_L2_ESP_FUSED(X)                        \
    X(P2S_VEC, "CFG_L2_BR_P2S+F_VEC", cfg_pixels(CFG_L2_BR_P2S))                                  \
    X(P4_VEC, "CFG_L2_BR_P4+F_VEC", cfg_pixels(CFG_L2_BR_P4))                                     \
    X(P4, "CFG_L2_BR_P4", 0)                                                                      \
    X(UNFUSED_P4_VEC, "unfused CFG_L2_BR_P4+F_VEC", cfg_pixels(CFG_L2_BR_P4))                     \
    X(UNFUSED_P4, "unfused CFG_L2_BR_P4", 0)
#define GS_FORMS_L2_ESP_LAST(X)             \
    X(P2S_VEC, "CFG_L2_BR_P2S+F_VEC", cfg_pixels(CFG_L2_BR_P2S))                                  \
    X(P4_VEC, "CFG_L2_BR_P4+F_VEC", cfg_pixels(CFG_L2_BR_P4))                                     \
    X(P4, "CFG_L2_BR_P4", 0)
#define GS_FORMS_CAT_B2(X)                            \
    X(KERNEL, "cat_b2_kernel", 0)
#define GS_FORMS_L3_REDUCE(X)                                    \
    X(BNL_P1, "CFG_L3_C1S_BNL_P1", 0)                                                             \
    X(BNL, "CFG_L3_C1S_BNL", 0)                                                                   \
    X(C1S, "CFG_L3_C1S", 0)
#define GS_FORMS_L3_DOWN(X)                              \
    X(P1R, "CFG_L3_BR_P1R", 0)                                                                    \
    X(P2R_VEC, "CFG_L3_BR_P2R+F_VEC", cfg_pixels(CFG_L3_BR_P2R))                                  \
    X(BR_VEC, "CFG_L3_BR+F_VEC", cfg_pixels(CFG_L3_BR))                                           \
    X(P2F, "CFG_L3_BR_P2F", 0)                                                                    \
    X(UNFUSED_BR_VEC, "unfused CFG_L3_BR+F_VEC", cfg_pixels(CFG_L3_BR))                           \
    X(UNFUSED_BR, "unfused CFG_L3_BR", 0)
#define GS_FORMS_L3_ESP_FUSED(X)    \
    X(P1R, "CFG_L3_BR_P1R", 0)                                                                    \
    X(P2R_VEC, "CFG_L3_BR_P2R+F_VEC", cfg_pixels(CFG_L3_BR_P2R))                                  \
    X(P2F, "CFG_L3_BR_P2F", 0)
#define GS_FORMS_L3_ESP_LAST(X)                      \
    X(P1R, "CFG_L3_BR_P1R", 0)                                                                    \
    X(P2R_VEC, "CFG_L3_BR_P2R+F_VEC", cfg_pixels(CFG_L3_BR_P2R))                                  \
    X(BR_VEC, "CFG_L3_BR+F_VEC", cfg_pixels(CFG_L3_BR))                                           \
    X(P2, "CFG_L3_BR_P2", 0)
#define GS_FORMS_DEC3(X)                                     \
    X(KERNEL, "dec3_kernel", 0)                                                                   \
    X(MT16, "MFMA MT16", 0)                                                                       \
    X(MT16_VEC, "MFMA MT16+F_VEC", dec_pixels(16))                                                \
    X(MT32, "MFMA MT32", 0)                                                                       \
    X(MT32_VEC, "MFMA MT32+F_VEC", dec_pixels(20))
#define GS_FORMS_DEC_CONV(X)                           \
    X(TAIL, "dec_tail_kernel", 0)                                                                 \
    X(MT16, "MFMA MT16", 0)                                                                       \
    X(MT16_VEC, "MFMA MT16+F_VEC", dec_pixels(16))                                                \
    X(MT32, "MFMA MT32", 0)                                                                       \
    X(MT32_VEC, "MFMA MT32+F_VEC", dec_pixels(20))
#define GS_LAUNCH_CLASSES(C)               \
    C(l2_down, GS_FORMS_L2_DOWN)           \
    C(l2_esp_fused, GS_FORMS_L2_ESP_FUSED) \
    C(l2_esp_last, GS_FORMS_L2_ESP_LAST)   \
    C(cat_b2, GS_FORMS_CAT_B2)             \
    C(l3_reduce, GS_FORMS_L3_REDUCE)       \
    C(l3_down, GS_FORMS_L3_DOWN)           \
    C(l3_esp_fused, GS_FORMS_L3_ESP_FUSED) \
    C(l3_esp_last, GS_FORMS_L3_ESP_LAST)   \
    C(dec3, GS_FORMS_DEC3)                 \
    C(dec_conv, GS_FORMS_DEC_CONV)

struct FormInfo {
    const char *name;
    int pixels_per_lane;
};
struct LaunchClassInfo {
    const char *name;
    const FormInfo *forms;
    int n_forms;
};

#define GS_FORM_ID(id, name, ppl) id,
#define GS_FORM_INFO(id, name, ppl) {name, ppl},
#define GS_CLASS_ENUM(cls, FORMS) enum class cls : int { none = -1, FORMS(GS_FORM_ID) };
#define GS_CLASS_FORMS(cls, FORMS)                                          \
    constexpr FormInfo kForms_##cls[] = {FORMS(GS_FORM_INFO)};              \
    constexpr int pixels_per_lane(form::cls f) { return kForms_##cls[(int)f].pixels_per_lane; }
#define GS_CLASS_INFO(cls, FORMS) {#cls, kForms_##cls, (int)(sizeof kForms_##cls / sizeof kForms_##cls[0])},
#define GS_PLAN_MEMBER(cls, FORMS) form::cls cls = form::cls::none;
#define GS_PLAN_CODE(cls, FORMS) *out++ = (int)cls;
namespace form {
GS_LAUNCH_CLASSES(GS_CLASS_ENUM)
}
GS_LAUNCH_CLASSES(GS_CLASS_FORMS)
constexpr LaunchClassInfo kLaunchClasses[] = {GS_LAUNCH_CLASSES(GS_CLASS_INFO)};
constexpr int kLaunchClassCount = (int)(sizeof kLaunchClasses / sizeof kLaunchClasses[0]);

struct ForwardPlan {
    GS_LAUNCH_CLASSES(GS_PLAN_MEMBER)
    bool lazy_b2 = false;
    void codes(int *out) const { GS_LAUNCH_CLASSES(GS_PLAN_CODE) }
};
#undef GS_FORM_ID
#undef GS_FORM_INFO
#undef GS_CLASS_ENUM
#undef GS_CLASS_FORMS
#undef GS_CLASS_INFO
#undef GS_PLAN_MEMBER
#undef GS_PLAN_CODE

template <typename F>
constexpr bool vec_fits(F v, int w, bool no_vec)
{
    return !no_vec && w % pixels_per_lane(v) == 0;
}

constexpr form::l2_down unfused_l2_down(int W2, bool no_vec)
{
    return vec_fits(form::l2_down::UNFUSED_P4_VEC, W2, no_vec) ? form::l2_down::UNFUSED_P4_VEC : form::l2_down::UNFUSED_P4;
}
constexpr form::l2_esp_fused unfused_l2_esp(int W2, bool no_vec)
{
    return vec_fits(form::l2_esp_fused::UNFUSED_P4_VEC, W2, no_vec) ? form::l2_esp_fused::UNFUSED_P4_VEC : form::l2_esp_fused::UNFUSED_P4;
}
constexpr form::l3_down unfused_l3_down(int W3, bool no_vec)
{
    return vec_fits(form::l3_down::UNFUSED_BR_VEC, W3, no_vec) ? form::l3_down::UNFUSED_BR_VEC : form::l3_down::UNFUSED_BR;
}
constexpr form::l3_esp_last whole_row_l3_esp(int W3, bool no_vec)
{
    return vec_fits(form::l3_esp_last::BR_VEC, W3, no_vec) ? form::l3_esp_last::BR_VEC : form::l3_esp_last::P2;
}

inline ForwardPlan plan_forward(int n, int H, int W, int p, int q, int cp, int num_cus, bool no_vec)
{
    namespace f = form;
    const int W1 = W / 2, H2 = H / 4, W2 = W / 4, H3 = H / 8, W3 = W / 8;
    const long long cus = num_cus;
    ForwardPlan pl;
    pl.lazy_b2 = b2_is_lazy(p);

    const bool small2 = CFG_SMALL2_WAVES > 0 && (long long)n * H2 * cdiv(W2, 64) * 2 <= cus * CFG_SMALL2_WAVES &&
                        vec_fits(f::l2_down::P2S_VEC, W2, no_vec);
    if (!l2_c1_fused(0, p))
        pl.l2_down = unfused_l2_down(W2, no_vec);
    else if (small2)
        pl.l2_down = f::l2_down::P2S_VEC;
    else if (CFG_L2_DOWN_SKIP && vec_fits(f::l2_down::P4S_VEC_SKIP, W2, no_vec))
        pl.l2_down = f::l2_down::P4S_VEC_SKIP;
    else
        pl.l2_down = vec_fits(f::l2_down::P4_VEC, W2, no_vec) ? f::l2_down::P4_VEC : f::l2_down::P4;
    if (p > 1) {
        if (!l2_c1_fused(1, p))
            pl.l2_esp_fused = unfused_l2_esp(W2, no_vec);
        else if (small2)
            pl.l2_esp_fused = f::l2_esp_fused::P2S_VEC;
        else
            pl.l2_esp_fused = vec_fits(f::l2_esp_fused::P4_VEC, W2, no_vec) ? f::l2_esp_fused::P4_VEC : f::l2_esp_fused::P4;
    }
    if (p > 0)
        pl.l2_esp_last = small2                                            ? f::l2_esp_last::P2S_VEC
                         : vec_fits(f::l2_esp_last::P4_VEC, W2, no_vec) ? f::l2_esp_last::P4_VEC
                                                                          : f::l2_esp_last::P4;
    if (!pl.lazy_b2)
        pl.cat_b2 = f::cat_b2::KERNEL;

    if (!pl.lazy_b2)
        pl.l3_reduce = f::l3_reduce::C1S;
    else
        pl.l3_reduce = (long long)n * H3 * cdiv(W3, 128) * 4 <= cus * 8 ? f::l3_reduce::BNL_P1 : f::l3_reduce::BNL;
    const bool small3 = (long long)n * H3 * cdiv(W3, 64) * 2 <= cus * CFG_SMALL3_WAVES && !no_vec;
    if (!l3_c1_fused(0, q))
        pl.l3_down = unfused_l3_down(W3, no_vec);
    else if (small3)
        pl.l3_down = f::l3_down::P1R;
    else if (CFG_L3_DOWN_P2 && vec_fits(f::l3_down::P2R_VEC, W3, no_vec))
        pl.l3_down = f::l3_down::P2R_VEC;
    else
        pl.l3_down = vec_fits(f::l3_down::BR_VEC, W3, no_vec) ? f::l3_down::BR_VEC : f::l3_down::P2F;
    if (q > 1 && l3_c1_fused(1, q))
        pl.l3_esp_fused = small3                                              ? f::l3_esp_fused::P1R
                          : vec_fits(f::l3_esp_fused::P2R_VEC, W3, no_vec) ? f::l3_esp_fused::P2R_VEC
                                                                             : f::l3_esp_fused::P2F;
    if (q > 0) {
        if (small3)
            pl.l3_esp_last = f::l3_esp_last::P1R;
        else if (CFG_L3_LAST_P2 && vec_fits(f::l3_esp_last::P2R_VEC, W3, no_vec))
            pl.l3_esp_last = f::l3_esp_last::P2R_VEC;
        else
            pl.l3_esp_last = whole_row_l3_esp(W3, no_vec);
    }

    if (!dec3_on_mfma(cp))
        pl.dec3 = f::dec3::KERNEL;
    else if (dec_mt(cp) == 16)
        pl.dec3 = vec_fits(f::dec3::MT16_VEC, W2, no_vec) ? f::dec3::MT16_VEC : f::dec3::MT16;
    else
        pl.dec3 = vec_fits(f::dec3::MT32_VEC, W2, no_vec) ? f::dec3::MT32_VEC : f::dec3::MT32;
    if (dec_tail_fused(cp))
        pl.dec_conv = f::dec_conv::TAIL;
    else if (dec_mt(cp) == 16)
        pl.dec_conv = vec_fits(f::dec_conv::MT16_VEC, W1, no_vec) ? f::dec_conv::MT16_VEC : f::dec_conv::MT16;
    else
        pl.dec_conv = vec_fits(f::dec_conv::MT32_VEC, W1, no_vec) ? f::dec_conv::MT32_VEC : f::dec_conv::MT32;
    return pl;
}

}
```

### glomeruli_segmentation_amd/engine.py

```python
import ctypes
import functools

import numpy as np
import torch

from . import _lib


def _to_numpy(v):
    if isinstance(v, torch.Tensor):
        return v.detach().cpu().numpy()
    return np.asarray(v)


def pack_state_dict(state_dict):
    items = []
    total = 0
    for name, v in state_dict.items():
        a = _to_numpy(v)
        if a.dtype.kind != "f":
            continue
        a = np.ascontiguousarray(a, dtype=np.float32)
        if a.ndim > 4:
            raise ValueError("tensor %s has %d dims" % (name, a.ndim))
# ... 98 lines not shown
        out = torch.empty((n, self.classes, oh, ow), dtype=torch.float32, device=x.device)
        with torch.cuda.device(x.device):
            _lib.check(self.lib.gs_espnet_forward(self.handle, x.data_ptr(), _lib.GS_IN_F32_NCHW, n, h, w, None, None,
                                                  out.data_ptr(), None, None, _stream_ptr(x.device)))
        return out

    def segment(self, tiles_u8, mean, std, want_logits=False, want_hist=True, out_mask=None, out_hist=None, lane=None,
                want_enc_logits=False):
        if tiles_u8.dtype != torch.uint8 or tiles_u8.dim() != 4 or tiles_u8.shape[3] != 3 or not tiles_u8.is_cuda:
            raise ValueError("expected a uint8 [N,H,W,3] tensor on the GPU")
        if want_enc_logits and not self.encoder_only:
            raise ValueError("want_enc_logits: the 1/8-scale logits are an output of ESPNet-C engines only")
        if want_logits and self.encoder_only:
            raise ValueError("want_logits: an ESPNet-C engine has no full-resolution logits (want_enc_logits=True gives the 1/8-scale ones)")
        want_logits = bool(want_logits or want_enc_logits)
        tiles_u8 = tiles_u8.contiguous()
        n, h, w, _ = tiles_u8.shape
        dev = tiles_u8.device
        _check_out(out_mask, "out_mask", (n, h, w), torch.uint8, dev)
        _check_out(out_hist, "out_hist", (n, self.classes), torch.int64, dev)
        mask = out_mask if out_mask is not None else torch.empty((n, h, w), dtype=torch.uint8, device=dev)
        hist = None
        if want_hist:
            hist = out_hist if out_hist is not None else torch.empty((n, self.classes), dtype=torch.int64, device=dev)
        lh, lw = (h // 8, w // 8) if self.encoder_only else (h, w)
        logits = torch.empty((n, self.classes, lh, lw), dtype=torch.float32, device=dev) if want_logits else None
        with torch.cuda.device(dev):
            if lane is None:
                if 0 in self._lane_streams:
                    torch.cuda.current_stream(dev).wait_stream(self._lane_streams[0])
                k, sp = 0, _stream_ptr(dev)
            else:
                st = self.lane_stream(lane)
                st.wait_stream(torch.cuda.current_stream(dev))
                for t in (tiles_u8, mask, hist, logits):
                    if t is not None:
                        t.record_stream(st)
                k, sp = lane, ctypes.c_void_p(st.cuda_stream)
            _lib.check(self.lib.gs_espnet_forward_lane(
                self.handle, k, tiles_u8.data_ptr(), _lib.GS_IN_U8_BGR_NHWC, n, h, w, _lib.fptr3(mean), _lib.fptr3(std),
                logits.data_ptr() if want_logits else None, mask.data_ptr(),
                hist.data_ptr() if want_hist else None, sp))
        return mask, hist, logits

    def segment_host(self, tiles, mean, std, batch=32, want_hist=True, out_masks=None, out_hist=None):
        self.quiesce()
        if isinstance(tiles, torch.Tensor):
            if tiles.is_cuda or tiles.dtype != torch.uint8 or not tiles.is_contiguous():
                raise ValueError("expected a contiguous uint8 CPU tensor")
            t, h, w, _ = tiles.shape
            in_ptr = ctypes.c_void_p(tiles.data_ptr())
            pin = tiles.is_pinned()
            _check_out(out_masks, "out_masks", (t, h, w), torch.uint8, torch.device("cpu"))
            _check_out(out_hist, "out_hist", (t, self.classes), torch.int64, torch.device("cpu"))
            masks_t = out_masks if out_masks is not None else torch.empty((t, h, w), dtype=torch.uint8, pin_memory=pin)
            hist_t = None
            if want_hist:
                hist_t = out_hist if out_hist is not None else torch.zeros((t, self.classes), dtype=torch.int64, pin_memory=pin)
            with torch.cuda.device(self.device):
                _lib.check(self.lib.gs_espnet_segment_host(
                    self.handle, in_ptr, t, h, w, _lib.fptr3(mean), _lib.fptr3(std), batch, ctypes.c_void_p(masks_t.data_ptr()),
                    ctypes.c_void_p(hist_t.data_ptr()) if want_hist else None))
            return masks_t.numpy(), (hist_t.numpy() if want_hist else None)
        tiles = np.ascontiguousarray(tiles, dtype=np.uint8)
        t, h, w, _ = tiles.shape
        masks = np.empty((t, h, w), dtype=np.uint8)
        hist = np.zeros((t, self.classes), dtype=np.uint64) if want_hist else None
        with torch.cuda.device(self.device):
            _lib.check(self.lib.gs_espnet_segment_host(
                self.handle, tiles.ctypes.data_as(ctypes.c_void_p), t, h, w, _lib.fptr3(mean), _lib.fptr3(std), batch,
                masks.ctypes.data_as(ctypes.c_void_p), hist.ctypes.data_as(ctypes.c_void_p) if want_hist else None))
        return masks, (hist.astype(np.int64) if want_hist else None)

    scores_crops = True

    def segment_crops(self, crops, mean, std, net_h=512, net_w=1024, batch=32, **kw):
        return segment_crops_host([self], [(mean, std)], crops, net_h, net_w, batch, **kw)

    def segment_crops_resident(self, packed_in, descs, mean, std, net_h=512, net_w=1024, want_net_maps=True, want_hist=True,
                               packed_out=None, paste=None, lane=None):
        n = len(descs)
        dev = packed_in.device
        tab = (_lib.CropDesc * n)(*descs)
        net = torch.empty((n, net_h, net_w), dtype=torch.uint8, device=dev) if want_net_maps else None
        hist = torch.empty((n, self.classes), dtype=torch.int64, device=dev) if want_hist else None
        with torch.cuda.device(dev):
            if lane is None:
                if 0 in self._lane_streams:
                    torch.cuda.current_stream(dev).wait_stream(self._lane_streams[0])
                k, sp = 0, _stream_ptr(dev)
            else:
                st = self.lane_stream(lane)
                st.wait_stream(torch.cuda.current_stream(dev))
                for t in (packed_in, packed_out, net, hist):
                    if t is not None:
                        t.record_stream(st)
                k, sp = lane, ctypes.c_void_p(st.cuda_stream)
            _lib.check(self.lib.gs_espnet_segment_crops(
                self.handle, k, packed_in.data_ptr(), tab, n, _lib.fptr3(mean), _lib.fptr3(std), net_h, net_w,
                net.data_ptr() if net is not None else None, packed_out.data_ptr() if packed_out is not None else None,
                hist.data_ptr() if hist is not None else None, ctypes.byref(paste) if paste is not None else None, sp))
        return net, hist

    def read_stage(self, name, image=0):
        dims = (ctypes.c_int * 3)()
        _lib.check(self.lib.gs_espnet_read_stage(self.handle, name.encode(), image, None, 0, ctypes.byref(dims)))
        out = np.empty(tuple(dims), dtype=np.float32)
        with torch.cuda.device(self.device):
            _lib.check(self.lib.gs_espnet_read_stage(self.handle, name.encode(), image,
                                                     out.ctypes.data_as(ctypes.c_void_p), out.size, ctypes.byref(dims)))
        return out

    def block_forward(self, kind, level, index, x):
        x = np.ascontiguousarray(x, dtype=np.float32)
        c, h, w = x.shape
        cout = 64 if level == 2 else 128
        out = np.empty((cout, h, w) if kind == 0 else (cout, h // 2, w // 2), dtype=np.float32)
        with torch.cuda.device(self.device):
            _lib.check(self.lib.gs_espnet_block_forward(self.handle, kind, level, index, x.ctypes.data_as(ctypes.c_void_p),
                                                        h, w, out.ctypes.data_as(ctypes.c_void_p)))
        return out

    def profile(self, on):
        _lib.check(self.lib.gs_espnet_profile_enable(self.handle, 1 if on else 0))

    def profile_read(self):
        arr = (_lib.KernelTime * 32)()
        n = ctypes.c_int()
        with torch.cuda.device(self.device):
            _lib.check(self.lib.gs_espnet_profile_read(self.handle, arr, 32, ctypes.byref(n)))
        return [{"name": arr[i].name.decode(), "total_ms": arr[i].total_ms, "launches": arr[i].launches,
                 "flops_per_tile": arr[i].flops_per_tile} for i in range(n.value)]


@functools.lru_cache(maxsize=None)
def forward_forms():
    lib = _lib.load()
    table = []
    name, ppl = ctypes.c_char_p(), ctypes.c_int()
    while lib.gs_espnet_form_info(len(table), _lib.GS_FORM_NONE, ctypes.byref(name), ctypes.byref(ppl)) == _lib.GS_OK:
        k, cls, forms = len(table), name.value.decode(), []
        while lib.gs_espnet_form_info(k, len(forms), ctypes.byref(name), ctypes.byref(ppl)) == _lib.GS_OK:
            forms.append((name.value.decode(), ppl.value))
        table.append((cls, tuple(forms)))
    return tuple(table)


def plan_forward(n, height, width, p, q, classes, num_cus):
    lib = _lib.load()
    table = forward_forms()
    codes, count = (ctypes.c_int * len(table))(), ctypes.c_int()
    _lib.check(lib.gs_espnet_plan_forward(n, height, width, p, q, classes, num_cus, codes, len(table), ctypes.byref(count)))
    return {cls: forms[codes[k]][0] for k, (cls, forms) in enumerate(table) if codes[k] != _lib.GS_FORM_NONE}


def crop_preprocess(crop_u8, mean, std, out_h, out_w, out=None):
    lib = _lib.load()
    crop_u8 = crop_u8.contiguous()
    h, w, _ = crop_u8.shape
    if out is None:
        out = torch.empty((3, out_h, out_w), dtype=torch.float32, device=crop_u8.device)
    with torch.cuda.device(crop_u8.device):
        _lib.check(lib.gs_crop_preprocess(crop_u8.data_ptr(), h, w, _lib.fptr3(mean), _lib.fptr3(std), out_h, out_w,
                                          out.data_ptr(), _stream_ptr(crop_u8.device)))
    return out


def mask_resize_nearest(mask, out_h, out_w):
    lib = _lib.load()
    mask = mask.contiguous()
    h, w = mask.shape
    out = torch.empty((out_h, out_w), dtype=torch.uint8, device=mask.device)
    with torch.cuda.device(mask.device):
        _lib.check(lib.gs_mask_resize_nearest(mask.data_ptr(), h, w, out_h, out_w, out.data_ptr(), _stream_ptr(mask.device)))
    return out


def paste_target(slide_map, ds=8, luts=None):
    if slide_map.dtype != torch.uint8 or slide_map.dim() != 2 or not slide_map.is_cuda or not slide_map.is_contiguous():
        raise ValueError("slide_map must be a contiguous uint8 [map_h,map_w] tensor on the GPU")
    t = _lib.PasteTarget()
    t.slide_map = slide_map.data_ptr()
    t.map_h, t.map_w, t.ds = int(slide_map.shape[0]), int(slide_map.shape[1]), int(ds)
    t.sx_lut = luts[0].data_ptr() if luts is not None else None
    t.sy_lut = luts[1].data_ptr() if luts is not None else None
    return t


def seen_values(seen_words):
    bits = np.unpackbits(np.ascontiguousarray(seen_words, dtype="<u8").view(np.uint8), bitorder="little")
    return np.nonzero(bits)[0].astype(np.uint8)


def score_crops_resident(net_masks, packed_labels, descs, classes, want_seen=True):
    lib = _lib.load()
    n, net_h, net_w = (int(v) for v in net_masks.shape)
    if n != len(descs):
        raise ValueError("%d masks for %d descriptors" % (n, len(descs)))
    if net_masks.dtype != torch.uint8 or packed_labels.dtype != torch.uint8 or not net_masks.is_contiguous() or not packed_labels.is_contiguous():
        raise ValueError("expected contiguous uint8 GPU tensors")
    need = max(int(d.out_off) + int(d.h) * int(d.w) for d in descs)
    if packed_labels.numel() < need:
        raise ValueError("packed_labels holds %d bytes, the descriptors reach %d" % (packed_labels.numel(), need))
    dev = net_masks.device
    tab = (_lib.CropDesc * n)(*descs)
    conf = torch.empty((n, classes, classes), dtype=torch.int64, device=dev)
    seen = torch.empty((n, 4), dtype=torch.int64, device=dev) if want_seen else None
    with torch.cuda.device(dev):
        _lib.check(lib.gs_espnet_score_crops(net_masks.data_ptr(), packed_labels.data_ptr(), tab, n, net_h, net_w, classes,
                                             conf.data_ptr(), seen.data_ptr() if seen is not None else None, _stream_ptr(dev)))
    return conf, seen


def segment_crops_host(engines, mean_stds, crops, net_h=512, net_w=1024, batch=32, want_masks=True, want_net_maps=False,
                       want_hist=True, paste=None, origins=None, overlay=None, labels=None, want_gt_overlay=False):
    lib = _lib.load()
    n = len(crops)
    if labels is not None and len(labels) != n:
        raise ValueError("%d labels for %d crops" % (len(labels), n))
    if want_gt_overlay and (labels is None or overlay is None):
        raise ValueError("want_gt_overlay needs labels and overlay")
    if n == 0:
        return {"masks": [] if want_masks else None, "net_maps": None, "counts": None, "overlays": [] if overlay is not None else None,
                "conf": None, "seen": [] if labels is not None else None, "gt_overlays": [] if want_gt_overlay else None}
    keep = []
    ptrs = (ctypes.c_void_p * n)()
    hs, ws = (ctypes.c_int * n)(), (ctypes.c_int * n)()
    for i, c in enumerate(crops):
        if isinstance(c, torch.Tensor):
            if c.is_cuda or c.dtype != torch.uint8 or c.dim() != 3 or c.shape[2] != 3 or not c.is_contiguous():
                raise ValueError("crop %d: expected a contiguous uint8 [h,w,3] CPU tensor" % i)
            ptrs[i] = c.data_ptr()
        else:
            c = np.ascontiguousarray(c, dtype=np.uint8)
            if c.ndim != 3 or c.shape[2] != 3:
                raise ValueError("crop %d: expected uint8 [h,w,3]" % i)
            ptrs[i] = c.ctypes.data
        keep.append(c)
        hs[i], ws[i] = int(c.shape[0]), int(c.shape[1])
    eng0 = engines[0]
    handles = (ctypes.c_void_p * len(engines))(*[e.handle for e in engines])
    means = (ctypes.c_float * (3 * len(engines)))(*[float(v) for ms in mean_stds for v in ms[0]])
    stds = (ctypes.c_float * (3 * len(engines)))(*[float(v) for ms in mean_stds for v in ms[1]])
    out_ptrs, out_buf, offs = None, None, None
    if want_masks:
        sizes = [int(hs[i]) * int(ws[i]) for i in range(n)]
        offs = np.zeros(n + 1, dtype=np.int64)
        np.cumsum([(s + 255) // 256 * 256 for s in sizes], out=offs[1:])
        out_buf = torch.empty(int(offs[-1]), dtype=torch.uint8, pin_memory=True)
        base = out_buf.data_ptr()
        out_ptrs = (ctypes.c_void_p * n)(*[base + int(offs[i]) for i in range(n)])
    net = torch.empty((n, net_h, net_w), dtype=torch.uint8, pin_memory=True) if want_net_maps else None
    hist = torch.zeros((n, eng0.classes), dtype=torch.int64, pin_memory=True) if want_hist else None
    x1 = y1 = None
    if paste is not None:
        if origins is None or len(origins) != n:
            raise ValueError("paste needs one (x1, y1) level-0 origin per crop")
        x1 = (ctypes.c_int * n)(*[int(o[0]) for o in origins])
        y1 = (ctypes.c_int * n)(*[int(o[1]) for o in origins])
    ov, ov_buf, ov_offs, pal = None, None, None, None
    if overlay is not None:
        palette, wa, wb = overlay
        pal = np.ascontiguousarray(palette, dtype=np.uint8).reshape(-1, 3)
        ov_offs = np.zeros(n + 1, dtype=np.int64)
        np.cumsum([(int(hs[i]) * int(ws[i]) * 3 + 255) // 256 * 256 for i in range(n)], out=ov_offs[1:])
        ov_buf = torch.empty(int(ov_offs[-1]), dtype=torch.uint8, pin_memory=True)
        ov = _lib.CropOverlay()
        ov.palette_rgb = pal.ctypes.data
        ov.n_colours = int(pal.shape[0])
        ov.wa, ov.wb = float(wa), float(wb)
        ov_ptrs = (ctypes.c_void_p * n)(*[ov_buf.data_ptr() + int(ov_offs[i]) for i in range(n)])
        ov.out_bgr = ctypes.cast(ov_ptrs, ctypes.POINTER(ctypes.c_void_p))
        keep.append(ov_ptrs)
    sc, conf, seen, gt_buf = None, None, None, None
    if labels is not None:
        lab_ptrs = (ctypes.c_void_p * n)()
        for i, lb in enumerate(labels):
            if not isinstance(lb, np.ndarray) or lb.dtype != np.uint8 or lb.shape != (int(hs[i]), int(ws[i])):
                raise ValueError("label %d: expected a uint8 [%d,%d] array" % (i, int(hs[i]), int(ws[i])))
            lb = np.ascontiguousarray(lb)
            keep.append(lb)
            lab_ptrs[i] = lb.ctypes.data
        conf = np.zeros((n, eng0.classes, eng0.classes), dtype=np.uint64)
        seen = np.zeros((n, 4), dtype=np.uint64)
        sc = _lib.CropScoring()
        sc.labels = ctypes.cast(lab_ptrs, ctypes.POINTER(ctypes.c_void_p))
        sc.conf, sc.seen = conf.ctypes.data, seen.ctypes.data
        sc.gt_clamp = 1
        keep.append(lab_ptrs)
        if want_gt_overlay:
            gt_buf = torch.empty(int(ov_offs[-1]), dtype=torch.uint8, pin_memory=True)
            gt_ptrs = (ctypes.c_void_p * n)(*[gt_buf.data_ptr() + int(ov_offs[i]) for i in range(n)])
            sc.gt_overlay_bgr = ctypes.cast(gt_ptrs, ctypes.POINTER(ctypes.c_void_p))
            keep.append(gt_ptrs)
    for e in engines:
        e.quiesce()
    args = (handles, len(engines), ptrs, hs, ws, n, means, stds, net_h, net_w, batch, out_ptrs,
            ctypes.c_void_p(net.data_ptr()) if net is not None else None,
            ctypes.c_void_p(hist.data_ptr()) if hist is not None else None,
            ctypes.byref(paste) if paste is not None else None, x1, y1, ctypes.byref(ov) if ov is not None else None)
    with torch.cuda.device(eng0.device):
        if sc is None:
            _lib.check(lib.gs_espnet_segment_crops_host(*args))
        else:
            _lib.check(lib.gs_espnet_segment_crops_host_scored(*args, ctypes.byref(sc)))
    masks = None
# ... 32 lines not shown
```

Measured before the change: 11470 patches/s.

## Fuse level3_C 1x1 class projection into stride-2 level-3 reduce kernel

```diff
diff --git a/glomeruli_segmentation_amd/_lib.py b/glomeruli_segmentation_amd/_lib.py
--- a/glomeruli_segmentation_amd/_lib.py
+++ b/glomeruli_segmentation_amd/_lib.py
@@ -139,6 +139,11 @@
     "gs_espnet_segment_crops_host_scored": (_I, PROTOTYPES["gs_espnet_segment_crops_host"][1] + [ctypes.POINTER(CropScoring)]),
 }
 
+PLAN_PROTOTYPES = {
+    "gs_espnet_plan_flags": (_I, [_I, _I, _I, _I, _I, _I, _I, _I, ctypes.POINTER(_I)]),
+}
+GS_PLAN_LAZY_B2, GS_PLAN_L3C_IN_REDUCE = 1, 2
+
 _lib = None
 
 
@@ -151,7 +156,9 @@
             "%s is missing: build it with `python -m glomeruli_segmentation_amd.build` "
             "(hipcc --offload-arch=gfx950).  There is no CPU fallback." % LIB_PATH)
     lib = ctypes.CDLL(LIB_PATH, mode=ctypes.RTLD_GLOBAL)
-    for name, (res, args) in list(PROTOTYPES.items()) + list(SCORING_PROTOTYPES.items()):
+    for name, (res, args) in list(PROTOTYPES.items()) + list(SCORING_PROTOTYPES.items()) + list(PLAN_PROTOTYPES.items()):
+        if name in PLAN_PROTOTYPES and not hasattr(lib, name):
+            continue
         fn = getattr(lib, name)
         fn.restype = res
         fn.argtypes = args
diff --git a/glomeruli_segmentation_amd/build.py b/glomeruli_segmentation_amd/build.py
--- a/glomeruli_segmentation_amd/build.py
+++ b/glomeruli_segmentation_amd/build.py
@@ -8,7 +8,8 @@
 LIB = os.path.join(PKG, "libglomseg.so")
 SOURCES = ["espnet.hip", "dec_tail.hip", "crops.hip", "detect_ops.hip", "detector.hip", "wsi_eval.hip", "contours.cpp"]
 HEADERS = ["gs_internal.h", "conv_mfma.h", "dec_tail.h", "dec_tail_args.h", "espnet_kernels.h", "crop_sample.h", "crop_plan.h", "detect_math.h", "detect_plan.h", "host_copy.h", "host_jobs.h", "host_pipe.h",
-           os.path.join("..", "..", "include", "glomseg.h"), os.path.join("..", "..", "include", "glomseg_scoring.h")]
+           os.path.join("..", "..", "include", "glomseg.h"), os.path.join("..", "..", "include", "glomseg_scoring.h"),
+           os.path.join("..", "..", "include", "glomseg_plan.h")]
 FLAGS = ["-O3", "--offload-arch=gfx950", "-std=c++17", "-fPIC", "-Wall", "-Wno-unused-result",
          "-Wno-unused-value"]
 
diff --git a/glomeruli_segmentation_amd/csrc/conv_mfma.h b/glomeruli_segmentation_amd/csrc/conv_mfma.h
--- a/glomeruli_segmentation_amd/csrc/conv_mfma.h
+++ b/glomeruli_segmentation_amd/csrc/conv_mfma.h
@@ -71,6 +71,10 @@
     int out3_sc, out3_pitch, out3_off, nout3;
     unsigned out3_img_bytes;
     int bnl_s0, bnl_s1;
+    float *side;
+    long long side_sn;
+    int side_sc, side_pitch, side_off;
+    unsigned side_img_bytes;
     int stagger;
     int prio_mode;
     unsigned long long *stamp;
@@ -153,6 +157,12 @@
 constexpr int F_S2_FLIP = 1048576;
 constexpr int F_SKIP_PAD = 4194304;
 constexpr int F_BNLOAD = 8388608;
+constexpr int F_SIDE_SHIFT = 27;
+constexpr int F_SIDE1X1(int classes) { return classes << F_SIDE_SHIFT; }
+constexpr int SIDE_REC = 8;
+constexpr int SIDE_ZROWS = 16;
+constexpr int side_table_floats(int CINP) { return (CINP + SIDE_ZROWS) * SIDE_REC; }
+constexpr int side_table_offset(int image_total, int CINP, int KL) { return image_total + (3 * (CINP + KL) + 3) / 4 * 4; }
 constexpr int F_X_NOLOAD = 16;
 constexpr int F_X_NOLDS = 32;
 constexpr int F_X_NOEPI = 64;
@@ -206,6 +216,11 @@
     constexpr bool S2FLIP = FLAGS & F_S2_FLIP;
     constexpr bool SKIP = FLAGS & F_SKIP_PAD;
     constexpr bool BNL = FLAGS & F_BNLOAD;
+    constexpr int SCLS = (FLAGS >> F_SIDE_SHIFT) & 15;
+    constexpr bool SIDE = SCLS > 0;
+    static_assert(!SIDE || ((FLAGS & F_S2PAIR) && TAPS == 9 && STRIDE == 2 && MT == 32 && NDIL == 1 && SCLS <= SIDE_REC &&
+                            (CINP / M_KL_OF(MT)) % G == 0 && G * M_KL_OF(MT) <= SIDE_ZROWS && !(FLAGS & (F_A_GLOBAL | F_VEC | F_X_ALL))),
+                  "F_SIDE1X1 is for the stride-2 3x3 reduce on 32-pixel runs, a tap row in whole chunks");
     static_assert(!BNL || ((FLAGS & F_S2PAIR) && !(FLAGS & (F_BNACT | F_A_GLOBAL | F_VEC))), "F_BNLOAD is for the plain stride-2 reduce");
     static_assert(!SKIP || (TAPS == 9 && STRIDE == 1 && !(FLAGS & F_S2PAIR) && G * M_KL_OF(MT) == CINP),
                   "F_SKIP_PAD: unit-stride 3x3 with one tap row per chunk");
@@ -250,6 +265,7 @@
     const float *tab = bnp + BNFL;
     constexpr int BNL_C = CINP + M::KL;
     const float *bnl = lds + (conv_image(CINP, TAPS, NDIL, NOUT1, NOUT, BNACT, DUAL, FUSE ? M::NACC : 0).total - LDS_SRC0);
+    const float *sidew = lds + side_table_offset(conv_image(CINP, TAPS, NDIL, NOUT1, NOUT, BNACT, DUAL, FUSE ? M::NACC : 0).total, CINP, M::KL);
     const __amdgpu_buffer_rsrc_t rsrc_w =
         __builtin_amdgcn_make_buffer_rsrc(const_cast<float *>(a.wpack), 0, AGL ? WFL * 4 : 0, 0x00020000);
 
@@ -463,6 +479,10 @@
             dst = zero ? 0.0f : v;
         };
 
+        float side[SIDE ? P : 1][SIDE ? SCLS : 1][2], sw[SIDE ? SCLS : 1];
+        const __amdgpu_buffer_rsrc_t rside = __builtin_amdgcn_make_buffer_rsrc(
+            SIDE ? a.side + (long long)n * a.side_sn : a.out, 0, SIDE ? a.side_img_bytes : 0u, 0x00020000);
+
         if (task == t0) {
 #pragma unroll
             for (int g = 0; g < G; ++g) {
@@ -627,6 +647,22 @@
                 for (int p = 0; p < P; ++p)
                     acc[p] = (typename M::acc_t)(0.0f);
             }
+            constexpr int CPR = SIDE ? NSTEP / G : 1;
+            int side_ty = 0;
+            if (SIDE) {
+                int ty0c, sidxc;
+                decode_rg(c, 0, ty0c, sidxc);
+                side_ty = flip ? TYN - 1 - ty0c : ty0c;
+                if (c % CPR == 0) {
+#pragma unroll
+                    for (int p = 0; p < P; ++p)
+#pragma unroll
+                        for (int k = 0; k < SCLS; ++k)
+                            side[p][k][0] = side[p][k][1] = 0.0f;
+                }
+            }
+            const bool side_row = SIDE && side_ty >= 1;
+            const float *side_wrow = sidew + (side_row ? (c % CPR) * G * KL + kq : CINP) * SIDE_REC;
             int nxl = c + 1;
             if (SKIP)
                 while (nxl < NCHUNK && !chunk_live(y, nxl))
@@ -668,6 +704,12 @@
                         else if (!last)
                             bnl_fetch(nx, g + 2 - G, y, flip, nsc, nsh, nal, nraw);
                     }
+                    if (SIDE && tx == 0) {
+                        const float *wr = side_wrow + g * KL * SIDE_REC;
+#pragma unroll
+                        for (int k = 0; k < SCLS; ++k)
+                            sw[k] = wr[k];
+                    }
 #pragma unroll
                     for (int p = 0; p < P; ++p) {
                         acc[p] = M::run(aq[u % RA], BNL ? bt[BNL ? g & 1 : 0][p][S2P ? tx : 0]
@@ -678,9 +720,37 @@
                                 bnl_apply(bt[BNL ? (g + 1) & 1 : 0][e / 3][e % 3], bl[S2P ? (g + 1) % G : 0][e / 3][e % 3], tsc, tsh, tal, tpin,
                                           e == 0 && x0 == 0 && px == 0);
                         }
+                        if (SIDE && tx == 2) {
+                            const float *v = BNL ? bt[BNL ? g & 1 : 0][p] : bl[S2P ? g : 0][p];
+#pragma unroll
+                            for (int k = 0; k < SCLS; ++k) {
+                                side[p][k][0] = fmaf(sw[k], v[S2P ? 1 : 0], side[p][k][0]);
+                                side[p][k][1] = fmaf(sw[k], v[S2P ? 2 : 0], side[p][k][1]);
+                                asm volatile("" : "+v"(side[p][k][0]), "+v"(side[p][k][1]));
+                            }
+                        }
                     }
                     refill(u);
                     __builtin_amdgcn_sched_barrier(0);
+                }
+            }
+            if (SIDE && side_row && (c + 1) % CPR == 0) {
+                const int sside = (a.side_off + (y * STRIDE + side_ty - 1) * a.side_pitch + x0 * STRIDE) * 4;
+#pragma unroll
+                for (int p = 0; p < P; ++p) {
+                    const bool sok = kq == 0 && x0 + p * MT + px < a.W;
+#pragma unroll
+                    for (int k = 0; k < SCLS; ++k) {
+                        float o[2];
+#pragma unroll
+                        for (int dx = 0; dx < 2; ++dx) {
+                            const float own = side[p][k][dx];
+                            const float oth = __builtin_bit_cast(
+                                float, __builtin_amdgcn_ds_bpermute((lane ^ 32) << 2, __builtin_bit_cast(int, own)));
+                            o[dx] = kq == 0 ? own + oth : oth + own;
+                        }
+                        buf_store_vec<2>(rside, sok ? sside + (k * a.side_sc + (p * MT + px) * STRIDE) * 4 : OOB, o);
+                    }
                 }
             }
             if (stamp2)
@@ -752,7 +822,10 @@
     if (const char *e = std::getenv("GS_STAGGER"))
         a.stagger = std::atoi(e);
 #endif
-    constexpr int EXTRA = (FLAGS & F_BNLOAD) ? 3 * (CINP + Mfma<MT>::KL) : 0;
+    constexpr bool SIDE = (FLAGS >> F_SIDE_SHIFT) & 15;
+    constexpr int EXTRA = SIDE                 ? side_table_offset(im.total, CINP, Mfma<MT>::KL) - im.total + side_table_floats(CINP)
+                          : (FLAGS & F_BNLOAD) ? 3 * (CINP + Mfma<MT>::KL)
+                                               : 0;
     a.wfloats = im.total + EXTRA;
     const int lds_floats = im.total + EXTRA - ((FLAGS & F_A_GLOBAL) ? im.w : 0);
     const size_t lds_bytes = (size_t)((lds_floats + 255) / 256 * 256) * sizeof(float);
diff --git a/glomeruli_segmentation_amd/csrc/espnet.hip b/glomeruli_segmentation_amd/csrc/espnet.hip
--- a/glomeruli_segmentation_amd/csrc/espnet.hip
+++ b/glomeruli_segmentation_amd/csrc/espnet.hip
@@ -9,6 +9,7 @@
 #include <thread>
 #include <vector>
 
+#include "../../include/glomseg_plan.h"
 #include "conv_mfma.h"
 #include "dec_tail_args.h"
 #include "enc_head.h"
@@ -80,7 +81,7 @@
     void *ws = nullptr;
     size_t ws_bytes = 0;
     int ws_n = 0, ws_h = 0, ws_w = 0;
-    Act a0c, a0, inp1, inp2, r2[2], bb[3], a1, r3[2], cc[3], o2c, tt, t3, ee, ff;
+    Act a0c, a0, inp1, inp2, r2[2], bb[3], a1, r3[2], cc[3], o2c, l3c, tt, t3, ee, ff;
     float *prob = nullptr;
     size_t prob_bytes = 0;
     std::map<std::string, std::pair<Act, int>> stages;
@@ -171,7 +172,8 @@
 
 static bool pack_block(WeightTable &t, BlobBuilder &bb, const std::string &pre, bool down, int level, PackedConv &pc,
                        const float *dual = nullptr, int dual_coff = 0, int dual_c = 0, const std::string &next = "",
-                       const float *in2_bn = nullptr, int in2_c0 = 0, int in2_cn = 0, int in2_c = 0)
+                       const float *in2_bn = nullptr, int in2_c0 = 0, int in2_cn = 0, int in2_c = 0,
+                       const float *side_w = nullptr, int side_n = 0)
 {
     const int n = level == 2 ? 12 : 25, n1 = level == 2 ? 16 : 28, nOut = n1 + 4 * n;
     const int cin = level == 2 ? (down ? 19 : 64) : (down ? 131 : 128);
@@ -183,7 +185,12 @@
         return false;
     const int c1_floats = conv_wfloats(cinp, taps, 1, n, n, false);
     const int bnl_c = cinp + kl;
-    pc.c1 = bb.reserve(c1_floats + (in2_bn ? 3 * bnl_c : 0));
+    const int side_at = side_table_offset(c1_floats, cinp, kl);
+    pc.c1 = bb.reserve(side_w ? side_at + side_table_floats(cinp) : c1_floats + (in2_bn ? 3 * bnl_c : 0));
+    if (side_w)
+        for (int ch = 0; ch < cin; ++ch)
+            for (int k = 0; k < side_n; ++k)
+                bb.data[pc.c1 + side_at + (size_t)ch * SIDE_REC + k] = side_w[(size_t)k * cin + ch];
     pack_conv(wc1, n, cin, down ? 3 : 1, bb.data.data() + pc.c1, 0, taps, cinp, n);
     if (in2_bn) {
         float *x = bb.data.data() + pc.c1 + c1_floats;
@@ -269,6 +276,7 @@
     for (int i = 0; i < 3; ++i)
         m->cc[i] = make_act(128, 128, H3, W3, 0, 0, 0, 0);
     m->o2c = make_act(cls, cls, H2, W2, 0, 0, 0, 0);
+    m->l3c = !m->encoder_only && l3c_side_sums(cls) ? make_act(cls, cls, H2, W2, 0, 0, 0, 0) : make_act(1, 1, 8, 8, 0, 0, 0, 0);
     const bool dec3_mfma = dec3_on_mfma(cls);
     m->tt = dec3_mfma ? make_act(2 * cls, 2 * cls, H2, W2, 1, 1, 32, 1) : make_act(2 * cls, 2 * cls, H2, W2, 0, 0, 0, 0);
     m->t3 = dec3_mfma ? make_act(cls, cls, H2, W2, 0, 0, 0, 0) : make_act(1, 1, 8, 8, 0, 0, 0, 0);
@@ -277,7 +285,7 @@
     if (lazy_b2)
         m->bb[0] = Act();
     Act *all[] = {&m->a0c, &m->inp1, &m->inp2, &m->r2[0], &m->r2[1], &m->bb[0], &m->bb[1], &m->bb[2], &m->a1, &m->r3[0], &m->r3[1],
-                  &m->cc[0], &m->cc[1], &m->cc[2], &m->o2c, &m->tt, &m->t3, &m->ff};
+                  &m->cc[0], &m->cc[1], &m->cc[2], &m->o2c, &m->l3c, &m->tt, &m->t3, &m->ff};
     for (Act *a : all) {
         if ((unsigned long long)a->sn * sizeof(float) >= (1ull << 31)) {
             set_error("tile %dx%d is too large: an activation of one image exceeds 2 GiB", H, W);
@@ -459,8 +467,16 @@
     return not_planned("l2_esp_last");
 }
 
-static gs_status launch_l3_reduce(const Model *m, form::l3_reduce f, const ConvArgs &ca, hipStream_t s)
-{
+static gs_status launch_l3_reduce(const Model *m, form::l3_reduce f, bool side5, const ConvArgs &ca, hipStream_t s)
+{
+    constexpr int SIDE5 = F_SIDE1X1(5);
+    if (side5)
+        switch (f) {
+        case form::l3_reduce::BNL_P1: return launch_conv_mfma<CFG_L3_C1S_BNL_P1, F_S2PAIR | POL_L3_C1S | S2FLIP_L3 | F_BNLOAD | SIDE5>(ca, m->num_cus, s);
+        case form::l3_reduce::BNL: return launch_conv_mfma<CFG_L3_C1S_BNL, F_S2PAIR | POL_L3_C1S | S2FLIP_L3 | F_BNLOAD | SIDE5>(ca, m->num_cus, s);
+        case form::l3_reduce::C1S: return launch_conv_mfma<CFG_L3_C1S, F_S2PAIR | POL_L3_C1S | S2FLIP_L3 | SIDE5>(ca, m->num_cus, s);
+        case form::l3_reduce::none: return not_planned("l3_reduce");
+        }
     switch (f) {
     case form::l3_reduce::BNL_P1: return launch_conv_mfma<CFG_L3_C1S_BNL_P1, F_S2PAIR | POL_L3_C1S | S2FLIP_L3 | F_BNLOAD>(ca, m->num_cus, s);
     case form::l3_reduce::BNL:
@@ -649,15 +665,25 @@
     m->set_stage("b2", m->a1, 131);
 
     int rd3 = 0;
-    L.run(K_L3_C1S, px3 * (131 * 9 * 25 * 2), [&] {
+    L.run(K_L3_C1S, px3 * (131 * 9 * 25 * 2) + (plan.l3c_in_reduce ? px2 * (131 * m->classes * 2) : 0), [&] {
         GS_DIAG_TRY(diag_reduce_s2(m, 3, conv_args(m->a1, wb + m->l3_0.c1, m->r3[0], nullptr, n), s, dst_));
         ConvArgs ca = conv_args(m->a1, wb + m->l3_0.c1, m->r3[0], nullptr, n);
         if (lazy_b2) {
             ca.bnl_s0 = 64 / 2;
             ca.bnl_s1 = 128 / 2;
         }
-        return launch_l3_reduce(m, plan.l3_reduce, ca, s);
+        if (plan.l3c_in_reduce) {
+            ca.side = m->l3c.base;
+            ca.side_sn = m->l3c.sn;
+            ca.side_sc = m->l3c.sc;
+            ca.side_pitch = m->l3c.pitch;
+            ca.side_off = m->l3c.off;
+            ca.side_img_bytes = (unsigned)(m->l3c.sn * sizeof(float));
+        }
+        return launch_l3_reduce(m, plan.l3_reduce, plan.l3c_in_reduce, ca, s);
     });
+    if (plan.l3c_in_reduce)
+        m->set_stage("level3_C", m->l3c, m->classes);
     L.run(K_L3_DOWN, px3 * (25 * 9 * 128 * 2) + (m->l3_0.fused_next ? px3 * (128 * 25 * 2) : 0), [&] {
         const ConvArgs ca = conv_args(m->r3[rd3], wb + m->l3_0.br, m->cc[0], nullptr, n);
         return launch_l3_down(m, plan.l3_down, m->l3_0.fused_next ? with_fused(ca, m->r3[rd3 ^ 1], 25) : ca, s);
@@ -730,19 +756,26 @@
     }
     m->set_stage("up_l3", m->o2c, ncls);
 
-    L.run(K_DEC2, px2 * (131 * ncls * 2), [&] {
+    L.run(K_DEC2, plan.l3c_in_reduce ? 0 : px2 * (131 * ncls * 2), [&] {
         Dec2Args a{};
+        a.o2c = view(m->o2c);
+        a.br = wb + m->cbr0;
+        a.t = view(m->tt);
+        a.N = n;
+        a.classes = ncls;
+        if constexpr (l3c_side_sums(CLS)) {
+            if (plan.l3c_in_reduce) {
+                a.a1 = view(m->l3c);
+                hipLaunchKernelGGL(dec2_br_kernel<CLS>, dim3(blocks_for((long long)n * H2 * W2)), dim3(256), 0, s, a);
+                return GS_OK;
+            }
+        }
         a.a1 = view(m->a1);
         a.raw = view(m->bb[0]);
         a.b2 = wb + m->b2;
         a.raw_c0 = 64;
         a.raw_cn = enc.lazy_b2 ? 64 : 0;
-        a.o2c = view(m->o2c);
         a.w3c = wb + m->w3c;
-        a.br = wb + m->cbr0;
-        a.t = view(m->tt);
-        a.N = n;
-        a.classes = ncls;
         hipLaunchKernelGGL(dec2_kernel<CLS>, dim3((unsigned)(((long long)n * H2 * W2 + 63) / 64)), dim3(256), 0, s, a);
         return GS_OK;
     });
@@ -837,7 +870,7 @@
 static gs_status forward_any(Model *m, const ForwardReq &r)
 {
     Launcher L{m, r.s, GS_OK, r.n};
-    const ForwardPlan plan = plan_forward(r.n, r.H, r.W, m->p, m->q, m->cp, m->num_cus, no_vec());
+    const ForwardPlan plan = plan_forward(r.n, r.H, r.W, m->p, m->q, m->cp, m->num_cus, no_vec(), m->encoder_only);
     const Encoded e = encode(m, L, plan, r);
     switch (m->cp) {
     case 5: return decode<5>(m, L, plan, r, e);
@@ -1054,7 +1087,10 @@
     for (int i = 0; i < p; ++i)
         if (!pack_block(t, bb, e + "level2." + std::to_string(i), false, 2, m.l2[i], i == p - 1 ? b2f.data() : nullptr, 0, 131, next2(i + 1)))
             return GS_ERR_INVALID;
-    if (!pack_block(t, bb, e + "level3_0", true, 3, m.l3_0, nullptr, 0, 0, next3(0), b2f.data(), 64, 64, 131)) return GS_ERR_INVALID;
+    const float *w3c_side = nullptr;
+    if (!m.encoder_only && l3c_side_sums(m.cp) && !(w3c_side = t.get("level3_C.conv.weight", {classes, 131, 1, 1}))) return GS_ERR_INVALID;
+    if (!pack_block(t, bb, e + "level3_0", true, 3, m.l3_0, nullptr, 0, 0, next3(0), b2f.data(), 64, 64, 131, w3c_side, classes))
+        return GS_ERR_INVALID;
     m.l3.resize(q);
     for (int i = 0; i < q; ++i)
         if (!pack_block(t, bb, e + "level3." + std::to_string(i), false, 3, m.l3[i], nullptr, 0, 0, next3(i + 1))) return GS_ERR_INVALID;
@@ -1360,7 +1396,7 @@
             r = kind == 1 ? launch_l2_down(&m, unfused_l2_down(dst.W, no_vec()), bca, s)
                           : launch_l2_esp_fused(&m, unfused_l2_esp(dst.W, no_vec()), bca, s);
         } else {
-            r = kind == 1 ? launch_l3_reduce(&m, form::l3_reduce::C1S, rca, s) : launch_l3_c1(&m, rca, s);
+            r = kind == 1 ? launch_l3_reduce(&m, form::l3_reduce::C1S, false, rca, s) : launch_l3_c1(&m, rca, s);
             if (r != GS_OK) return r;
             r = kind == 1 ? launch_l3_down(&m, unfused_l3_down(dst.W, no_vec()), bca, s)
                           : launch_l3_esp_last(&m, whole_row_l3_esp(dst.W, no_vec()), bca, s);
@@ -1393,6 +1429,17 @@
         return GS_OK;
     GS_REQUIRE(cap >= kLaunchClassCount, "gs_espnet_plan_forward: %d entries needed, room for %d", kLaunchClassCount, cap);
     plan_forward(n, height, width, p, q, padded_classes(classes), num_cus, no_vec()).codes(out_forms);
+    return GS_OK;
+}
+
+gs_status gs_espnet_plan_flags(int n, int height, int width, int p, int q, int classes, int encoder_only, int num_cus, int *flags)
+{
+    GS_REQUIRE(flags, "gs_espnet_plan_flags: null argument");
+    int count = 0;
+    gs_status st = gs_espnet_plan_forward(n, height, width, p, q, classes, num_cus, nullptr, 0, &count);
+    if (st != GS_OK) return st;
+    const ForwardPlan pl = plan_forward(n, height, width, p, q, padded_classes(classes), num_cus, no_vec(), encoder_only != 0);
+    *flags = (pl.lazy_b2 ? GS_PLAN_LAZY_B2 : 0) | (pl.l3c_in_reduce ? GS_PLAN_L3C_IN_REDUCE : 0);
     return GS_OK;
 }
 
diff --git a/glomeruli_segmentation_amd/csrc/espnet_kernels.h b/glomeruli_segmentation_amd/csrc/espnet_kernels.h
--- a/glomeruli_segmentation_amd/csrc/espnet_kernels.h
+++ b/glomeruli_segmentation_amd/csrc/espnet_kernels.h
@@ -443,14 +443,6 @@
     for (int k = 0; k < CLS; ++k)
         s[k] = 0.0f;
     const int cb = 32 * w;
-#if defined(GS_DIAG) && defined(DEC2_X_NOCAT)
-    if (w == 0) {
-#pragma unroll
-        for (int k = 0; k < CLS; ++k)
-            s[k] = ld_stream<NT_DEC2_LD>(at(a.a1, n, k, y, x));
-    }
-    if (false)
-#endif
     if (cb >= a.raw_c0 && cb < a.raw_c0 + a.raw_cn) {
 #pragma unroll 16
         for (int c = cb; c < cb + 32; ++c) {
@@ -470,9 +462,6 @@
                 s[k] = fmaf(pc[k], v, s[k]);
         }
     }
-#if defined(GS_DIAG) && defined(DEC2_X_NOCAT)
-    if (false)
-#endif
     if (w == 3) {
 #pragma unroll
         for (int c = 128; c < 131; ++c) {
@@ -505,6 +494,25 @@
     for (int k = 0; k < 2 * CLS; ++k)
         if (k % CLS < ncls)
             *at(a.t, n, k, y, x) = tv[k];
+}
+
+template <int CLS>
+__global__ void __launch_bounds__(256) dec2_br_kernel(const Dec2Args a)
+{
+    const int H2 = a.t.H, W2 = a.t.W;
+    const long long idx = (long long)blockIdx.x * 256 + threadIdx.x;
+    if (idx >= (long long)a.N * H2 * W2)
+        return;
+    const int x = (int)(idx % W2);
+    const int y = (int)((idx / W2) % H2);
+    const int n = (int)(idx / ((long long)W2 * H2));
+    const int ncls = real_classes<CLS>(a.classes);
+#pragma unroll
+    for (int k = 0; k < CLS; ++k)
+        if (k < ncls) {
+            *at(a.t, n, k, y, x) = bn_prelu(*at(a.a1, n, k, y, x), a.br, 2 * CLS, k);
+            *at(a.t, n, CLS + k, y, x) = bn_prelu(*at(a.o2c, n, k, y, x), a.br, 2 * CLS, CLS + k);
+        }
 }
 
 struct Dec3Args {
diff --git a/glomeruli_segmentation_amd/csrc/forward_plan.h b/glomeruli_segmentation_amd/csrc/forward_plan.h
--- a/glomeruli_segmentation_amd/csrc/forward_plan.h
+++ b/glomeruli_segmentation_amd/csrc/forward_plan.h
@@ -10,6 +10,7 @@
 constexpr bool l2_c1_fused(int i, int p) { return CFG_FUSE_L2 && i < p; }
 constexpr bool l3_c1_fused(int i, int q) { return (CFG_FUSE_L3 == 2 || (CFG_FUSE_L3 == 1 && i == 0)) && i < q; }
 constexpr bool dec3_on_mfma(int cp) { return cp >= 12; }
+constexpr bool l3c_side_sums(int cp) { return cp == 5; }
 constexpr bool dec_tail_fused(int cp) { return cp == 5; }
 constexpr int dec_mt(int cp) { return cp <= 16 ? 16 : 32; }
 constexpr int dec_pixels(int cp) { return cp <= 16 ? 8 : 4; }
@@ -106,6 +107,7 @@
 struct ForwardPlan {
     GS_LAUNCH_CLASSES(GS_PLAN_MEMBER)
     bool lazy_b2 = false;
+    bool l3c_in_reduce = false;
     void codes(int *out) const { GS_LAUNCH_CLASSES(GS_PLAN_CODE) }
 };
 #undef GS_FORM_ID
@@ -139,13 +141,14 @@
     return vec_fits(form::l3_esp_last::BR_VEC, W3, no_vec) ? form::l3_esp_last::BR_VEC : form::l3_esp_last::P2;
 }
 
-inline ForwardPlan plan_forward(int n, int H, int W, int p, int q, int cp, int num_cus, bool no_vec)
+inline ForwardPlan plan_forward(int n, int H, int W, int p, int q, int cp, int num_cus, bool no_vec, bool encoder_only = false)
 {
     namespace f = form;
     const int W1 = W / 2, H2 = H / 4, W2 = W / 4, H3 = H / 8, W3 = W / 8;
     const long long cus = num_cus;
     ForwardPlan pl;
     pl.lazy_b2 = b2_is_lazy(p);
+    pl.l3c_in_reduce = !encoder_only && l3c_side_sums(cp);
 
     const bool small2 = CFG_SMALL2_WAVES > 0 && (long long)n * H2 * cdiv(W2, 64) * 2 <= cus * CFG_SMALL2_WAVES &&
                         vec_fits(f::l2_down::P2S_VEC, W2, no_vec);
diff --git a/glomeruli_segmentation_amd/engine.py b/glomeruli_segmentation_amd/engine.py
--- a/glomeruli_segmentation_amd/engine.py
+++ b/glomeruli_segmentation_amd/engine.py
@@ -274,6 +274,12 @@
     codes, count = (ctypes.c_int * len(table))(), ctypes.c_int()
     _lib.check(lib.gs_espnet_plan_forward(n, height, width, p, q, classes, num_cus, codes, len(table), ctypes.byref(count)))
     return {cls: forms[codes[k]][0] for k, (cls, forms) in enumerate(table) if codes[k] != _lib.GS_FORM_NONE}
+
+
+def plan_flags(n, height, width, p, q, classes, num_cus, encoder_only=False):
+    flags = ctypes.c_int()
+    _lib.check(_lib.load().gs_espnet_plan_flags(n, height, width, p, q, classes, int(bool(encoder_only)), num_cus, ctypes.byref(flags)))
+    return {"lazy_b2": bool(flags.value & _lib.GS_PLAN_LAZY_B2), "l3c_in_reduce": bool(flags.value & _lib.GS_PLAN_L3C_IN_REDUCE)}
 
 
 def crop_preprocess(crop_u8, mean, std, out_h, out_w, out=None):
diff --git a/include/glomseg_plan.h b/include/glomseg_plan.h
--- /dev/null
+++ b/include/glomseg_plan.h
@@ -0,0 +1,19 @@
+#ifndef GLOMSEG_PLAN_H
+#define GLOMSEG_PLAN_H
+
+#include "glomseg.h"
+
+#ifdef __cplusplus
+extern "C" {
+#endif
+
+#define GS_PLAN_LAZY_B2 1
+#define GS_PLAN_L3C_IN_REDUCE 2
+
+gs_status gs_espnet_plan_flags(int n, int height, int width, int p, int q, int classes, int encoder_only, int num_cus, int *flags);
+
+#ifdef __cplusplus
+}
+#endif
+
+#endif
```

New measurement: 11670 patches/s (median of 6 runs). 1.7% higher.
